# GRatTWCU/Social-STGCNN

Hardware: AMD Instinct MI355X
Metric: scene-windows/sec fwd+bwd (obs=8,pred=12) (higher is better)
Workload: dtype f32; 1 GPU; synthetic V=32 scene-windows, obs 8 / pred 12, batch 2048 per GPU, f32 (BASELINE north-star: V<=32, batch=2048; SURVEY 8d generator); global_batch=2048, step=aggregation + forward + bivariate NLL + backward + SGD update, parallelism=dp1

## Files before the change

include/stgcnn_hip.h:

```cpp
#ifndef STGCNN_HIP_H
#define STGCNN_HIP_H

#include <stddef.h>
#include <stdint.h>

#ifdef __cplusplus
extern "C" {
#endif

#define STG_OK 0
#define STG_EINVAL (-1)
#define STG_EUNSUPPORTED (-2)
#define STG_ELDS (-3)

#define STG_ABI_VERSION 8
#define STG_MAX_BLOCKS 4

int stg_abi_version(void);
const char *stg_last_error(void);

int stg_adj_build(const float *rel, int64_t rel_sn, int64_t rel_sv, int64_t rel_sc, int64_t rel_st,
                  const int32_t *num_peds, int N, int V, int T, int normalize,
                  float *nodes, float *adj, void *stream);

int stg_spatial_agg_fwd(const float *x, int64_t x_sn, int64_t x_sc, int64_t x_st, int64_t x_sv,
                        const float *adj, int64_t a_sn, const int32_t *num_peds,
                        int N, int C, int T, int V, float *y, void *stream);
int stg_spatial_agg_bwd(const float *dy, const float *adj, int64_t a_sn, const int32_t *num_peds,
                        int N, int C, int T, int V, float *dx, void *stream);

int stg_conv_t_fwd(const float *x, int64_t x_sn, int64_t x_sc, int64_t x_st, int64_t x_sv,
                   const float *w, const float *b, const int32_t *num_peds,
                   int N, int Cin, int Cout, int T, int V, int kt, int pad, float *y, void *stream);
int stg_conv_t_bwd(const float *x, int64_t x_sn, int64_t x_sc, int64_t x_st, int64_t x_sv,
                   const float *w, const float *dy, const int32_t *num_peds,
                   int N, int Cin, int Cout, int T, int V, int kt, int pad,
                   float *dx, float *dw, float *db, void *stream);

typedef struct {
    int32_t n_stgcnn;
    int32_t n_txpcnn;
    int32_t c_in;
    int32_t c_out;
    int32_t t_obs;
    int32_t t_pred;
    int32_t kt;
    int32_t residual0;
    int32_t use_mdn;
    int32_t bn_mode;
    float bn_eps;
    float bn_momentum;
    int32_t flags;
    int32_t wg_waves;
} stg_model_desc;

#define STG_OPT_WG_PATH 1
#define STG_OPT_SPLIT_BF16 2
#define STG_OPT_BF16_STORE 8
#define STG_OPT_F32_MFMA 16
#define STG_OPT_WAVE_PATH 4

int64_t stg_model_param_count(const stg_model_desc *d);
int64_t stg_model_buffer_count(const stg_model_desc *d);
int64_t stg_model_ws_floats(const stg_model_desc *d, int V);
int64_t stg_model_ws_tail_floats(const stg_model_desc *d, int N, int V);
int64_t stg_model_stat_floats(const stg_model_desc *d);
int64_t stg_model_fwd_scratch_floats(const stg_model_desc *d, int N, int V);
int64_t stg_model_bwd_scratch_floats(const stg_model_desc *d, int N, int V);

int stg_model_fwd(const stg_model_desc *d, const float *params, const float *buffers,
                  const float *x, int64_t x_sn, int64_t x_sc, int64_t x_st, int64_t x_sv,
                  const float *adj, int64_t a_sn, const int32_t *num_peds, int N, int V,
                  float *y, float *ws, float *stats, float *scratch, void **events, int n_events, void *stream);
int stg_model_bwd(const stg_model_desc *d, const float *params, const float *buffers,
                  const float *x, int64_t x_sn, int64_t x_sc, int64_t x_st, int64_t x_sv,
                  const float *adj, int64_t a_sn, const int32_t *num_peds, int N, int V,
                  const float *dy, const float *ws, float *scratch, float *grad_params, float *dx,
                  void **events, int n_events, void *stream);

int stg_model_bwd_nll(const stg_model_desc *d, const float *params, const float *buffers, const float *x, int64_t x_sn,
                      int64_t x_sc, int64_t x_st, int64_t x_sv, const float *adj, int64_t a_sn, const int32_t *num_peds,
                      int N, int V, const float *y, const float *target, const float *weights, float *losses,
                      const float *ws, float *scratch, float *grad_params, void **events, int n_events, void *stream);

typedef struct stg_step_tail {
    float *params;
    const float *lr_dev;
    float lr;
    const float *stats;
    float *buffers;
    int64_t *const *nbt;
    int n_bn;
    float *total;
} stg_step_tail;
int stg_model_bwd_step(const stg_model_desc *d, const float *params, const float *buffers, const float *x, int64_t x_sn,
                       int64_t x_sc, int64_t x_st, int64_t x_sv, const float *adj, int64_t a_sn, const int32_t *num_peds,
                       int N, int V, const float *y, const float *target, const float *weights, float *losses,
                       const float *ws, float *scratch, float *grad_params, const stg_step_tail *tail, void **events,
                       int n_events, void *stream);
int stg_bn_fold(const stg_model_desc *d, const float *stats, const int32_t *num_peds, int N,
                float *buffers, int64_t *const *nbt, int n_bn, void *stream);

int stg_nll_fwd(const float *pred, int64_t p_sn, int64_t p_sf, int64_t p_sp, int64_t p_sv,
                const float *target, const int32_t *num_peds, const float *grad_scale, int N, int P, int V,
                float *loss, float *grad, void *stream);
int stg_nll_bwd(const float *grad, const float *gloss, int N, int P, int V, float *out, void *stream);

int stg_sgd_step(float *params, const float *grads, int64_t count, float lr, void *stream);

int stg_scene_order(const int32_t *num_peds, int N, int V, int32_t *order, int32_t *key_start, void *stream);

int stg_optim_step(float *params, float *grads, int64_t count, const float *lr_dev, float lr, float max_norm,
                   float *grad_norm, void *stream);

int stg_gather_windows(const float *seq_rel_all, const int32_t *win_start, const int32_t *index, int n_windows, int N,
                       int V, int T_obs, int T_pred, float *obs_rel, float *target, int32_t *num_peds, void *stream);

int stg_dp_pack(const float *grads, const float *bn_before, const float *bn_after, const int32_t *num_peds, int N,
                float momentum, int rank, int world, int n_params, int n_buffers, float *pack, void *stream);
int stg_dp_fold(const float *pack, const float *bn_before, float momentum, int rank, int world, int n_params,
                int n_buffers, float *buffers, int64_t *const *nbt, int n_bn, void *stream);
int stg_weighted_sum(const float *values, const float *weights, int N, float *out, void *stream);

int stg_train_tail(const stg_model_desc *d, const float *stats, const int32_t *num_peds, int N, float *buffers,
                   int64_t *const *nbt, int n_bn, const float *losses, const float *weights, float *total,
                   float *params, float *grads, int64_t count, const float *lr_dev, float lr, float max_norm,
                   float *grad_norm, void *stream);

int stg_bestofk_eval(const float *pred, int64_t p_sn, int64_t p_sf, int64_t p_sp, int64_t p_sv,
                     const float *target_rel, const float *obs_last, const int32_t *num_peds, const float *noise,
                     uint64_t seed, int N, int P, int V, int K, float *ade, float *fde, void *stream);

int stg_sample_trajectories(const float *pred, int64_t p_sn, int64_t p_sf, int64_t p_sp, int64_t p_sv,
                            const float *obs_last, const int32_t *num_peds, const float *noise, uint64_t seed,
                            const uint64_t *seed_dev, int N, int P, int V, int K, float *samples, float *mean,
                            void *stream);

#define STG_TRACK_MAX_DETECTIONS 2048
#define STG_TRACK_MAX_SLOTS 2048
#define STG_TRACK_DUPLICATE 1
#define STG_TRACK_OVERFLOW 2
#define STG_TRACK_TRUNCATED 4
#define STG_TRACK_TOO_MANY 8
int stg_frame_scene_counts(const int32_t *frame_start, const int64_t *ids, int F, int T_obs, int32_t *count,
                           void *stream);
int stg_frame_scenes(const int32_t *frame_start, const int64_t *ids, const double *xy, const int32_t *frames, int N,
                     int V, int T_obs, double scale, double *obs_abs, int64_t *out_ids, int32_t *num_peds,
                     void *stream);
int stg_track_push(const int64_t *det_id, const double *det_xy, const int32_t *det_count, int M_max, int64_t *slot_id,
                   uint32_t *mask, double *ring, int32_t *head_flags, int S, int T_obs, double scale, int V,
                   double *obs_abs, int64_t *out_ids, int32_t *num_peds, void *stream);

#define STG_TRACK_MAX_STREAMS 4096
#define STG_TRACK_MAX_TOTAL_DETECTIONS (STG_TRACK_MAX_STREAMS * STG_TRACK_MAX_DETECTIONS)
int stg_track_push_streams(const int64_t *det_id, int64_t id_stride, const double *det_xy, int64_t xy_stride,
                           int M_total, const int32_t *det_start, const int32_t *pushed, int NS, int M_max,
                           int64_t *slot_id, uint32_t *mask, double *ring, int32_t *head_flags, int S, int T_obs,
                           double scale, int V, double *obs_abs, int64_t *out_ids, int32_t *num_peds,
                           int32_t *out_flags, int block_threads, void *stream);

int stg_fill_tracks(double *obs_abs, const int32_t *seen, const int32_t *num_peds, int N, int T_obs, int V,
                    double scale, void *stream);
int stg_frame_scene_counts_rule(const int32_t *frame_start, const int64_t *ids, int F, int T_obs, int min_seen,
                                int max_gap, int32_t *count, void *stream);
int stg_frame_scenes_rule(const int32_t *frame_start, const int64_t *ids, const double *xy, const int32_t *frames,
                          int N, int V, int T_obs, double scale, int min_seen, int max_gap, double *obs_abs,
                          int64_t *out_ids, int32_t *num_peds, int32_t *seen, void *stream);
int stg_track_push_rule(const int64_t *det_id, const double *det_xy, const int32_t *det_count, int M_max,
                        int64_t *slot_id, uint32_t *mask, double *ring, int32_t *head_flags, int S, int T_obs,
                        double scale, int V, int min_seen, int max_gap, double *obs_abs, int64_t *out_ids,
                        int32_t *num_peds, int32_t *seen, void *stream);
int stg_track_push_streams_rule(const int64_t *det_id, int64_t id_stride, const double *det_xy, int64_t xy_stride,
                                int M_total, const int32_t *det_start, const int32_t *pushed, int NS, int M_max,
                                int64_t *slot_id, uint32_t *mask, double *ring, int32_t *head_flags, int S, int T_obs,
                                double scale, int V, int min_seen, int max_gap, double *obs_abs, int64_t *out_ids,
                                int32_t *num_peds, int32_t *out_flags, int32_t *seen, int block_threads,
                                void *stream);

#define STG_TRACK_MAX_HISTORY 256
#define STG_TRACK_TIME_ORDER 16
int stg_track_push_timed(const int64_t *det_id, const double *det_xy, const int32_t *det_count,
                         const int64_t *det_time, int M_max, int64_t *slot_id, int64_t *t_ring, double *xy_ring,
                         int32_t *slot_head, int64_t *clock, int32_t *head_flags, int S, int R, int T_obs, double scale,
                         int V, int64_t step, int64_t max_dt, int min_seen, int max_gap, double *obs_abs,
                         int64_t *out_ids, int32_t *num_peds, int32_t *seen, void *stream);
int stg_track_push_streams_timed(const int64_t *det_id, int64_t id_stride, const double *det_xy, int64_t xy_stride,
                                 int M_total, const int32_t *det_start, const int32_t *pushed, const int64_t *det_time,
                                 int NS, int M_max, int64_t *slot_id, int64_t *t_ring, double *xy_ring,
                                 int32_t *slot_head, int64_t *clock, int32_t *head_flags, int S, int R, int T_obs,
                                 double scale, int V, int64_t step, int64_t max_dt, int min_seen, int max_gap,
                                 double *obs_abs, int64_t *out_ids, int32_t *num_peds, int32_t *out_flags,
                                 int32_t *seen, int block_threads, void *stream);

#define STG_RISK_MAX_V 256
#define STG_RISK_MAX_K 64
#define STG_RISK_MAX_Z 16
#define STG_RISK_MAX_P 32
int stg_sample_risk(const float *pred, int64_t p_sn, int64_t p_sf, int64_t p_sp, int64_t p_sv, const float *obs_last,
                    const int32_t *num_peds, const float *noise, uint64_t seed, const uint64_t *seed_dev, int N, int P,
                    int V, int K, float radius, const float *zones, int64_t z_sn, int Z, int32_t *conflict,
                    int32_t *conflict_any, int32_t *partner, int32_t *pair, int32_t *zone_any, int32_t *zone_count,
                    int32_t *ped_zone, void *stream);

#define STG_SCORE_MAX_V 256
#define STG_SCORE_MAX_K 64
#define STG_SCORE_MAX_P 32
#define STG_SCORE_MAX_Q 4
typedef struct stg_score_state {
    int64_t *rec_ids;
    int32_t *rec_peds;
    float *rec_mean, *rec_cov, *rec_samples, *acc, *acc_mean;
    int32_t *steps, *head;
    double *totals, *traj_totals;
} stg_score_state;
typedef struct stg_score_out {
    int64_t *rec_ids;
    int32_t *matched;
    float *err, *d2, *nll, *best;
    int32_t *traj_steps;
    float *traj_ade, *traj_fde, *traj_ade_mean, *traj_fde_mean;
} stg_score_out;
int stg_score_push(const int64_t *det_id, const double *det_xy, const int32_t *det_count, int M_max, double scale,
                   const float *mean, const float *v_pred, int64_t p_sn, int64_t p_sf, int64_t p_sp, int64_t p_sv,
                   const float *samples, const int64_t *ids, const int32_t *num_peds, int P, int V, int K,
                   const stg_score_state *state, const float *thr, int Q, const stg_score_out *out, void *stream);
int stg_score_push_streams(const int64_t *det_id, int64_t id_stride, const double *det_xy, int64_t xy_stride,
                           int M_total, const int32_t *det_start, const int32_t *pushed, int NS, int M_max,
                           double scale, const float *mean, const float *v_pred, int64_t p_sn, int64_t p_sf,
                           int64_t p_sp, int64_t p_sv, const float *samples, const int64_t *ids,
                           const int32_t *num_peds, int P, int V, int K, const stg_score_state *state,
                           const float *thr, int Q, const stg_score_out *out, void *stream);

#define STG_ASSOC_MAX_SLOTS STG_TRACK_MAX_SLOTS
#define STG_ASSOC_MAX_DETECTIONS STG_TRACK_MAX_DETECTIONS
#define STG_ASSOC_FULL 1
int stg_associate(int64_t *det_id, const double *det_xy, const int32_t *det_count, int M_max, int64_t *trk_id,
                  double *trk_pos, double *trk_vel, int32_t *trk_miss, int32_t *trk_hits, int64_t *next_id,
                  int32_t *assoc_flags, int C, double scale, double gate2, double gate_new2, int max_miss,
                  void *stream);
int stg_associate_streams(int64_t *det_id, int64_t id_stride, const double *det_xy, int64_t xy_stride, int M_total,
                          const int32_t *det_start, const int32_t *pushed, int NS, int M_max, int64_t *trk_id,
                          double *trk_pos, double *trk_vel, int32_t *trk_miss, int32_t *trk_hits, int64_t *next_id,
                          int32_t *assoc_flags, int C, double scale, double gate2, double gate_new2, int max_miss,
                          void *stream);

int stg_selftest_mfma(const float *a, const float *b, int K, float *c, void *stream);

#ifdef __cplusplus
}
#endif
#endif
```

social_stgcnn_amd/_lib.py:

```python
import ctypes
import os
import subprocess

import torch

_HERE = os.path.dirname(os.path.abspath(__file__))
CSRC = os.path.join(_HERE, "csrc")
DIAG = os.environ.get("STG_USE_DIAG_LIB", "0") not in ("", "0")
LIB_PATH = os.path.join(CSRC, "libstgcnn_hip_diag.so" if DIAG else "libstgcnn_hip.so")
ABI_VERSION = 8
OPT_WG_PATH, OPT_SPLIT_BF16, OPT_WAVE_PATH, OPT_BF16_STORE, OPT_F32_MFMA = 1, 2, 4, 8, 16
EUNSUPPORTED = -2

c_f = ctypes.c_void_p
c_i = ctypes.c_int
c_l = ctypes.c_int64


class ModelDesc(ctypes.Structure):
    _fields_ = [("n_stgcnn", ctypes.c_int32), ("n_txpcnn", ctypes.c_int32), ("c_in", ctypes.c_int32),
                ("c_out", ctypes.c_int32), ("t_obs", ctypes.c_int32), ("t_pred", ctypes.c_int32),
                ("kt", ctypes.c_int32), ("residual0", ctypes.c_int32), ("use_mdn", ctypes.c_int32),
                ("bn_mode", ctypes.c_int32), ("bn_eps", ctypes.c_float), ("bn_momentum", ctypes.c_float),
                ("flags", ctypes.c_int32), ("wg_waves", ctypes.c_int32)]


class ScoreState(ctypes.Structure):
    _fields_ = [(n, ctypes.c_void_p) for n in ("rec_ids", "rec_peds", "rec_mean", "rec_cov", "rec_samples", "acc",
                                               "acc_mean", "steps", "head", "totals", "traj_totals")]


class ScoreOut(ctypes.Structure):
    _fields_ = [(n, ctypes.c_void_p) for n in ("rec_ids", "matched", "err", "d2", "nll", "best", "traj_steps",
                                               "traj_ade", "traj_fde", "traj_ade_mean", "traj_fde_mean")]


_SIGNATURES = {
    "stg_abi_version": (c_i, []),
    "stg_last_error": (ctypes.c_char_p, []),
    "stg_adj_build": (c_i, [c_f, c_l, c_l, c_l, c_l, c_f, c_i, c_i, c_i, c_i, c_f, c_f, c_f]),
    "stg_spatial_agg_fwd": (c_i, [c_f, c_l, c_l, c_l, c_l, c_f, c_l, c_f, c_i, c_i, c_i, c_i, c_f, c_f]),
    "stg_spatial_agg_bwd": (c_i, [c_f, c_f, c_l, c_f, c_i, c_i, c_i, c_i, c_f, c_f]),
    "stg_conv_t_fwd": (c_i, [c_f, c_l, c_l, c_l, c_l, c_f, c_f, c_f, c_i, c_i, c_i, c_i, c_i, c_i, c_i, c_f, c_f]),
    "stg_conv_t_bwd": (c_i, [c_f, c_l, c_l, c_l, c_l, c_f, c_f, c_f, c_i, c_i, c_i, c_i, c_i, c_i, c_i,
                             c_f, c_f, c_f, c_f]),
    "stg_model_param_count": (c_l, [ctypes.POINTER(ModelDesc)]),
    "stg_model_buffer_count": (c_l, [ctypes.POINTER(ModelDesc)]),
    "stg_model_ws_floats": (c_l, [ctypes.POINTER(ModelDesc), c_i]),
    "stg_model_ws_tail_floats": (c_l, [ctypes.POINTER(ModelDesc), c_i, c_i]),
    "stg_model_stat_floats": (c_l, [ctypes.POINTER(ModelDesc)]),
    "stg_model_fwd_scratch_floats": (c_l, [ctypes.POINTER(ModelDesc), c_i, c_i]),
    "stg_model_bwd_scratch_floats": (c_l, [ctypes.POINTER(ModelDesc), c_i, c_i]),
    "stg_model_fwd": (c_i, [ctypes.POINTER(ModelDesc), c_f, c_f, c_f, c_l, c_l, c_l, c_l, c_f, c_l, c_f, c_i, c_i,
                            c_f, c_f, c_f, c_f, ctypes.POINTER(ctypes.c_void_p), c_i, c_f]),
    "stg_model_bwd": (c_i, [ctypes.POINTER(ModelDesc), c_f, c_f, c_f, c_l, c_l, c_l, c_l, c_f, c_l, c_f, c_i, c_i,
                            c_f, c_f, c_f, c_f, c_f, ctypes.POINTER(ctypes.c_void_p), c_i, c_f]),
    "stg_model_bwd_nll": (c_i, [ctypes.POINTER(ModelDesc), c_f, c_f, c_f, c_l, c_l, c_l, c_l, c_f, c_l, c_f, c_i, c_i,
                                c_f, c_f, c_f, c_f, c_f, c_f, c_f, ctypes.POINTER(ctypes.c_void_p), c_i, c_f]),
    "stg_model_bwd_step": (c_i, [ctypes.POINTER(ModelDesc), c_f, c_f, c_f, c_l, c_l, c_l, c_l, c_f, c_l, c_f, c_i, c_i,
                                 c_f, c_f, c_f, c_f, c_f, c_f, c_f, ctypes.c_void_p, ctypes.POINTER(ctypes.c_void_p), c_i,
                                 c_f]),
    "stg_bn_fold": (c_i, [ctypes.POINTER(ModelDesc), c_f, c_f, c_i, c_f, ctypes.POINTER(ctypes.c_void_p), c_i, c_f]),
    "stg_nll_fwd": (c_i, [c_f, c_l, c_l, c_l, c_l, c_f, c_f, c_f, c_i, c_i, c_i, c_f, c_f, c_f]),
    "stg_nll_bwd": (c_i, [c_f, c_f, c_i, c_i, c_i, c_f, c_f]),
    "stg_sgd_step": (c_i, [c_f, c_f, c_l, ctypes.c_float, c_f]),
    "stg_scene_order": (c_i, [c_f, c_i, c_i, c_f, c_f, c_f]),
    "stg_optim_step": (c_i, [c_f, c_f, c_l, c_f, ctypes.c_float, ctypes.c_float, c_f, c_f]),
    "stg_bestofk_eval": (c_i, [c_f, c_l, c_l, c_l, c_l, c_f, c_f, c_f, c_f, ctypes.c_uint64, c_i, c_i, c_i, c_i,
                               c_f, c_f, c_f]),
    "stg_sample_trajectories": (c_i, [c_f, c_l, c_l, c_l, c_l, c_f, c_f, c_f, ctypes.c_uint64, c_f, c_i, c_i, c_i, c_i,
                                      c_f, c_f, c_f]),
    "stg_sample_risk": (c_i, [c_f, c_l, c_l, c_l, c_l, c_f, c_f, c_f, ctypes.c_uint64, c_f, c_i, c_i, c_i, c_i,
                              ctypes.c_float, c_f, c_l, c_i, c_f, c_f, c_f, c_f, c_f, c_f, c_f, c_f]),
    "stg_gather_windows": (c_i, [c_f, c_f, c_f, c_i, c_i, c_i, c_i, c_i, c_f, c_f, c_f, c_f]),
    "stg_dp_pack": (c_i, [c_f, c_f, c_f, c_f, c_i, ctypes.c_float, c_i, c_i, c_i, c_i, c_f, c_f]),
    "stg_dp_fold": (c_i, [c_f, c_f, ctypes.c_float, c_i, c_i, c_i, c_i, c_f, ctypes.POINTER(ctypes.c_void_p), c_i, c_f]),
    "stg_weighted_sum": (c_i, [c_f, c_f, c_i, c_f, c_f]),
    "stg_train_tail": (c_i, [ctypes.POINTER(ModelDesc), c_f, c_f, c_i, c_f, ctypes.POINTER(ctypes.c_void_p), c_i, c_f, c_f,
                             c_f, c_f, c_f, c_l, c_f, ctypes.c_float, ctypes.c_float, c_f, c_f]),
    "stg_frame_scene_counts": (c_i, [c_f, c_f, c_i, c_i, c_f, c_f]),
    "stg_frame_scenes": (c_i, [c_f, c_f, c_f, c_f, c_i, c_i, c_i, ctypes.c_double, c_f, c_f, c_f, c_f]),
    "stg_track_push": (c_i, [c_f, c_f, c_f, c_i, c_f, c_f, c_f, c_f, c_i, c_i, ctypes.c_double, c_i, c_f, c_f, c_f,
                             c_f]),
    "stg_track_push_streams": (c_i, [c_f, c_l, c_f, c_l, c_i, c_f, c_f, c_i, c_i, c_f, c_f, c_f, c_f, c_i, c_i,
                                     ctypes.c_double, c_i, c_f, c_f, c_f, c_f, c_i, c_f]),
    "stg_fill_tracks": (c_i, [c_f, c_f, c_f, c_i, c_i, c_i, ctypes.c_double, c_f]),
    "stg_frame_scene_counts_rule": (c_i, [c_f, c_f, c_i, c_i, c_i, c_i, c_f, c_f]),
    "stg_frame_scenes_rule": (c_i, [c_f, c_f, c_f, c_f, c_i, c_i, c_i, ctypes.c_double, c_i, c_i, c_f, c_f, c_f, c_f,
                                    c_f]),
    "stg_track_push_rule": (c_i, [c_f, c_f, c_f, c_i, c_f, c_f, c_f, c_f, c_i, c_i, ctypes.c_double, c_i, c_i, c_i,
                                  c_f, c_f, c_f, c_f, c_f]),
    "stg_track_push_streams_rule": (c_i, [c_f, c_l, c_f, c_l, c_i, c_f, c_f, c_i, c_i, c_f, c_f, c_f, c_f, c_i, c_i,
                                          ctypes.c_double, c_i, c_i, c_i, c_f, c_f, c_f, c_f, c_f, c_i, c_f]),
    "stg_track_push_timed": (c_i, [c_f, c_f, c_f, c_f, c_i, c_f, c_f, c_f, c_f, c_f, c_f, c_i, c_i, c_i,
                                   ctypes.c_double, c_i, c_l, c_l, c_i, c_i, c_f, c_f, c_f, c_f, c_f]),
    "stg_track_push_streams_timed": (c_i, [c_f, c_l, c_f, c_l, c_i, c_f, c_f, c_f, c_i, c_i, c_f, c_f, c_f, c_f, c_f,
                                           c_f, c_i, c_i, c_i, ctypes.c_double, c_i, c_l, c_l, c_i, c_i, c_f, c_f, c_f,
                                           c_f, c_f, c_i, c_f]),
    "stg_score_push": (c_i, [c_f, c_f, c_f, c_i, ctypes.c_double, c_f, c_f, c_l, c_l, c_l, c_l, c_f, c_f, c_f, c_i, c_i,
                             c_i, ctypes.POINTER(ScoreState), c_f, c_i, ctypes.POINTER(ScoreOut), c_f]),
    "stg_score_push_streams": (c_i, [c_f, c_l, c_f, c_l, c_i, c_f, c_f, c_i, c_i, ctypes.c_double, c_f, c_f, c_l, c_l,
                                     c_l, c_l, c_f, c_f, c_f, c_i, c_i, c_i, ctypes.POINTER(ScoreState), c_f, c_i,
                                     ctypes.POINTER(ScoreOut), c_f]),
    "stg_associate": (c_i, [c_f, c_f, c_f, c_i, c_f, c_f, c_f, c_f, c_f, c_f, c_f, c_i, ctypes.c_double,
                            ctypes.c_double, ctypes.c_double, c_i, c_f]),
    "stg_associate_streams": (c_i, [c_f, c_l, c_f, c_l, c_i, c_f, c_f, c_i, c_i, c_f, c_f, c_f, c_f, c_f, c_f, c_f,
                                    c_i, ctypes.c_double, ctypes.c_double, ctypes.c_double, c_i, c_f]),
    "stg_selftest_mfma": (c_i, [c_f, c_f, c_i, c_f, c_f]),
}
EXPORTS = tuple(_SIGNATURES)

_lib = None


def build(verbose=False):
    cmd = ["make", "-C", CSRC, "-j8"] + (["DIAG=1"] if DIAG else [])
    res = subprocess.run(cmd, stdout=subprocess.PIPE, stderr=subprocess.STDOUT, text=True)
    if verbose or res.returncode != 0:
        print(res.stdout)
    if res.returncode != 0:
        raise RuntimeError("building libstgcnn_hip.so failed (exit %d)" % res.returncode)
    return LIB_PATH


def lib():
    global _lib
    if _lib is None:
        if not os.path.exists(LIB_PATH):
            raise RuntimeError(
                "social_stgcnn_amd: %s is missing -- build it with `make -C %s` (hipcc, "
                "--offload-arch=gfx950) or `python -c 'import __graft_entry__ as g; g.build()'`. "
                "There is no CPU or eager-PyTorch fallback for this path." % (LIB_PATH, CSRC))
        h = ctypes.CDLL(LIB_PATH)
        for name, (res, args) in _SIGNATURES.items():
            fn = getattr(h, name)
            fn.restype = res
            fn.argtypes = args
        if h.stg_abi_version() != ABI_VERSION:
            raise RuntimeError("libstgcnn_hip.so ABI %d != binding ABI %d" % (h.stg_abi_version(), ABI_VERSION))
        _lib = h
    return _lib


class StepTail(ctypes.Structure):
    _fields_ = [("params", ctypes.c_void_p), ("lr_dev", ctypes.c_void_p), ("lr", ctypes.c_float),
                ("stats", ctypes.c_void_p), ("buffers", ctypes.c_void_p), ("nbt", ctypes.POINTER(ctypes.c_void_p)),
                ("n_bn", ctypes.c_int), ("total", ctypes.c_void_p)]


class HipEvents:
    _hip = None

    @classmethod
    def hip(cls):
        if cls._hip is None:
            h = ctypes.CDLL("libamdhip64.so")
            h.hipEventCreate.argtypes = [ctypes.POINTER(ctypes.c_void_p)]
            h.hipEventElapsedTime.argtypes = [ctypes.POINTER(ctypes.c_float), ctypes.c_void_p, ctypes.c_void_p]
            h.hipEventSynchronize.argtypes = [ctypes.c_void_p]
            h.hipEventDestroy.argtypes = [ctypes.c_void_p]
            cls._hip = h
        return cls._hip

    def __init__(self, n):
        self.n = n
        self.arr = (ctypes.c_void_p * n)()
        for i in range(n):
            ev = ctypes.c_void_p()
            if self.hip().hipEventCreate(ctypes.byref(ev)) != 0:
                raise RuntimeError("hipEventCreate failed")
            self.arr[i] = ev

    def intervals_ms(self):
        out = []
        self.hip().hipEventSynchronize(self.arr[self.n - 1])
        for k in range(1, self.n):
            ms = ctypes.c_float()
            if self.hip().hipEventElapsedTime(ctypes.byref(ms), self.arr[k - 1], self.arr[k]) != 0:
                raise RuntimeError("hipEventElapsedTime failed")
            out.append(ms.value)
        return out

    def __del__(self):
        try:
            for i in range(self.n):
                self.hip().hipEventDestroy(self.arr[i])
        except Exception:
            pass


def check(rc, what):
    if rc != 0:
        msg = lib().stg_last_error().decode("utf-8", "replace")
        raise RuntimeError("%s failed (status %d): %s" % (what, rc, msg))


def stream_ptr():
    return ctypes.c_void_p(torch.cuda.current_stream().cuda_stream)


def ptr(t):
    if t is None:
        return None
    return ctypes.c_void_p(t.data_ptr())


def require_gpu(*tensors):
    for t in tensors:
        if t is not None and not t.is_cuda:
            raise RuntimeError("social_stgcnn_amd runs on MI355X only: got a %s tensor (no CPU fallback)"
                               % t.device.type)


def seed_u64(seed):
# ... 24 lines not shown
```

social_stgcnn_amd/csrc/model_bwd.hip:

```cpp
#include "model_common.hpp"
#include "stgcn_block.hpp"
#include "txp_scene_common.hpp"
#include "txp_f32_operands.hpp"
#include "step_plan.hpp"
#include "txp_wgrad.hpp"
#include "tail_parts.hpp"
#include "nll_elem.hpp"

namespace stg {

struct BwdArgs {
    ModelLayout lay;
    const float *params, *buffers, *x;
    int64_t x_sn, x_sc, x_st, x_sv;
    const float *adj;
    int64_t a_sn;
    const int32_t *num_peds;
    int N, V;
    const float *dy, *ws;
    const float *nll_target, *nll_weights;
    float *nll_losses;
    int64_t ws_stride;
    float *slab1;
    float *dzg;
// ... 200 lines not shown
                if (!STG_SKIP(a, 2)) {
                    if (l == 0)
                        txp_dgrad<Cfg::T, WAVES>(Pm + w_off, dzb, dcur, vi, false);
                    else
                        txp_dgrad<Cfg::P, WAVES>(Pm + w_off, dzb, dcur, vi, !is_out);
                }
                __syncthreads();
            }
        } else {
            for (int e = tid; e < C * T * vi; e += NT) {
                const int r = e / vi, w = e - r * vi;
                dcur[e] = dyn[(int64_t)r * V + w];
            }
            __syncthreads();
        }
        float *H1 = dzb, *DH2 = dzb + C * (T + 2) * Vl, *DB1 = DH2 + C * (T + 2) * Vl;
        for (int j = L.n_blocks - 1; j >= 0 && !STG_SKIP(a, 4); --j) {
            const float *xin = j > 0 ? wsn + L.ws_hdr_floats + (int64_t)L.blk[j - 1].ws_s * V : nullptr;
            float *dxs = j > 0 ? dcur : nullptr;
            float *dxg = j == 0 ? dxn : nullptr;
            if (L.blk[j].cin == Cfg::CIN0)
                stgcn_block_bwd<Cfg::CIN0, WAVES, true>(a, params, L.blk[j], n, vi, dcur, H1, DH2, DB1, red, tot, gsm, wsn,
                                                        xin, dxs, dxg, nullptr);
            else
                stgcn_block_bwd<Cfg::C, WAVES, true>(a, params, L.blk[j], n, vi, dcur, H1, DH2, DB1, red, tot, gsm, wsn, xin,
                                                     dxs, dxg, nullptr);
        }
    }
    __syncthreads();
    float *slab = a.slab1 + (int64_t)blockIdx.x * n_small;
    for (int e = tid; e < n_small; e += NT) slab[e] = gsm[e];
}

struct ReduceSeg {
    int p0, len, rows, row_stride;
    int64_t base;
};
struct ReduceArgs {
    ReduceSeg seg[kMaxTxp + 3];
    int n_seg;
    const float *slabs;
    float *grad;
    int n_params;
};

struct TailArgs {
    float *params;
    const float *lr_dev;
    float lr;
    const float *stats, *losses, *weights;
    const int32_t *num_peds;
    float *buffers, *total;
    NbtPtrs nbt;
    int n_reduce, n_buffers, N, stat_floats;
    float momentum;
};

__global__ __launch_bounds__(256) void reduce_slabs_kernel(const ReduceArgs a, const TailArgs t_) {
    __shared__ float part[32][8];
    if ((int)blockIdx.x >= t_.n_reduce) {
        float *acc_s = &part[0][0];
        __shared__ float dec_s[256];
        __shared__ int cnt_s[256];
        const int b = (int)blockIdx.x - t_.n_reduce;
        if (b < t_.n_buffers)
            bn_fold_body<256>(b, t_.stats, t_.num_peds, t_.N, t_.stat_floats, t_.momentum, t_.buffers, t_.nbt, acc_s, dec_s,
                              cnt_s);
        else if (t_.total)
            weighted_sum_body(t_.losses, t_.weights, t_.N, t_.total, acc_s);
        return;
    }
    const int col = threadIdx.x & 7, grp = threadIdx.x >> 3;
    const int p = blockIdx.x * 8 + col;
    float s = 0.f;
    if (p < a.n_params) {
        for (int q = 0; q < a.n_seg; ++q) {
            const ReduceSeg g = a.seg[q];
            if (p >= g.p0 && p < g.p0 + g.len) {
                const float *src = a.slabs + g.base + (p - g.p0);
                int k = grp;
                for (; k + 992 < g.rows; k += 1024) {
                    float v[32];
#pragma unroll
                    for (int u = 0; u < 32; ++u) v[u] = src[(int64_t)(k + 32 * u) * g.row_stride];
#pragma unroll
                    for (int u = 0; u < 32; ++u) s += v[u];
                }
                for (; k + 480 < g.rows; k += 512) {
                    float v[16];
#pragma unroll
                    for (int u = 0; u < 16; ++u) v[u] = src[(int64_t)(k + 32 * u) * g.row_stride];
#pragma unroll
                    for (int u = 0; u < 16; ++u) s += v[u];
                }
                for (; k + 96 < g.rows; k += 128) {
                    float v[4];
#pragma unroll
                    for (int u = 0; u < 4; ++u) v[u] = src[(int64_t)(k + 32 * u) * g.row_stride];
#pragma unroll
                    for (int u = 0; u < 4; ++u) s += v[u];
                }
                for (; k < g.rows; k += 32) s += src[(int64_t)k * g.row_stride];
            }
        }
    }
    part[grp][col] = s;
    __syncthreads();
    if (grp == 0 && p < a.n_params) {
        float t = 0.f;
#pragma unroll
        for (int g = 0; g < 32; ++g) t += part[g][col];
        a.grad[p] = t;
        if (t_.params) t_.params[p] -= (t_.lr_dev ? t_.lr_dev[0] : t_.lr) * t;
    }
}

static int env_waves(const char *name, int dflt) {
    const int w = diag_env(name, dflt);
    return (w == 1 || w == 2 || w == 4 || w == 8) ? w : dflt;
}

static size_t bwd_lds_bytes(const ModelLayout &L, int V, int waves) {
    const int plane = Cfg::P * txp_sc(V);
    const int st = (2 * Cfg::C * (Cfg::T + 2) + Cfg::C * Cfg::T) * V;
    const int reg = plane > st ? plane : st;
    const int dcur = Cfg::P * Cfg::C * V;
    const int n_small = L.n_blk_params + L.n_txp;
    const size_t fl = ((n_small + 3) & ~3) + (size_t)reg + (size_t)dcur + (size_t)waves * kRedMax + kRedMax;
    return fl * sizeof(float);
}

static int bwd_waves(const StepPath &path, int V) {
    return path.wg_waves ? path.wg_waves : (V <= 40 ? 1 : (V <= 80 ? 4 : 8));
}

static int bwd_grid_w(const ModelLayout &L, int N, int V, int waves) {
    const size_t lds = bwd_lds_bytes(L, V, waves);
    if (lds > (size_t)kLdsBytes) return -1;
    int per_cu = (int)(kLdsBytes / lds);
    const int by_waves = 8 / waves > 0 ? 8 / waves : 1;
    if (per_cu > by_waves) per_cu = by_waves;
    if (per_cu < 1) per_cu = 1;
    int grid = kNumCU * per_cu;
    if (const int g = diag_env("STG_BWD_GRID", 0)) grid = g > 0 ? g : grid;
    return grid < N ? grid : N;
}
static int bwd_grid(const ModelLayout &L, const StepPath &path, int N, int V) { return bwd_grid_w(L, N, V, bwd_waves(path, V)); }
constexpr int kBwdTierV = 32;
static int bwd_grid_small(const ModelLayout &L, int N, int V) {
    return V > kBwdTierV ? bwd_grid_w(L, N, kBwdTierV, 1) : 0;
}

struct BwdCarve {
    int64_t rows, slab2, dzg, order, total;
};
static bool bwd_carve(const ModelLayout &L, const StepPath &path, int N, int V, BwdCarve *c, WgradGeom *wg) {
    const int g1 = bwd_grid(L, path, N, V);
    if (g1 < 0) return false;
    int gs = bwd_grid_small(L, N, V);
    if (gs < 0) gs = 0;
    int64_t n_rows = g1 + gs;
    if (path.scene() && N > n_rows) n_rows = N;
    c->rows = 0;
    int64_t fl = (n_rows * (L.n_blk_params + L.n_txp) + 3) & ~(int64_t)3;
    c->slab2 = fl;
    c->dzg = fl;
    if (L.n_txp > 0) {
        if (!wgrad_geom(L, N, V, wg)) return false;
        fl = (fl + wgrad_slab_base(L.L + 1, wg->rows) + 3) & ~(int64_t)3;
        c->dzg = fl;
        fl = (fl + (int64_t)N * (L.L + 1) * dz_slot(V) + 3) & ~(int64_t)3;
    }
    c->order = fl;
    c->total = fl + order_floats(N, V);
    return true;
}

}

extern "C" {

int64_t stg_model_bwd_scratch_floats(const stg_model_desc *d, int N, int V) {
    stg::ModelLayout l;
    const int rc = stg::make_layout(d, &l);
    if (rc != STG_OK) return rc;
    if (N <= 0 || V <= 0) return stg::fail(STG_EINVAL, "stg_model_bwd_scratch_floats: N=%d V=%d", N, V);
    stg::BwdCarve c;
    stg::WgradGeom wg{};
    if (!stg::bwd_carve(l, stg::choose_path(l, N, V), N, V, &c, &wg)) return stg::fail(STG_ELDS, "stg_model_bwd: V=%d does not fit the LDS of one CU", V);
    return c.total;
}

static int model_bwd_impl(const stg_model_desc *d, const float *params, const float *buffers, const float *x, int64_t x_sn,
                          int64_t x_sc, int64_t x_st, int64_t x_sv, const float *adj, int64_t a_sn,
                          const int32_t *num_peds, int N, int V, const float *dy, const float *nll_target,
                          const float *nll_weights, float *nll_losses, const stg_step_tail *tail, const float *ws,
                          float *scratch, float *grad_params, float *dx, void **events, int n_events, void *stream) {
    using namespace stg;
    BwdArgs a{};
    const int rc = make_layout(d, &a.lay);
    if (rc != STG_OK) return rc;
    const ModelLayout &L = a.lay;
    STG_REQUIRE(N >= 0 && V > 0, STG_EINVAL, "stg_model_bwd: bad sizes N=%d V=%d", N, V);
    STG_REQUIRE(grad_params, STG_EINVAL, "stg_model_bwd: null grad_params");
    STG_REQUIRE(N == 0 || (params && buffers && x && adj && dy && ws && scratch), STG_EINVAL,
                "stg_model_bwd: null pointer");
    STG_REQUIRE((reinterpret_cast<uintptr_t>(ws) & 15) == 0 && (reinterpret_cast<uintptr_t>(scratch) & 15) == 0,
                STG_EINVAL, "stg_model_bwd: ws / scratch must be 16-byte aligned");
    hipStream_t st = as_stream(stream);
    EventList evl{events, events ? n_events : 0, 0, st};
    evl.mark();
    if (N == 0) {
        hipError_t e = hipMemsetAsync(grad_params, 0, sizeof(float) * L.n_params, st);
        if (e != hipSuccess) return hip_fail(e, "stg_model_bwd: memset");
        return STG_OK;
    }
    BwdCarve cv;
    WgradGeom wg{};
    const StepPath path = choose_path(L, N, V);
    STG_REQUIRE(bwd_carve(L, path, N, V, &cv, &wg), STG_ELDS, "stg_model_bwd: V=%d does not fit the LDS of one CU", V);
    const int n_small = L.n_blk_params + L.n_txp;
    float *rows = scratch + cv.rows, *slab2 = scratch + cv.slab2;
    float *dzg = L.n_txp > 0 ? scratch + cv.dzg : nullptr;
    STG_REQUIRE(path.scene() || !(L.flags & STG_OPT_BF16_STORE), STG_EUNSUPPORTED,
                "stg_model_bwd: bf16 storage (STG_OPT_BF16_STORE) is built for the wave-per-scene kernels only");
    STG_REQUIRE(!((L.flags & STG_OPT_BF16_STORE) && (L.flags & STG_OPT_SPLIT_BF16)), STG_EUNSUPPORTED,
                "stg_model_bwd: STG_OPT_BF16_STORE and STG_OPT_SPLIT_BF16 cannot be combined");
    if (nll_target && ((L.flags & STG_OPT_SPLIT_BF16) || L.n_txp == 0))
        return STG_EUNSUPPORTED;
    STG_REQUIRE(!(path.scene() && dx), STG_EUNSUPPORTED,
                "stg_model_bwd: dx is only computed by the workgroup-per-scene kernels: set STG_OPT_WG_PATH in the "
                "descriptor of the forward and the backward call");
    a.params = params; a.buffers = buffers; a.x = x;
    a.x_sn = x_sn; a.x_sc = x_sc; a.x_st = x_st; a.x_sv = x_sv;
    a.adj = adj; a.a_sn = a_sn; a.num_peds = num_peds; a.N = N; a.V = V;
    a.nll_target = nll_target; a.nll_weights = nll_weights; a.nll_losses = nll_losses;
    a.dy = dy; a.ws = ws; a.ws_stride = ws_floats_per_scene(L, V); a.slab1 = rows; a.dzg = dzg; a.dx = dx;
    int32_t *order = reinterpret_cast<int32_t *>(scratch + cv.order);
    bool sorted;
    const WsTail wt = ws_tail(L, path, N, V);
    const float *ws_end = ws + wt.base;
    if (tail_has_order(path, num_peds, N, V)) {
        order = reinterpret_cast<int32_t *>(const_cast<float *>(ws_end) + wt.order);
        sorted = true;
    } else {
        sorted = launch_scene_order(num_peds, N, V, order, order + N, st, order + N + V + 2);
    }
    int32_t *order_peds = order + N + V + 2;
    const int serp = diag_env("STG_WALK", 1);
    a.tier = SceneTier{sorted ? order : nullptr, sorted ? order + N : nullptr, -1, V, serp};
    a.debug_skip = diag_env("STG_DEBUG_SKIP", 0);
    int slab_rows;
    if (path.scene()) {
        TxpBwdArgs t{};
        t.lay = L; t.params = params; t.num_peds = num_peds; t.N = N; t.V = V; t.dy = dy; t.ws = ws;
        t.nll_target = nll_target; t.nll_weights = nll_weights; t.nll_losses = nll_losses;
        t.x = x; t.x_sn = x_sn; t.x_sc = x_sc; t.x_st = x_st; t.x_sv = x_sv; t.adj = adj; t.a_sn = a_sn;
        t.ws_stride = a.ws_stride; t.dzg = dzg; t.rows = rows;
        t.tier = a.tier;
        t.Vl = V;
        t.debug_skip = a.debug_skip;
        t.split_bf16 = (L.flags & STG_OPT_SPLIT_BF16) ? 1 : 0;
        t.stagger = diag_env("STG_STAGGER_B", 0);
        if (wt.wp >= 0) t.wp = reinterpret_cast<const unsigned *>(ws_end + wt.wp);
        const int rcw = launch_scene_bwd(path, t, st);
        if (rcw != STG_OK) return rcw;
        slab_rows = N;
    } else {
        const int waves = bwd_waves(path, V);
        const size_t lds = bwd_lds_bytes(L, V, waves);
        STG_REQUIRE(lds <= (size_t)kLdsBytes, STG_ELDS, "stg_model_bwd: V=%d needs %zu bytes of LDS (> %d)", V, lds,
                    kLdsBytes);
        const int grid = bwd_grid(L, path, N, V);
        void (*k1)(BwdArgs, const float *);
        switch (waves) {
            case 1: k1 = model_bwd_kernel<1>; break;
            case 2: k1 = model_bwd_kernel<2>; break;
            case 4: k1 = model_bwd_kernel<4>; break;
            default: k1 = model_bwd_kernel<8>; break;
        }
        slab_rows = grid;
        const int grid_small = a.tier.order ? bwd_grid_small(L, N, V) : 0;
        if (grid_small > 0) a.tier.v_lo = kBwdTierV;
        int rck = launch(Launch{"stg_model_bwd: K1", dim3(grid), dim3(waves * 64), lds, st}, k1, a, params);
        if (rck != STG_OK) return rck;
        if (grid_small > 0) {
            a.Vl = kBwdTierV;
            a.tier.v_lo = -1; a.tier.v_hi = kBwdTierV;
            a.slab1 = rows + (int64_t)grid * n_small;
            rck = launch(Launch{"stg_model_bwd: K1 (small scenes)", dim3(grid_small), dim3(64), bwd_lds_bytes(L, kBwdTierV, 1), st},
                         model_bwd_kernel<1>, a, params);
            if (rck != STG_OK) return rck;
            slab_rows = grid + grid_small;
            a.slab1 = rows;
            a.Vl = 0;
            a.tier.v_hi = V;
        }
    }
    evl.mark();

    ReduceArgs r{};
    r.slabs = scratch;
    r.grad = grad_params;
    r.n_params = L.n_params;
    r.seg[r.n_seg++] = ReduceSeg{0, L.n_blk_params, slab_rows, n_small, cv.rows};
    if (L.n_txp > 0) {
        r.seg[r.n_seg++] = ReduceSeg{L.prelus, L.n_txp, slab_rows, n_small, cv.rows + (int64_t)L.n_blk_params};
        WgradArgs w{};
        w.lay = L; w.num_peds = num_peds; w.order = a.tier.order; w.order_peds = sorted ? order_peds : nullptr;
        w.key_start = a.tier.key_start;
        w.serpentine = a.tier.serpentine; w.N = N; w.V = V;
        w.ws = ws; w.dzg = dzg; w.ws_stride = a.ws_stride; w.slab2 = slab2; w.rows = wg.rows; w.debug_skip = a.debug_skip;
        for (int l = 0; l <= L.L + 1; ++l) w.wg_begin[l] = wg.wg_begin[l];
        if (!STG_SKIP(a, 1)) {
            const int rck = launch_txp_wgrad(w, wg, st);
            if (rck != STG_OK) return rck;
        }
        evl.mark();
        for (int l = 0; l <= L.L; ++l) {
            const int p0 = l == L.L ? L.out_w : L.txp_w[l];
            r.seg[r.n_seg++] = ReduceSeg{p0, wgrad_row_len(l), STG_SKIP(a, 1) ? 0 : wg.wg_begin[l + 1] - wg.wg_begin[l],
                                         wgrad_row_len(l), cv.slab2 + wgrad_slab_base(l, wg.rows)};
        }
    }
    TailArgs ta{};
    ta.n_reduce = (L.n_params + 7) / 8;
    int extra = 0;
    if (tail) {
        ta.params = tail->params; ta.lr_dev = tail->lr_dev; ta.lr = tail->lr;
        ta.stats = tail->stats; ta.buffers = tail->buffers; ta.total = tail->total;
        ta.losses = nll_losses; ta.weights = nll_weights; ta.num_peds = num_peds;
        ta.N = N; ta.stat_floats = L.stat_floats; ta.momentum = d->bn_momentum;
        ta.n_buffers = (tail->stats && N > 0) ? L.n_buffers : 0;
        ta.nbt.n = tail->nbt ? tail->n_bn : 0;
        for (int k = 0; k < ta.nbt.n; ++k) ta.nbt.p[k] = tail->nbt[k];
        extra = ta.n_buffers + 1;
    }
    hipLaunchKernelGGL(reduce_slabs_kernel, dim3(ta.n_reduce + extra), dim3(256), 0, st, r, ta);
    STG_LAUNCH_CHECK("stg_model_bwd: reduce_slabs");
    evl.mark();
    evl.finish();
    return STG_OK;
}

int stg_model_bwd(const stg_model_desc *d, const float *params, const float *buffers, const float *x, int64_t x_sn,
                  int64_t x_sc, int64_t x_st, int64_t x_sv, const float *adj, int64_t a_sn, const int32_t *num_peds,
                  int N, int V, const float *dy, const float *ws, float *scratch, float *grad_params, float *dx,
                  void **events, int n_events, void *stream) {
    return model_bwd_impl(d, params, buffers, x, x_sn, x_sc, x_st, x_sv, adj, a_sn, num_peds, N, V, dy, nullptr, nullptr,
                          nullptr, nullptr, ws, scratch, grad_params, dx, events, n_events, stream);
}

int stg_model_bwd_nll(const stg_model_desc *d, const float *params, const float *buffers, const float *x, int64_t x_sn,
                      int64_t x_sc, int64_t x_st, int64_t x_sv, const float *adj, int64_t a_sn, const int32_t *num_peds,
                      int N, int V, const float *y, const float *target, const float *weights, float *losses,
                      const float *ws, float *scratch, float *grad_params, void **events, int n_events, void *stream) {
    if (!target || !losses || (N > 0 && !y)) return stg::fail(STG_EINVAL, "stg_model_bwd_nll: null pointer");
    return model_bwd_impl(d, params, buffers, x, x_sn, x_sc, x_st, x_sv, adj, a_sn, num_peds, N, V, y, target, weights,
                          losses, nullptr, ws, scratch, grad_params, nullptr, events, n_events, stream);
}

int stg_model_bwd_step(const stg_model_desc *d, const float *params, const float *buffers, const float *x, int64_t x_sn,
                       int64_t x_sc, int64_t x_st, int64_t x_sv, const float *adj, int64_t a_sn, const int32_t *num_peds,
                       int N, int V, const float *y, const float *target, const float *weights, float *losses,
                       const float *ws, float *scratch, float *grad_params, const stg_step_tail *tail, void **events,
                       int n_events, void *stream) {
    if (!target || !losses || (N > 0 && !y)) return stg::fail(STG_EINVAL, "stg_model_bwd_step: null pointer");
    if (!tail || !tail->params || (tail->stats && !tail->buffers) || tail->n_bn < 0 || tail->n_bn > 3 * STG_MAX_BLOCKS)
        return stg::fail(STG_EINVAL, "stg_model_bwd_step: bad tail");
    if (N == 0) return STG_EUNSUPPORTED;
    return model_bwd_impl(d, params, buffers, x, x_sn, x_sc, x_st, x_sv, adj, a_sn, num_peds, N, V, y, target, weights,
                          losses, tail, ws, scratch, grad_params, nullptr, events, n_events, stream);
}

}
```

social_stgcnn_amd/csrc/model_fwd.hip:

```cpp
#include "model_common.hpp"
#include "stgcn_block.hpp"
#include "txp_scene_common.hpp"
#include "txp_f32_operands.hpp"
#include "step_plan.hpp"

namespace stg {

struct FwdArgs {
    ModelLayout lay;
    const float *params, *buffers, *x;
    int64_t x_sn, x_sc, x_st, x_sv;
    const float *adj;
    int64_t a_sn;
    const int32_t *num_peds;
    int N, V;
    float *y, *ws;
    int64_t ws_stride;
    float *stats;
    const int32_t *order;
    const float *agg;
    int64_t agg_stride, agg_ax, agg_cs;
    int debug_skip;
};

// ... 4 lines not shown
                              const float *in, float *out, int vi, int V, float *zsave, float *yout) {
    constexpr int C = Cfg::C, P = Cfg::P, KS = CINL * 9 / 4;
    const int lane = threadIdx.x & 63, wave = threadIdx.x >> 6;
    const int nq = lane & 15, kq = lane >> 4;
    const int SW = txp_sw(vi), SC = txp_sc(vi);
    const int npos = C * vi, ntiles = (npos + 15) >> 4;
    float wreg[KS];
    load_w_fwd<CINL>(W, wreg);
    f32x4 binit;
#pragma unroll
    for (int r = 0; r < 4; ++r) binit[r] = (4 * kq + r) < P ? bias[4 * kq + r] : 0.f;

    for (int tile0 = wave * 2; tile0 < ntiles; tile0 += WAVES * 2) {
        int pos[2], hh[2], ww[2], base[2];
        bool ok[2];
#pragma unroll
        for (int u = 0; u < 2; ++u) {
            pos[u] = (tile0 + u) * 16 + nq;
            ok[u] = pos[u] < npos;
            const int pc = ok[u] ? pos[u] : 0;
            hh[u] = pc / vi;
            ww[u] = pc - hh[u] * vi;
            base[u] = kq * SC + hh[u] * SW + ww[u];
        }
        f32x4 acc0 = binit, acc1 = binit;
#pragma unroll
        for (int tap = 0; tap < 9; ++tap) {
            const int toff = (tap / 3) * SW + (tap % 3);
#pragma unroll
            for (int j = 0; j < CINL / 4; ++j) {
                const float b0 = in[base[0] + 4 * j * SC + toff];
                const float b1 = in[base[1] + 4 * j * SC + toff];
                acc0 = __builtin_amdgcn_mfma_f32_16x16x4f32(wreg[tap * (CINL / 4) + j], b0, acc0, 0, 0, 0);
                acc1 = __builtin_amdgcn_mfma_f32_16x16x4f32(wreg[tap * (CINL / 4) + j], b1, acc1, 0, 0, 0);
            }
        }
#pragma unroll
        for (int u = 0; u < 2; ++u) {
            if (!ok[u] || kq == 3) continue;
            const f32x4 acc = u == 0 ? acc0 : acc1;
#pragma unroll
            for (int r = 0; r < 4; ++r) {
                const int co = 4 * kq + r;
                const float z = acc[r];
                const int flat = (co * C + hh[u]) * vi + ww[u];
                if (kind == 2) {
                    yout[(int64_t)(co * C + hh[u]) * V + ww[u]] = z;
                } else {
                    const int li = co * SC + (hh[u] + 1) * SW + (ww[u] + 1);
                    float av = z > 0.f ? z : alpha * z;
                    if (kind == 1) av += in[li];
                    out[li] = av;
                    if (zsave) zsave[flat] = z;
                }
            }
        }
    }
}

template <int WAVES>
__global__ __launch_bounds__(WAVES * 64) void model_fwd_kernel(const FwdArgs a, const float *__restrict__ params,
                                                               const float *__restrict__ buffers) {
    constexpr int C = Cfg::C, T = Cfg::T, P = Cfg::P, NT = WAVES * 64;
    extern __shared__ __attribute__((aligned(16))) float sm[];
    const int V = a.V, tid = threadIdx.x;
    const int xin_floats = C * T * V;
    const int plane_floats = fwd_plane_floats(V);
    const int reg_floats = plane_floats > 3 * C * T * V ? plane_floats : 3 * C * T * V;
    float *bufA = sm;
    float *reg = bufA + plane_floats;
    float *red = reg + reg_floats;
    const ModelLayout &L = a.lay;
    const int c_in = L.blk[0].cin;
    const int out_rows = L.n_txp > 0 ? C * P : C * T;

    for (int it = blockIdx.x; it < a.N; it += gridDim.x) {
        const int n = a.order ? a.order[it] : it;
        int vi = a.num_peds ? a.num_peds[n] : V;
        vi = vi < 0 ? 0 : (vi > V ? V : vi);
        float *yn = a.y + (int64_t)n * out_rows * V;
        if (vi < V)
            for (int e = tid; e < out_rows * (V - vi); e += NT) {
                const int r = e / (V - vi), w = vi + (e - r * (V - vi));
                yn[(int64_t)r * V + w] = 0.f;
            }
        if (vi == 0) continue;
        float *wsn = a.ws ? a.ws + n * a.ws_stride : nullptr;
        float *statn = a.stats ? a.stats + (int64_t)n * L.stat_floats : nullptr;
        const int SW = txp_sw(vi), SC = txp_sc(vi);
        __syncthreads();
        float *X = reg, *G = reg + xin_floats, *H = G + C * T * V;
        {
            const float *xn = a.x + n * a.x_sn;
            for (int e = tid; e < c_in * T * vi; e += NT) {
                const int v = e % vi, ct = e / vi, t = ct % T, c = ct / T;
                X[e] = xn[c * a.x_sc + t * a.x_st + v * a.x_sv];
            }
            if (L.n_txp > 0) {
                float4 *z4 = reinterpret_cast<float4 *>(bufA);
                for (int e = tid; e < ((P * SC) >> 2); e += NT) z4[e] = make_float4(0.f, 0.f, 0.f, 0.f);
            }
        }
        __syncthreads();
        for (int j = 0; j < L.n_blocks && !STG_SKIP(a, 32); ++j) {
            const bool last = j == L.n_blocks - 1;
            float *yb = (last && L.n_txp == 0) ? yn : nullptr;
            const float *pax = j == 0 ? a.agg + n * a.agg_stride + a.agg_ax : nullptr;
            const float *pcs = j == 0 ? a.agg + n * a.agg_stride + a.agg_cs : nullptr;
            if (L.blk[j].cin == Cfg::CIN0)
                stgcn_block_fwd<Cfg::CIN0, WAVES>(a, params, buffers, L.blk[j], n, vi, X, G, H, red, wsn, statn, pax, pcs,
                                                  last && L.n_txp > 0, bufA, SC, bufA, 0, yb, !last);
            else
                stgcn_block_fwd<Cfg::C, WAVES>(a, params, buffers, L.blk[j], n, vi, X, G, H, red, wsn, statn, pax, pcs,
                                               last && L.n_txp > 0, bufA, SC, bufA, 0, yb, !last);
            float *tmp = X; X = H; H = tmp;
        }
        if (L.n_txp == 0 || STG_SKIP(a, 16)) continue;
        float *bufB = reg;
        for (int e = tid; e < P * SC; e += NT) bufB[e] = 0.f;
        __syncthreads();
        const float *__restrict__ Pm = params;
        float *in = bufA, *out = bufB;
        auto save_plane = [&](const float *pl, int idx) {
            if (!wsn) return;
            float *dst = wsn + ws_plane_off(L, V, idx);
            for (int h = 0; h < C; ++h)
                for (int e = tid; e < SW * P; e += NT) {
                    const int col = e / P, ch = e - col * P;
                    dst[(h * SW) * P + e] = pl[ch * SC + (h + 1) * SW + col];
                }
        };
        save_plane(in, 0);
        for (int l = 0; l < L.L; ++l) {
            float *zs = wsn ? wsn + L.ws_hdr_floats + (int64_t)L.ws_z[l] * V : nullptr;
            const float alpha = Pm[L.prelus + l];
            if (l == 0)
                txp_layer_fwd<Cfg::T, WAVES>(Pm + L.txp_w[0], Pm + L.txp_b[0], alpha, 0, in, out, vi, V, zs, nullptr);
            else
                txp_layer_fwd<Cfg::P, WAVES>(Pm + L.txp_w[l], Pm + L.txp_b[l], alpha, 1, in, out, vi, V, zs, nullptr);
            __syncthreads();
            float *tmp = in; in = out; out = tmp;
            save_plane(in, l + 1);
        }
        txp_layer_fwd<Cfg::P, WAVES>(Pm + L.out_w, Pm + L.out_b, 0.f, 2, in, out, vi, V, nullptr, yn);
    }
}

static size_t fwd_lds_bytes(int V, int waves) {
    const int plane = fwd_plane_floats(V);
    const int reg = plane > 3 * Cfg::C * Cfg::T * V ? plane : 3 * Cfg::C * Cfg::T * V;
    return (size_t)(plane + reg + waves * 16 + 16) * sizeof(float);
}

}

extern "C" int stg_model_fwd(const stg_model_desc *d, const float *params, const float *buffers, const float *x,
                             int64_t x_sn, int64_t x_sc, int64_t x_st, int64_t x_sv, const float *adj,
                             int64_t a_sn, const int32_t *num_peds, int N, int V, float *y, float *ws,
                             float *stats, float *scratch, void **events, int n_events, void *stream) {
    using namespace stg;
    FwdArgs a{};
    const int rc = make_layout(d, &a.lay);
    if (rc != STG_OK) return rc;
    STG_REQUIRE(N >= 0 && V > 0, STG_EINVAL, "stg_model_fwd: bad sizes N=%d V=%d", N, V);
    if (N == 0) return STG_OK;
    STG_REQUIRE(params && buffers && x && adj && y, STG_EINVAL, "stg_model_fwd: null pointer");
    STG_REQUIRE(scratch && (reinterpret_cast<uintptr_t>(scratch) & 15) == 0, STG_EINVAL,
                "stg_model_fwd: scratch (stg_model_fwd_scratch_floats floats, 16-byte aligned) is missing");
    STG_REQUIRE(!ws || (reinterpret_cast<uintptr_t>(ws) & 15) == 0, STG_EINVAL, "stg_model_fwd: ws must be 16-byte aligned");
    const ModelLayout &L = a.lay;
    a.params = params; a.buffers = buffers; a.x = x;
    a.x_sn = x_sn; a.x_sc = x_sc; a.x_st = x_st; a.x_sv = x_sv;
    a.adj = adj; a.a_sn = a_sn; a.num_peds = num_peds; a.N = N; a.V = V;
    a.y = y; a.ws = ws; a.ws_stride = ws_floats_per_scene(L, V); a.stats = stats;
    const StepPath path = choose_path(L, N, V);
    const FwdCarve fc = fwd_carve(L, path, N, V);
    const WsTail wt = ws_tail(L, path, N, V);
    float *ws_end = ws ? ws + wt.base : nullptr;
    STG_REQUIRE(path.scene() || !(L.flags & STG_OPT_BF16_STORE), STG_EUNSUPPORTED,
                "stg_model_fwd: bf16 storage (STG_OPT_BF16_STORE) is built for the wave-per-scene kernels only "
                "(one st_gcn block, input_feat 2, V <= 68, no STG_OPT_WG_PATH)");
    hipStream_t st = as_stream(stream);
    EventList evl{events, events ? n_events : 0, 0, st};
    evl.mark();
    const BlockLayout &b0 = L.blk[0];
    if (ws) {
        a.agg = ws; a.agg_stride = a.ws_stride;
        a.agg_ax = L.ws_hdr_floats + (int64_t)b0.ws_ax * V;
        a.agg_cs = L.ws_hdr_floats + (int64_t)b0.ws_cs * V;
    } else {
        a.agg = scratch + fc.agg; a.agg_stride = (int64_t)(b0.cin + 1) * Cfg::T * V;
        a.agg_ax = 0;
        a.agg_cs = (int64_t)b0.cin * Cfg::T * V;
    }
    a.debug_skip = diag_env("STG_DEBUG_SKIP", 0);
    int32_t *order = reinterpret_cast<int32_t *>(ws_end && path.scene() ? ws_end + wt.order : scratch + fc.order);
    bool sorted_in_agg = false;
    {
        AggPrep prep{};
        prep.params = params;
        prep.n_layers = L.L + 1;
        for (int l = 0; l <= L.L; ++l) prep.w_off[l] = l < L.L ? L.txp_w[l] : L.out_w;
        if (ws_end && wt.wp >= 0) prep.wp = reinterpret_cast<unsigned *>(ws_end + wt.wp);
        if (fc.wp_fwd >= 0) prep.wp_fwd = reinterpret_cast<unsigned *>(scratch + fc.wp_fwd);
        sorted_in_agg = path.scene() && agg_sorts(num_peds, N, V);
        if (sorted_in_agg) { prep.order = order; prep.key_start = order + N; prep.order_peds = order + N + V + 2; }
        const int rca = launch_stgcn_agg(b0.cin, x, x_sn, x_sc, x_st, x_sv, adj, a_sn, num_peds, N, V,
                                         const_cast<float *>(a.agg), a.agg_stride, a.agg_ax, a.agg_cs, st,
                                         (prep.wp || prep.wp_fwd || prep.order) ? &prep : nullptr);
        if (rca != STG_OK) return rca;
    }
    evl.mark();
    if (path.scene()) {
        bool sorted = sorted_in_agg;
        if (!sorted) {
            sorted = launch_scene_order(num_peds, N, V, order, order + N, st, order + N + V + 2);
            if (!sorted && scene_order_applies(num_peds, N, V)) return hip_fail(hipErrorLaunchFailure, "stg_model_fwd: scene_order launch");
        }
        TxpFwdArgs t{};
        t.lay = L; t.params = params; t.buffers = buffers; t.num_peds = num_peds; t.N = N; t.V = V;
        t.x = x; t.x_sn = x_sn; t.x_sc = x_sc; t.x_st = x_st; t.x_sv = x_sv;
        t.adj = adj; t.a_sn = a_sn;
        t.agg = a.agg; t.agg_stride = a.agg_stride; t.agg_ax = a.agg_ax; t.agg_cs = a.agg_cs;
        t.y = y; t.ws = ws; t.ws_stride = a.ws_stride; t.stats = stats;
        if (fc.wp_fwd >= 0) t.wpf = reinterpret_cast<const unsigned *>(scratch + fc.wp_fwd);
        if (fc.stamps >= 0) t.stamps = reinterpret_cast<unsigned long long *>(scratch + fc.stamps);
        const int serp = diag_env("STG_WALK", 1);
        t.tier = SceneTier{sorted ? order : nullptr, sorted ? order + N : nullptr, -1, V, serp};
        t.Vl = V;
        t.debug_skip = a.debug_skip;
        t.stagger = diag_env("STG_STAGGER_F", 0);
        const int rcw = launch_scene_fwd(path, t, st);
        evl.mark();
        evl.finish();
        return rcw;
    }
    int waves = V <= 12 ? 1 : (V <= 40 ? 2 : (V <= 80 ? 4 : 8));
    if (path.wg_waves) waves = path.wg_waves;
    const size_t lds = fwd_lds_bytes(V, waves);
    STG_REQUIRE(lds <= (size_t)kLdsBytes, STG_ELDS, "stg_model_fwd: V=%d needs %zu bytes of LDS (> %d)", V, lds,
                kLdsBytes);
    const Launch lc{"stg_model_fwd", dim3((unsigned)N), dim3(waves * 64), lds, st};
    int rck;
    switch (waves) {
        case 1: rck = launch(lc, model_fwd_kernel<1>, a, params, buffers); break;
        case 2: rck = launch(lc, model_fwd_kernel<2>, a, params, buffers); break;
        case 4: rck = launch(lc, model_fwd_kernel<4>, a, params, buffers); break;
        default: rck = launch(lc, model_fwd_kernel<8>, a, params, buffers); break;
    }
    if (rck != STG_OK) return rck;
    evl.mark();
    evl.finish();
    return STG_OK;
}
```

social_stgcnn_amd/csrc/model_layout.hip:

```cpp
#include <cstring>
#include <type_traits>
#include "model_common.hpp"
#include "scene_order.hpp"
#include "step_plan.hpp"
#include "txp_wave.hpp"

namespace stg {

int make_layout(const stg_model_desc *d, ModelLayout *lay) {
    STG_REQUIRE(d && lay, STG_EINVAL, "model descriptor is null");
    STG_REQUIRE(d->n_stgcnn >= 1 && d->n_stgcnn <= STG_MAX_BLOCKS, STG_EUNSUPPORTED,
                "n_stgcnn=%d outside 1..%d", d->n_stgcnn, STG_MAX_BLOCKS);
    STG_REQUIRE(d->n_txpcnn >= 0 && d->n_txpcnn <= kMaxTxp, STG_EUNSUPPORTED, "n_txpcnn=%d outside 0..%d",
                d->n_txpcnn, kMaxTxp);
    STG_REQUIRE(d->c_out == Cfg::C && d->t_obs == Cfg::T && d->kt == Cfg::KT, STG_EUNSUPPORTED,
                "fused kernels are built for output_feat=%d seq_len=%d kernel_size=%d (got %d,%d,%d)", Cfg::C,
                Cfg::T, Cfg::KT, d->c_out, d->t_obs, d->kt);
    STG_REQUIRE(d->c_in == Cfg::CIN0 || d->c_in == Cfg::C, STG_EUNSUPPORTED,
                "fused kernels are built for input_feat %d or %d (got %d)", Cfg::CIN0, Cfg::C, d->c_in);
    STG_REQUIRE(d->n_txpcnn == 0 || d->t_pred == Cfg::P, STG_EUNSUPPORTED,
                "fused kernels are built for pred_seq_len=%d (got %d)", Cfg::P, d->t_pred);
    STG_REQUIRE(d->bn_mode == 0 || d->bn_mode == 1, STG_EINVAL, "bn_mode=%d (0 eval, 1 per-scene train)", d->bn_mode);
    STG_REQUIRE(d->residual0 >= 0 && d->residual0 <= 2, STG_EINVAL, "residual0=%d", d->residual0);
    STG_REQUIRE(d->residual0 != 1 || d->c_in == d->c_out, STG_EINVAL, "identity residual needs c_in == c_out");
    STG_REQUIRE((d->flags & ~(STG_OPT_WG_PATH | STG_OPT_SPLIT_BF16 | STG_OPT_WAVE_PATH | STG_OPT_BF16_STORE | STG_OPT_F32_MFMA)) == 0, STG_EINVAL,
                "unknown flags 0x%x", d->flags);
    STG_REQUIRE(d->wg_waves == 0 || d->wg_waves == 1 || d->wg_waves == 2 || d->wg_waves == 4 || d->wg_waves == 8,
                STG_EINVAL, "wg_waves=%d (0 auto, 1, 2, 4, 8)", d->wg_waves);
    ModelLayout &l = *lay;
    l = layout_of(ModelShape{d->n_stgcnn, d->n_txpcnn, d->c_in, d->residual0, d->use_mdn});
    l.bn_mode = d->bn_mode;
    l.eps = d->bn_eps;
    l.momentum = d->bn_momentum;
    l.flags = d->flags;
    l.wg_waves = d->wg_waves;
    return STG_OK;
}

bool is_canonical(const ModelLayout &L) {
    ModelLayout c = L;
    c.eps = kCanonLayout.eps;
    c.momentum = kCanonLayout.momentum;
    c.bn_mode = kCanonLayout.bn_mode;
    c.flags = kCanonLayout.flags;
    c.wg_waves = kCanonLayout.wg_waves;
    static_assert(std::is_trivially_copyable<ModelLayout>::value && sizeof(ModelLayout) % 4 == 0, "compared bytewise");
    return std::memcmp(&c, &kCanonLayout, sizeof c) == 0;
}

constexpr int kSmallBatch = 288;

StepPath choose_path(const ModelLayout &L, int N, int V) {
    StepPath p{StepPath::Workgroup, L.wg_waves, txp_fwd_x6_fits(L, V), txp_bwd_x6_fits(L, V)};
    if (L.n_txp < 1 || L.n_blocks != 1 || L.blk[0].cin != Cfg::CIN0 || (L.flags & STG_OPT_WG_PATH)) return p;
    if (p.fwd_x6 && p.bwd_x6) {
        p.kind = StepPath::SceneX6;
    } else if (txp_wave_f32_fits(V)) {
        if (N >= kSmallBatch || L.wg_waves != 0 || V > 40 || (L.flags & (STG_OPT_WAVE_PATH | STG_OPT_BF16_STORE)))
            p.kind = StepPath::WaveF32;
        else
            p.wg_waves = N <= 192 ? 8 : 4;
    }
    return p;
}

FwdCarve fwd_carve(const ModelLayout &L, const StepPath &path, int N, int V) {
    const bool stamps = diag_env("STG_STAMPS", 0) != 0;
    FwdCarve c;
    c.agg = 0;
    c.order = (((int64_t)N * (L.blk[0].cin + 1) * Cfg::T * V + 3) & ~(int64_t)3) + 4;
    c.stamps = stamps ? c.order + order_floats(N, V) : -1;
    const int64_t wp = (c.order + order_floats(N, V) + (stamps ? (int64_t)N * 32 : 0) + 3) & ~(int64_t)3;
    c.wp_fwd = path.scene() && path.fwd_x6 ? wp : -1;
    c.total = wp + (path.fwd_x6 ? txp_bwd_x6_wp_floats(L) : 0);
    return c;
}

WsTail ws_tail(const ModelLayout &L, const StepPath &path, int N, int V) {
    WsTail t;
    t.base = (int64_t)N * ws_floats_per_scene(L, V);
    t.wp = path.scene() && path.bwd_x6 ? 0 : -1;
    t.order = path.bwd_x6 ? txp_bwd_x6_wp_floats(L) : 0;
    t.total = t.order + order_floats(N, V);
    return t;
}

int launch_scene_fwd(const StepPath &path, const TxpFwdArgs &a, hipStream_t st) {
    return path.fwd_x6 ? launch_txp_fwd_x6(a, st) : launch_txp_fwd_wave(a, st);
}
int launch_scene_bwd(const StepPath &path, const TxpBwdArgs &a, hipStream_t st) {
    return path.bwd_x6 ? launch_txp_bwd_x6(a, st) : launch_txp_bwd_wave(a, st);
}

__global__ __launch_bounds__(1024) void scene_order_kernel(const int32_t *__restrict__ num_peds, int N, int V,
                                                           int32_t *__restrict__ order,
                                                           int32_t *__restrict__ key_start,
                                                           int32_t *__restrict__ order_peds) {
    extern __shared__ int hist[];
    __shared__ int wave_tot[16];
    scene_order_body<16>(num_peds, N, V, order, key_start, order_peds, hist, wave_tot);
}

bool launch_scene_order(const int32_t *num_peds, int N, int V, int32_t *order, int32_t *key_start, hipStream_t st,
                        int32_t *order_peds) {
    if (!order || !scene_order_applies(num_peds, N, V)) return false;
    const size_t lds = (size_t)(V + 1) * 16 * sizeof(int);
    if (lds > 48 * 1024 &&
        hipFuncSetAttribute(reinterpret_cast<const void *>(&scene_order_kernel),
                            hipFuncAttributeMaxDynamicSharedMemorySize, (int)lds) != hipSuccess)
        return false;
    hipLaunchKernelGGL(scene_order_kernel, dim3(1), dim3(1024), lds, st, num_peds, N, V, order, key_start, order_peds);
    return hipGetLastError() == hipSuccess;
}

}

extern "C" {

int64_t stg_model_param_count(const stg_model_desc *d) {
    stg::ModelLayout l;
    const int rc = stg::make_layout(d, &l);
    return rc == STG_OK ? l.n_params : rc;
}
int64_t stg_model_buffer_count(const stg_model_desc *d) {
    stg::ModelLayout l;
    const int rc = stg::make_layout(d, &l);
    return rc == STG_OK ? l.n_buffers : rc;
}
int64_t stg_model_ws_floats(const stg_model_desc *d, int V) {
    stg::ModelLayout l;
    const int rc = stg::make_layout(d, &l);
    if (rc != STG_OK) return rc;
    if (V <= 0) return stg::fail(STG_EINVAL, "stg_model_ws_floats: V=%d", V);
    return stg::ws_floats_per_scene(l, V);
}
int64_t stg_model_ws_tail_floats(const stg_model_desc *d, int N, int V) {
    stg::ModelLayout l;
    const int rc = stg::make_layout(d, &l);
    if (rc != STG_OK) return rc;
    if (N < 0 || V <= 0) return stg::fail(STG_EINVAL, "stg_model_ws_tail_floats: N=%d V=%d", N, V);
    return stg::ws_tail(l, stg::choose_path(l, N, V), N, V).total;
}
int64_t stg_model_fwd_scratch_floats(const stg_model_desc *d, int N, int V) {
    stg::ModelLayout l;
    const int rc = stg::make_layout(d, &l);
    if (rc != STG_OK) return rc;
    if (N < 0 || V <= 0) return stg::fail(STG_EINVAL, "stg_model_fwd_scratch_floats: N=%d V=%d", N, V);
    return stg::fwd_carve(l, stg::choose_path(l, N, V), N, V).total;
}
int stg_scene_order(const int32_t *num_peds, int N, int V, int32_t *order, int32_t *key_start, void *stream) {
    STG_REQUIRE(N >= 0 && V > 0, STG_EINVAL, "stg_scene_order: bad sizes N=%d V=%d", N, V);
    if (N == 0) return STG_OK;
    STG_REQUIRE(num_peds && order, STG_EINVAL, "stg_scene_order: null pointer");
    STG_REQUIRE(N >= 2, STG_EUNSUPPORTED, "stg_scene_order: a single scene needs no order");
    STG_REQUIRE(N <= stg::kOrderMaxN && V <= stg::kOrderMaxV, STG_EUNSUPPORTED,
                "stg_scene_order: N=%d V=%d outside the single-workgroup sort (N <= %d, V <= %d)", N, V,
                stg::kOrderMaxN, stg::kOrderMaxV);
    STG_REQUIRE(stg::launch_scene_order(num_peds, N, V, order, key_start, stg::as_stream(stream)), STG_EINVAL,
                "stg_scene_order: launch failed");
    return STG_OK;
}

int64_t stg_model_stat_floats(const stg_model_desc *d) {
    stg::ModelLayout l;
    const int rc = stg::make_layout(d, &l);
    return rc == STG_OK ? l.stat_floats : rc;
}

}
```

social_stgcnn_amd/csrc/step_plan.hpp:

```cpp
#pragma once
#include "model_common.hpp"

namespace stg {

struct TxpFwdArgs;
struct TxpBwdArgs;

struct StepPath {
    enum Kind { SceneX6, WaveF32, Workgroup } kind;
    int wg_waves;
    bool fwd_x6, bwd_x6;
    bool scene() const { return kind != Workgroup; }
};
StepPath choose_path(const ModelLayout &L, int N, int V);

struct FwdCarve {
    int64_t agg, order, stamps, wp_fwd, total;
};
FwdCarve fwd_carve(const ModelLayout &L, const StepPath &path, int N, int V);

struct WsTail {
    int64_t base, wp, order, total;
};
WsTail ws_tail(const ModelLayout &L, const StepPath &path, int N, int V);
inline bool tail_has_order(const StepPath &path, const int32_t *num_peds, int N, int V) {
    return path.scene() && scene_order_applies(num_peds, N, V);
}

int launch_scene_fwd(const StepPath &path, const TxpFwdArgs &a, hipStream_t st);
int launch_scene_bwd(const StepPath &path, const TxpBwdArgs &a, hipStream_t st);

}
```

social_stgcnn_amd/csrc/txp_scene_common.hpp:

```cpp
#pragma once
#include "model_common.hpp"
#include "stgcn_block.hpp"

namespace stg {

struct MixGeom {
    int on;
    int v_small, v_mid;
    int block_floats;
};

constexpr int kTeamMaxV = 128;
struct TeamGeom {
    int on;
    int v1, v2;
    int region_floats;
};

struct TxpFwdArgs {
    ModelLayout lay;
    const float *params, *buffers;
    const int32_t *num_peds;
    SceneTier tier;
    int Vl;
    MixGeom mix;
    TeamGeom team;
    int N, V;
    const float *x;
    int64_t x_sn, x_sc, x_st, x_sv;
    const float *adj;
    int64_t a_sn;
    const float *agg;
    int64_t agg_stride, agg_ax, agg_cs;
    float *y;
    const unsigned *wpf;
    float *ws;
    int64_t ws_stride;
    float *stats;
    unsigned long long *stamps;
    int debug_skip;
    int stagger;
};

struct TxpBwdArgs {
    ModelLayout lay;
    const float *params;
    const int32_t *num_peds;
    SceneTier tier;
    int Vl;
    MixGeom mix;
    TeamGeom team;
    int N, V;
    const float *x;
    int64_t x_sn, x_sc, x_st, x_sv;
    const float *adj;
    int64_t a_sn;
    const float *dy;
    const float *nll_target;
    const float *nll_weights;
    float *nll_losses;
    const float *ws;
    int64_t ws_stride;
    float *dzg;
    const unsigned *wp;
    float *rows;
    int debug_skip;
    int split_bf16;
    int stagger;
};

bool txp_fwd_x6_fits(const ModelLayout &L, int V);
bool txp_bwd_x6_fits(const ModelLayout &L, int V);
int64_t txp_bwd_x6_wp_floats(const ModelLayout &L);
int launch_txp_fwd_x6(const TxpFwdArgs &a, hipStream_t st);
int launch_txp_bwd_x6(const TxpBwdArgs &a, hipStream_t st);

__host__ __device__ inline int ptab_floats(int v) { return ((Cfg::T * v + 1) / 2 + 3) & ~3; }
__host__ __device__ inline int bwd_ptab_floats(int v) { return ptab_floats(v) + kRedMax; }
__host__ __device__ inline int wave_param_floats(const ModelLayout &L) {
    return ((L.n_blk_params + 3) & ~3) + ((L.n_buffers + 3) & ~3);
}

__device__ __forceinline__ void build_ptab(ptab_t *ptab, int vi) {
    const int lane = threadIdx.x & 63;
    for (int p = lane; p < Cfg::T * vi; p += 64) {
        const int h = p / vi;
        ptab[p] = (ptab_t)((h << 8) | (p - h * vi));
    }
}
__device__ __forceinline__ void build_ptab(ptab_t *ptab, int w0, int wc) {
    const int lane = threadIdx.x & 63;
    if (wc <= 0 && lane == 0) ptab[0] = 0;
    for (int p = lane; p < Cfg::T * wc; p += 64) {
        const int h = p / wc;
        ptab[p] = (ptab_t)((h << 8) | (w0 + p - h * wc));
    }
}


__device__ __forceinline__ void vm_drain() { __builtin_amdgcn_s_waitcnt(0x0F70); }

__device__ __forceinline__ void stage_block_params(const ModelLayout &L, const float *__restrict__ params,
                                                   const float *__restrict__ buffers, float *blk_p, float *blk_b, int nt) {
    for (int e = threadIdx.x; e < L.n_blk_params; e += nt) blk_p[e] = params[e];
    if (buffers)
        for (int e = threadIdx.x; e < L.n_buffers; e += nt) blk_b[e] = buffers[e];
    __syncthreads();
}

inline int wave_wpb(size_t per_wave) {
    int wpb = diag_env("STG_TXP_WPB", 4);
    if (wpb != 1 && wpb != 2 && wpb != 8) wpb = 4;
    while (wpb > 1 && per_wave * wpb > (size_t)kLdsBytes) wpb >>= 1;
    return wpb;
}

inline int wave_grid(size_t lds, int wpb, int N) {
    int per_cu = (int)(kLdsBytes / lds);
    if (per_cu * wpb > 8) per_cu = 8 / wpb;
    if (per_cu < 1) per_cu = 1;
    const int need = (N + wpb - 1) / wpb;
    const int g = kNumCU * per_cu;
    if (g >= need) return need;
    const int rounds = (need + g - 1) / g;
    return (need + rounds - 1) / rounds;
}

}
```

social_stgcnn_amd/csrc/txp_x6.hip:

```cpp
#include "txp_scene_common.hpp"
#include "nll_elem.hpp"
#include "txp_conv_bf16.hpp"

namespace stg {

namespace {

constexpr int C = Cfg::C, P = Cfg::P, T = Cfg::T;

enum class Shape { Generic, Canon, Canon32 };
constexpr int kCanonV = 32;
constexpr int64_t kCanonWs32 = ws_floats_per_scene(kCanonLayout, kCanonV);
constexpr int64_t kCanonAggStride32[2] = {(int64_t)(Cfg::CIN0 + 1) * Cfg::T * kCanonV, kCanonWs32};
constexpr int64_t kCanonAggAx32[2] = {0, kCanonLayout.ws_hdr_floats + (int64_t)kCanonLayout.blk[0].ws_ax * kCanonV};
constexpr int64_t kCanonAggCs32[2] = {(int64_t)Cfg::CIN0 * Cfg::T * kCanonV,
                                      kCanonLayout.ws_hdr_floats + (int64_t)kCanonLayout.blk[0].ws_cs * kCanonV};

template <Shape S, typename Args>
__device__ __forceinline__ void fold_shape(Args &a) {
    if constexpr (S != Shape::Generic) {
        ModelLayout k = kCanonLayout;
        k.eps = a.lay.eps;
        k.momentum = a.lay.momentum;
        k.bn_mode = a.lay.bn_mode;
        k.flags = a.lay.flags;
        k.wg_waves = a.lay.wg_waves;
        a.lay = k;
    }
    if constexpr (S == Shape::Canon32) {
        a.V = a.Vl = kCanonV;
        a.num_peds = nullptr;
        a.tier.order = nullptr;
        a.tier.key_start = nullptr;
        a.ws_stride = kCanonWs32;
    }
}
__device__ __forceinline__ unsigned canon32_code(int t, int nq) {
    return (unsigned)(cv::tile_row(kCanonV, t) << 8 | (cv::tile_col0(kCanonV, t) + nq));
}
template <Shape S>
__device__ __forceinline__ int lay_txp_b(const ModelLayout &L, int l) {
    if constexpr (S == Shape::Generic) return L.txp_b[l];
    else return kCanonLayout.txp_b[l];
}
template <Shape S>
__device__ __forceinline__ int lay_ws_z(const ModelLayout &L, int l) {
    if constexpr (S == Shape::Generic) return L.ws_z[l];
    else return kCanonLayout.ws_z[l];
}

constexpr int kF6Tiles = 10, kF6Slots = 7;

__host__ __device__ inline int fwd6_region_floats(int v) { return (cv::image_bytes(v, kF6Slots) / 4 + 3) & ~3; }

template <bool BF, typename CK, Shape SH = Shape::Generic>
__device__ __forceinline__ void txp_fwd_scene_x6(const TxpFwdArgs &a, const float *__restrict__ params,
                                                 const float *blk_params, const float *blk_buffers, int n, int vi,
                                                 float *region, ptab_t *ptab, const CK &ck) {
    const ModelLayout &L = a.lay;
    const int V = a.V, lane = threadIdx.x & 63, nq = lane & 15, kq = lane >> 4;
    float *yn = a.y + (int64_t)n * (C * P) * V;
    if (vi < V)
        for (int e = lane + 64 * ck.ci(); e < C * P * (V - vi); e += 64 * ck.nch()) {
            const int r = e / (V - vi), w = vi + (e - r * (V - vi));
            yn[(int64_t)r * V + w] = 0.f;
        }
    if (vi == 0) return;
    const int npos = C * ck.wc(), ntiles = (npos + 15) >> 4;
    const float *Pm = params;
    float *wsn = a.ws ? a.ws + n * a.ws_stride : nullptr;
    float *statn = a.stats ? a.stats + (int64_t)n * L.stat_floats : nullptr;
    unsigned char *img = reinterpret_cast<unsigned char *>(region);
    const cv::LaneGeom lg = cv::lane_geom(vi, kF6Slots);
    constexpr bool bf16 = BF;
    const int SWs = save_sw(vi, bf16), VWs = save_vw(vi, bf16);

    {
        float sv[C * T / 2];
        const float *agn = a.agg + n * a.agg_stride;
        stgcn_block_fwd_cols<true, SH != Shape::Canon32>(a, blk_params, blk_buffers, L.blk[0], n, vi, wsn, statn,
                                                         agn + a.agg_ax, agn + a.agg_cs, nullptr, 0, region,
                                                         cv::image_bytes(vi, kF6Slots) >> 4, ptab, sv, ck);
        float *d2 = wsn ? wsn + ws_plane_off(L, V, 0) : nullptr;
        const int pl = lane & 31, pw = ck.w0() + pl, q = lane >> 5;
        if (pl < ck.wc()) {
#pragma unroll
            for (int row = 0; row < C; ++row) {
                const f32x4 v4 = {sv[row], sv[C + row], sv[2 * C + row], sv[3 * C + row]};
                cv::put4(img, (unsigned)(cv::pos_off(vi, 1 + row, pw) + 8 * q), lg.PL, v4);
                if (d2) {
                    store_vec4(d2, (row * SWs + pw + 1) * 3 + q, v4, bf16);
                    if (q == 0) store_vec4(d2, (row * SWs + pw + 1) * 3 + 2, f32x4{0.f, 0.f, 0.f, 0.f}, bf16);
                }
            }
        }
        if (wsn && lane < 2 * C * 3 && ck.lead()) {
            const int b = lane / 3, q = lane - b * 3, pos = (b >> 1) * SWs + ((b & 1) ? vi + 1 : 0);
            for (int l = 0; l <= L.L; ++l)
                store_vec4(wsn + ws_plane_off(L, V, l), pos * 3 + q, f32x4{0.f, 0.f, 0.f, 0.f}, bf16);
        }
    }
    ck.sync();

    if (STG_SKIP(a, 16)) return;
    const unsigned lds_base = (unsigned)(uintptr_t)img;
    [[maybe_unused]] cv::LaneBases lb;
    if constexpr (SH == Shape::Canon32) {
        static_assert(!CK::kTeam && 16 * kF6Tiles == C * kCanonV, "Canon32: one wave, ten full tiles");
        lb = cv::lane_bases(lds_base, lg, vi);
    }
    f32x4 av[kF6Tiles];
#pragma unroll
    for (int t = 0; t < kF6Tiles; ++t) av[t] = f32x4{0.f, 0.f, 0.f, 0.f};
    for (int l = 0; l <= L.L; ++l) {
        const bool is_out = l == L.L;
        cv::u32x4 w[cv::kWpVecs];
        cv::load_wp(a.wpf + (int64_t)l * cv::kWpDwords, w);
        const float *bias = Pm + (is_out ? L.out_b : lay_txp_b<SH>(L, l));
        f32x4 binit;
#pragma unroll
        for (int r = 0; r < 4; ++r) binit[r] = kq < 3 ? bias[4 * kq + r] : 0.f;
        const float alpha = is_out ? 0.f : Pm[L.prelus + l];
        float *zs = (wsn && !is_out) ? wsn + L.ws_hdr_floats + (int64_t)lay_ws_z<SH>(L, l) * V : nullptr;
        float *ps = (wsn && !is_out) ? wsn + ws_plane_off(L, V, l + 1) : nullptr;
        asm volatile("" ::"v"(w[0]), "v"(w[cv::kWpVecs - 1]), "v"(binit), "v"(alpha) : "memory");
        vm_drain();
        __builtin_amdgcn_s_setprio(1);
        auto finish = [&](int t, int h, int wc, bool ok, const f32x4 &z) __attribute__((always_inline)) {
            if (ok && kq < 3) {
                if (is_out) {
#pragma unroll
                    for (int r = 0; r < 4; ++r) yn[(int64_t)((4 * kq + r) * C + h) * V + wc] = z[r];
                } else {
                    f32x4 v4;
#pragma unroll
                    for (int r = 0; r < 4; ++r) v4[r] = (z[r] > 0.f ? z[r] : alpha * z[r]) + av[t][r];
                    av[t] = v4;
                    if (zs) {
                        store_vec4(zs, (h * VWs + wc) * 3 + kq, z, bf16);
                        store_vec4(ps, (h * SWs + wc + 1) * 3 + kq, v4, bf16);
                    }
                }
            }
        };
        if constexpr (SH == Shape::Canon32) {
            cv::for_tiles<kF6Tiles>([&](auto tc) __attribute__((always_inline)) {
                constexpr int t = decltype(tc)::value;
                cv::BHalf b;
                f32x4 z = binit;
                cv::load_b_half_imm<0, kCanonV, t>(lb, b);
                cv::mma_half<0>(w, b, z);
                cv::load_b_half_imm<1, kCanonV, t>(lb, b);
                cv::mma_half<1>(w, b, z);
                finish(t, cv::tile_row(kCanonV, t), cv::tile_col0(kCanonV, t) + nq, true, z);
            });
        } else {
            unsigned code = cv::tile_code(0, ptab, npos);
#pragma unroll
            for (int t = 0; t < kF6Tiles; ++t) {
                if (t < ntiles) {
                    const cv::Tile tl = cv::tile_from<1>(t, code, npos, lg, vi);
                    if (t + 1 < kF6Tiles) code = cv::tile_code(t + 1, ptab, npos);
                    cv::BHalf b;
                    f32x4 z = binit;
                    cv::load_b_half<0>(lds_base, tl, b);
                    cv::mma_half<0>(w, b, z);
                    cv::load_b_half<1>(lds_base, tl, b);
                    cv::mma_half<1>(w, b, z);
                    finish(t, tl.h, tl.w, tl.ok, z);
                }
            }
        }
        __builtin_amdgcn_s_setprio(0);
        if (is_out) break;
        ck.sync();
        unsigned codes[kF6Tiles];
#pragma unroll
        for (int t = 0; t < kF6Tiles; ++t) codes[t] = SH == Shape::Canon32 ? canon32_code(t, nq) : cv::tile_code(t, ptab, npos);
#pragma unroll
        for (int t = 0; t < kF6Tiles; ++t) {
            const int p = 16 * t + nq;
            if (p < npos && kq < 3) {
                const unsigned hw = codes[t];
                cv::put4(img, (unsigned)(cv::pos_off(vi, 1 + (int)(hw >> 8), (int)(hw & 0xffu)) + 8 * kq), lg.PL, av[t]);
            }
        }
        ck.sync();
    }
}

template <int WPB, bool BF, Shape S>
__global__ __launch_bounds__(WPB * 64, WPB == 8 ? 1 : 2) __attribute__((amdgpu_waves_per_eu(2, 2))) void txp_fwd_x6_kernel(
    const TxpFwdArgs a0, const float *__restrict__ params, const float *__restrict__ buffers) {
    extern __shared__ __attribute__((aligned(16))) float sm[];
    TxpFwdArgs a = a0;
    fold_shape<S>(a);
    if constexpr (S == Shape::Canon32) {
        const int w = a.ws != nullptr;
        a.agg_stride = kCanonAggStride32[w];
        a.agg_ax = kCanonAggAx32[w];
        a.agg_cs = kCanonAggCs32[w];
    }
    const int Vl = a.Vl, wave = threadIdx.x >> 6;
    const int per_wave = fwd6_region_floats(Vl) + ptab_floats(Vl);
    float *region = sm + wave * per_wave;
    ptab_t *ptab = reinterpret_cast<ptab_t *>(region + fwd6_region_floats(Vl));
    float *blk_p = sm + WPB * per_wave, *blk_b = blk_p + ((a.lay.n_blk_params + 3) & ~3);
    stage_block_params(a.lay, params, buffers, blk_p, blk_b, WPB * 64);
    const int gw = __builtin_amdgcn_readfirstlane(blockIdx.x * WPB + wave), nw = gridDim.x * WPB;
    int begin, end;
    tier_range(a.tier, a.N, a.V, begin, end);
    const int M = end - begin;
    for (int r = 0; r * nw < M; ++r) {
        const int it = walk_item(r, gw, nw, M, a.tier.order != nullptr && a.tier.serpentine);
        if (it < 0) continue;
        const int n = __builtin_amdgcn_readfirstlane(a.tier.order ? scene_index(a.tier.order[begin + it], a.N) : it);
        int vi = a.num_peds ? a.num_peds[n] : a.V;
        vi = __builtin_amdgcn_readfirstlane(vi < 0 ? 0 : (vi > a.V ? a.V : vi));
        txp_fwd_scene_x6<BF, SoloScene, S>(a, params, blk_p, blk_b, n, vi, region, ptab, SoloScene{vi});
        __builtin_amdgcn_wave_barrier();
    }
}

constexpr int kX6Tiles = 10;
constexpr int kX6Slots = 7;
__host__ __device__ inline int bwd6_region_floats(int v) {
    const int img = cv::image_bytes(v, kX6Slots) / 4, tail = (2 * C * (T + 2) + C * T) * v;
    return ((img > tail ? img : tail) + 3) & ~3;
}

template <bool BF, typename CK, Shape SH = Shape::Generic>
__device__ __forceinline__ void txp_bwd_scene_x6(const TxpBwdArgs &a, const float *blk_params, int n, int vi, float *region,
                                                 ptab_t *ptab, const CK &ck) {
    const ModelLayout &L = a.lay;
    const int V = a.V, lane = threadIdx.x & 63, nq = lane & 15, kq = lane >> 4;
    float *slope_row = a.rows + (int64_t)n * (L.n_blk_params + L.n_txp) + L.n_blk_params;
    if (vi == 0) {
        for (int e = lane; e < L.n_blk_params + L.n_txp; e += 64) slope_row[e - L.n_blk_params] = 0.f;
        if (a.nll_target && lane == 0) a.nll_losses[n] = 0.f;
        return;
    }
    const int npos = C * ck.wc(), ntiles = (npos + 15) >> 4;
    const float *Pm = a.params;
    const float *wsn = a.ws + n * a.ws_stride;
    const float *dyn = a.dy + (int64_t)n * (C * P) * V;
    float *prow = ck.row(slope_row - L.n_blk_params);
    if constexpr (CK::kTeam) {
        for (int e = lane; e < kTeamRow; e += 64) prow[e] = 0.f;
    }
    unsigned char *img = reinterpret_cast<unsigned char *>(region);
    const cv::LaneGeom lg = cv::lane_geom(vi, kX6Slots);
    constexpr bool bf16 = BF;
    const int VWs = save_vw(vi, bf16);
    auto tile_slots = [&](int t, int &rec, int &quad) {
        if constexpr (SH == Shape::Canon32) {
            const int h = cv::tile_row(kCanonV, t), w = cv::tile_col0(kCanonV, t) + nq;
            quad = (h * VWs + w) * 3 + kq;
            rec = cv::pos_off(vi, 1 + h, w) + 8 * kq;
        } else {
            const int p = 16 * t + nq;
            const unsigned hw = ptab[p < npos ? p : 0];
            const int h = (int)(hw >> 8), w = (int)(hw & 0xffu);
            quad = (h * VWs + w) * 3 + kq;
            rec = (p < npos && kq < 3) ? cv::pos_off(vi, 1 + h, w) + 8 * kq : -1;
        }
    };
    auto has_quad = [&](int rec) { return SH == Shape::Canon32 ? kq < 3 : rec >= 0; };
    {
        uint4 *z4 = reinterpret_cast<uint4 *>(img);
        for (int e = lane + 64 * ck.ci(); e < cv::image_bytes(vi, kX6Slots) >> 4; e += 64 * ck.nch()) z4[e] = make_uint4(0u, 0u, 0u, 0u);
    }
    [[maybe_unused]] cv::LaneBases lb;
    if constexpr (SH == Shape::Canon32) {
        static_assert(!CK::kTeam && 16 * kX6Tiles == C * kCanonV, "Canon32: one wave, ten full tiles");
        lb = cv::lane_bases((unsigned)(uintptr_t)img, lg, vi);
    } else {
        build_ptab(ptab, ck.w0(), ck.wc());
    }
    ck.sync();
    f32x4 dcur[kX6Tiles];
#pragma unroll
    for (int t = 0; t < kX6Tiles; ++t) dcur[t] = f32x4{0.f, 0.f, 0.f, 0.f};

    for (int l = L.L; l >= 0; --l) {
        float *dzo = a.dzg + ((int64_t)n * (L.L + 1) + l) * dz_slot(V);
        if (STG_SKIP(a, 512) || (l == L.L && STG_SKIP(a, 2048)) || (l != L.L && STG_SKIP(a, 4096))) {
        } else if (l == L.L) {
            const int wcw = ck.wc();
            const int vp = wcw <= 1 ? 1 : (wcw <= 2 ? 2 : (wcw <= 4 ? 4 : (wcw <= 8 ? 8 : (wcw <= 16 ? 16 : 32))));
            const int sh = __builtin_ctz(vp), rpi = 64 >> sh;
            const int sub = lane >> sh, wl = lane & (vp - 1), w = ck.w0() + wl;
            const bool okw = wl < wcw;
            float *S = reinterpret_cast<float *>(img + lg.PL);
            auto put1 = [&](int rc, float g) { S[rc * vi + w] = g; };
            if (a.nll_target) {
                const float *tn = a.nll_target + (int64_t)n * P * V * 2;
                const float inv_cnt = 1.0f / (float)(P * vi);
                const float gs = inv_cnt * (a.nll_weights ? a.nll_weights[n] : 1.f);
                float lacc = 0.f;
#pragma unroll 1
                for (int p0 = 0; p0 < P; p0 += rpi) {
                    const int p = p0 + sub;
                    if (okw && p < P) {
                        const float *q = dyn + (int64_t)p * V + w;
                        const float2 tg = *reinterpret_cast<const float2 *>(tn + ((int64_t)p * V + w) * 2);
                        float g[5];
#ifdef STG_DIAG
                        if (STG_SKIP(a, 1 << 21))
                            lacc += nll_elem_t<true>(q[0], q[(int64_t)P * V], q[(int64_t)2 * P * V], q[(int64_t)3 * P * V],
                                                     q[(int64_t)4 * P * V], tg.x, tg.y, true, g);
                        else
#endif
                        lacc += nll_elem(q[0], q[(int64_t)P * V], q[(int64_t)2 * P * V], q[(int64_t)3 * P * V],
                                         q[(int64_t)4 * P * V], tg.x, tg.y, true, g);
#pragma unroll
                        for (int f = 0; f < C; ++f) put1(f * P + p, g[f] * gs);
                    }
                }
                float ls[1] = {lacc};
                ck.template reduce<1>(ls);
                if (ck.writer()) {
                    if constexpr (CK::kTeam) prow[kTeamRowLoss] = ls[0];
                    else a.nll_losses[n] = ls[0] * inv_cnt;
                }
            } else {
                constexpr int U = 4;
#pragma unroll 1
                for (int r0 = 0; r0 < C * P; r0 += rpi * U) {
                    float dv[U];
#pragma unroll
                    for (int u = 0; u < U; ++u) {
                        const int row = r0 + u * rpi + sub;
                        dv[u] = (okw && row < C * P) ? dyn[(int64_t)row * V + w] : 0.f;
                    }
#pragma unroll
                    for (int u = 0; u < U; ++u) {
                        const int row = r0 + u * rpi + sub;
                        if (okw && row < C * P) put1(row, dv[u]);
                    }
                }
            }
            __builtin_amdgcn_wave_barrier();
            vm_drain();
            f32x4 (&qd)[kX6Tiles] = dcur;
#pragma unroll
            for (int t = 0; t < kX6Tiles; ++t) {
                const int p = 16 * t + nq;
                const unsigned hw = SH == Shape::Canon32 ? canon32_code(t, nq) : ptab[p < npos ? p : 0];
                const float *sq = S + ((4 * (kq < 3 ? kq : 0)) * C + (int)(hw >> 8)) * vi + (int)(hw & 0xffu);
                qd[t] = f32x4{sq[0], sq[C * vi], sq[2 * C * vi], sq[3 * C * vi]};
            }
            ck.sync();
            {
                uint4 *z4 = reinterpret_cast<uint4 *>(img + lg.PL);
                for (int e = lane + 64 * ck.ci(); e < (2 * lg.PL + 128) >> 4; e += 64 * ck.nch()) z4[e] = make_uint4(0u, 0u, 0u, 0u);
            }
            ck.sync();
            int rec[kX6Tiles], qv[kX6Tiles];
#pragma unroll
            for (int t = 0; t < kX6Tiles; ++t) tile_slots(t, rec[t], qv[t]);
#pragma unroll
            for (int t = 0; t < kX6Tiles; ++t) {
                if (has_quad(rec[t])) {
                    cv::put4(img, (unsigned)rec[t], lg.PL, qd[t]);
                    store_vec4(dzo, qv[t], qd[t], bf16);
                }
            }
        } else {
            const float *zl = wsn + L.ws_hdr_floats + (int64_t)lay_ws_z<SH>(L, l) * V;
            const float alpha = Pm[L.prelus + l];
            float slope_acc = 0.f;
            f32x4 zv[kX6Tiles];
            int rec[kX6Tiles], qv[kX6Tiles];
#pragma unroll
            for (int t = 0; t < kX6Tiles; ++t) tile_slots(t, rec[t], qv[t]);
#pragma unroll
            for (int t = 0; t < kX6Tiles; ++t)
                zv[t] = has_quad(rec[t]) ? load_vec4_raw(zl, qv[t], bf16) : f32x4{1.f, 1.f, 1.f, 1.f};
            asm volatile("" ::"v"(zv[0]), "v"(zv[1]), "v"(zv[2]), "v"(zv[3]), "v"(zv[4]), "v"(zv[5]), "v"(zv[6]), "v"(zv[7]),
                         "v"(zv[8]), "v"(zv[9]), "v"(alpha)
                         : "memory");
            vm_drain();
#pragma unroll
            for (int t = 0; t < kX6Tiles; ++t) {
                if (has_quad(rec[t])) {
                    f32x4 dzv;
                    const f32x4 zq = finish_vec4(zv[t], bf16);
#pragma unroll
                    for (int r = 0; r < 4; ++r) {
                        const float z = zq[r], d = dcur[t][r];
                        float dz = d;
                        if (!(z > 0.f)) {
                            dz = alpha * d;
                            slope_acc = fmaf(d, z, slope_acc);
                        }
                        dzv[r] = dz;
                    }
                    cv::put4(img, (unsigned)rec[t], lg.PL, dzv);
                    store_vec4(dzo, qv[t], dzv, bf16);
                }
            }
            float ss[1] = {slope_acc};
            ck.template reduce<1>(ss);
            if (ck.writer()) prow[L.n_blk_params + l] = ss[0];
        }
        ck.sync();
        if (!STG_SKIP(a, 1024)) {
            cv::u32x4 w[cv::kWpVecs];
            cv::load_wp(a.wp + (int64_t)l * cv::kWpDwords, w);
            asm volatile("" ::"v"(w[0]), "v"(w[cv::kWpVecs - 1]) : "memory");
            vm_drain();
            const unsigned lds_base = (unsigned)(uintptr_t)img;
            const bool keep = l != L.L && l != 0;
            const f32x4 zero = {0.f, 0.f, 0.f, 0.f};
            if constexpr (SH == Shape::Canon32) {
                cv::for_tiles<kX6Tiles>([&](auto tc) __attribute__((always_inline)) {
                    constexpr int t = decltype(tc)::value;
                    cv::BHalf b;
                    f32x4 acc = keep ? dcur[t] : zero;
                    cv::load_b_half_imm<0, kCanonV, t>(lb, b);
                    cv::mma_half<0>(w, b, acc);
                    cv::load_b_half_imm<1, kCanonV, t>(lb, b);
                    cv::mma_half<1>(w, b, acc);
                    dcur[t] = acc;
                });
            } else {
                unsigned code = cv::tile_code(0, ptab, npos);
#pragma unroll
                for (int t = 0; t < kX6Tiles; ++t) {
                    if (t < ntiles) {
                        const cv::Tile tl = cv::tile_from<1>(t, code, npos, lg, vi);
                        if (t + 1 < kX6Tiles) code = cv::tile_code(t + 1, ptab, npos);
                        cv::BHalf b;
                        f32x4 acc = keep ? dcur[t] : zero;
                        cv::load_b_half<0>(lds_base, tl, b);
                        cv::mma_half<0>(w, b, acc);
                        cv::load_b_half<1>(lds_base, tl, b);
                        cv::mma_half<1>(w, b, acc);
                        dcur[t] = acc;
                    }
                }
            }
        }
        ck.sync();
    }
    float *D = region;
#pragma unroll
    for (int t = 0; t < kX6Tiles; ++t) {
        const int p = 16 * t + nq;
        if (p < npos && kq < T / 4) {
            const unsigned hw = SH == Shape::Canon32 ? canon32_code(t, nq) : ptab[p];
            const int h = (int)(hw >> 8), ww = (int)(hw & 0xffu);
#pragma unroll
            for (int r = 0; r < 4; ++r) D[((4 * kq + r) * C + h) * vi + ww] = dcur[t][r];
        }
    }
    __builtin_amdgcn_wave_barrier();
    if constexpr (!CK::kTeam) {
        for (int e = L.L + lane; e < L.n_txp; e += 64) slope_row[e] = 0.f;
    }
    if (!STG_SKIP(a, 4))
        stgcn_block_bwd_cols<true>(a, blk_params, L.blk[0], n, vi, D, slope_row - L.n_blk_params, a.ws + n * a.ws_stride, ck);
    if constexpr (CK::kTeam) {
        ck.sync();
        if (ck.lead()) {
            float *row = slope_row - L.n_blk_params;
            const int nrow = L.n_blk_params + L.n_txp;
            for (int e0 = 0; e0 < kTeamRow; e0 += 64) {
                const int e = e0 + lane < kTeamRow ? e0 + lane : kTeamRow - 2;
                float t = ck.row_of(0)[e];
                for (int c = 1; c < ck.nch(); ++c) t += ck.row_of(c)[e];
                if (e < nrow) row[e] = t;
                if (e == kTeamRowLoss && a.nll_target) a.nll_losses[n] = t * (1.0f / (float)(P * vi));
            }
        }
    }
}

template <int WPB, bool BF, Shape S>
__global__ __launch_bounds__(WPB * 64, WPB == 8 ? 1 : 2) __attribute__((amdgpu_waves_per_eu(2, 2))) void txp_bwd_x6_kernel(
    const TxpBwdArgs a0) {
    extern __shared__ __attribute__((aligned(16))) float sm[];
    TxpBwdArgs a = a0;
    fold_shape<S>(a);
    const int Vl = a.Vl, wave = threadIdx.x >> 6;
    const int per_wave = bwd6_region_floats(Vl) + bwd_ptab_floats(Vl);
    float *region = sm + wave * per_wave;
    ptab_t *ptab = reinterpret_cast<ptab_t *>(region + bwd6_region_floats(Vl));
    float *blk_p = sm + WPB * per_wave;
    stage_block_params(a.lay, a.params, nullptr, blk_p, nullptr, WPB * 64);
    const int gw = __builtin_amdgcn_readfirstlane(blockIdx.x * WPB + wave), nw = gridDim.x * WPB;
    int begin, end;
    tier_range(a.tier, a.N, a.V, begin, end);
    const int M = end - begin;
    for (int r = 0; r * nw < M; ++r) {
        const int it = walk_item(r, gw, nw, M, a.tier.order != nullptr && a.tier.serpentine);
        if (it < 0) continue;
        const int n = __builtin_amdgcn_readfirstlane(a.tier.order ? scene_index(a.tier.order[begin + it], a.N) : it);
        int vi = a.num_peds ? a.num_peds[n] : a.V;
        vi = __builtin_amdgcn_readfirstlane(vi < 0 ? 0 : (vi > a.V ? a.V : vi));
        txp_bwd_scene_x6<BF, SoloScene, S>(a, blk_p, n, vi, region, ptab, SoloScene{vi});
        __builtin_amdgcn_wave_barrier();
    }
}

struct TeamCount {
    int n4, n2, n1;
    int u4, u2, units;
    bool sorted;
};
__device__ __forceinline__ TeamCount team_count(const SceneTier &t, const TeamGeom &g, const int32_t *num_peds, int N, int V) {
    TeamCount c;
    c.sorted = t.order && t.key_start;
    if (c.sorted) {
        const int a4 = g.v2 < V ? t.key_start[V - g.v2] : 0, a2 = g.v1 < V ? t.key_start[V - g.v1] : 0;
        c.n4 = a4;
        c.n2 = a2 - a4;
        c.u2 = (c.n2 + 1) >> 1;
    } else {
        const bool pairs = !num_peds && V > g.v1 && V <= g.v2;
        c.n4 = (V > g.v1 && !pairs) ? N : 0;
        c.n2 = pairs ? N : 0;
        c.u2 = (c.n2 + 1) >> 1;
    }
    c.n1 = N - c.n4 - c.n2;
    c.u4 = c.n4;
    c.units = c.u4 + c.u2 + ((c.n1 + 3) >> 2);
    return c;
}
struct TeamUnit {
    int n, vi;
    int nch, ci, slot;
    int w0, wc;
};
__device__ __forceinline__ TeamUnit team_unit(const SceneTier &t, const TeamCount &c, const int32_t *__restrict__ num_peds,
                                              int N, int V, int u) {
    const int wave = __builtin_amdgcn_readfirstlane(threadIdx.x >> 6);
    TeamUnit q;
    int idx;
    if (u < c.u4) {
        q.nch = 4; q.slot = 0; q.ci = wave; idx = u;
    } else if (u < c.u4 + c.u2) {
        const int i0 = c.n4 + 2 * (u - c.u4);
        if (i0 + 1 < c.n4 + c.n2) { q.nch = 2; q.slot = wave >> 1; q.ci = wave & 1; idx = i0 + q.slot; }
        else { q.nch = 4; q.slot = 0; q.ci = wave; idx = i0; }
    } else {
        q.nch = 1; q.slot = wave; q.ci = 0; idx = c.n4 + c.n2 + 4 * (u - c.u4 - c.u2) + wave;
    }
    q.n = idx < N ? (c.sorted ? scene_index(t.order[idx], N) : idx) : -1;
    q.n = __builtin_amdgcn_readfirstlane(q.n);
    int vi = q.n >= 0 ? (num_peds ? num_peds[q.n] : V) : 0;
    vi = __builtin_amdgcn_readfirstlane(vi < 0 ? 0 : (vi > V ? V : vi));
    q.vi = vi;
    const int wc = (vi + q.nch - 1) / q.nch;
    q.w0 = q.ci * wc;
    q.wc = vi - q.w0 < wc ? (vi - q.w0 > 0 ? vi - q.w0 : 0) : wc;
    return q;
}
__device__ __forceinline__ int team_workers(int units, int grid) {
    const int rounds = (units + grid - 1) / grid;
    return rounds > 0 ? (units + rounds - 1) / rounds : 1;
}
__host__ __device__ inline int team_ptab_floats() { return ptab_floats(32); }

template <bool BF>
__global__ __launch_bounds__(256, 2) __attribute__((amdgpu_waves_per_eu(2, 2))) void txp_fwd_team_kernel(
    const TxpFwdArgs a, const float *__restrict__ params, const float *__restrict__ buffers) {
    extern __shared__ __attribute__((aligned(16))) float sm[];
    const int wave = __builtin_amdgcn_readfirstlane(threadIdx.x >> 6);
    const int R = a.team.region_floats;
    ptab_t *ptab = reinterpret_cast<ptab_t *>(sm + R + wave * team_ptab_floats());
    float *xr = sm + R + 4 * team_ptab_floats();
    float *blk_p = xr + 2 * kXrFwd, *blk_b = blk_p + ((a.lay.n_blk_params + 3) & ~3);
    stage_block_params(a.lay, params, buffers, blk_p, blk_b, 256);
    const TeamCount tc = team_count(a.tier, a.team, a.num_peds, a.N, a.V);
    const int G = team_workers(tc.units, gridDim.x);
    int prev = 1;
    for (int r = 0; r * G < tc.units; ++r) {
        const int u = walk_item(r, blockIdx.x, G, tc.units, a.tier.serpentine != 0);
        if (u < 0 || (int)blockIdx.x >= G) continue;
        const TeamUnit q = team_unit(a.tier, tc, a.num_peds, a.N, a.V, u);
        if (q.nch > 1 || prev > 1) team_barrier();
        prev = q.nch;
        if (q.n >= 0) {
            const TeamScene ck{q.vi, q.w0, q.wc, q.nch, q.ci, xr + (q.slot & 1) * kXrFwd, nullptr, q.nch > 1 && !STG_SKIP(a, 1 << 20)};
            float *region = sm + q.slot * ((R >> 2) * q.nch);
            txp_fwd_scene_x6<BF>(a, params, blk_p, blk_b, q.n, q.vi, region, ptab, ck);
        }
        __builtin_amdgcn_wave_barrier();
    }
}

template <bool BF>
__global__ __launch_bounds__(256, 2) __attribute__((amdgpu_waves_per_eu(2, 2))) void txp_bwd_team_kernel(const TxpBwdArgs a) {
    extern __shared__ __attribute__((aligned(16))) float sm[];
    const int wave = __builtin_amdgcn_readfirstlane(threadIdx.x >> 6);
    const int R = a.team.region_floats;
    ptab_t *ptab = reinterpret_cast<ptab_t *>(sm + R + wave * team_ptab_floats());
    float *xr = sm + R + 4 * team_ptab_floats();
    float *blk_p = xr + kXrBwdWg;
    stage_block_params(a.lay, a.params, nullptr, blk_p, nullptr, 256);
    const TeamCount tc = team_count(a.tier, a.team, a.num_peds, a.N, a.V);
    const int G = team_workers(tc.units, gridDim.x);
    int prev = 1;
    for (int r = 0; r * G < tc.units; ++r) {
        const int u = walk_item(r, blockIdx.x, G, tc.units, a.tier.serpentine != 0);
        if (u < 0 || (int)blockIdx.x >= G) continue;
        const TeamUnit q = team_unit(a.tier, tc, a.num_peds, a.N, a.V, u);
        if (q.nch > 1 || prev > 1) team_barrier();
        prev = q.nch;
        if (q.n >= 0) {
            const TeamScene ck{q.vi, q.w0, q.wc, q.nch, q.ci, xr + (q.slot & 1) * kXrRows,
                               xr + 2 * kXrRows + q.slot * q.nch * kTeamRow, q.nch > 1 && !STG_SKIP(a, 1 << 20)};
            float *region = sm + q.slot * ((R >> 2) * q.nch);
            txp_bwd_scene_x6<BF>(a, blk_p, q.n, q.vi, region, ptab, ck);
        }
        __builtin_amdgcn_wave_barrier();
    }
}

}

bool txp_fwd_x6_fits(const ModelLayout &L, int V) {
    return L.n_txp > 0 && V <= kTeamMaxV && !(L.flags & STG_OPT_F32_MFMA) && L.n_blocks == 1 &&
           L.blk[0].cin == Cfg::CIN0 && !diag_env("STG_FWD_F32", 0);
}

constexpr int kTeamFineBatch = 1536, kTeamFinestBatch = 384;
static int team_waves(int v, int v1, int v2) { return v <= v1 ? 1 : (v <= v2 ? 2 : 4); }
static bool team_geom(int N, int V, bool uniform, TeamGeom *g) {
    g->on = 0;
    if (V > kTeamMaxV) return false;
    int v1 = 32, v2 = 64;
    if (N < kTeamFinestBatch) { v1 = 8; v2 = 16; }
    else if (N < kTeamFineBatch) { v1 = 16; v2 = 32; }
    if (uniform)
        while (v1 < 32 && (int64_t)N * team_waves(V, v1, v2) > 2048) { v1 *= 2; v2 *= 2; }
    if (const int e = diag_env("STG_TEAM_V1", 0)) v1 = e;
    if (const int e = diag_env("STG_TEAM_V2", 0)) v2 = e;
    if (v1 > 32) v1 = 32;
    if (v2 > 64) v2 = 64;
    if (v2 < v1) v2 = v1;
    auto region = [&](int v) { return fwd6_region_floats(v); };
    int r = 4 * region(v1 < V ? v1 : V);
    if (2 * region(v2 < V ? v2 : V) > r) r = 2 * region(v2 < V ? v2 : V);
    if (region(V) > r) r = region(V);
    g->on = 1; g->v1 = v1; g->v2 = v2; g->region_floats = (r + 15) & ~15;
    return true;
}
static bool team_wanted(int N, int V, bool uniform, TeamGeom *g) {
    if (!team_geom(N, V, uniform, g)) return false;
    return V > 16 * kF6Tiles / C || g->v1 < V || diag_env("STG_TEAM", 0) != 0;
}
static int team_grid(size_t lds_bytes, int N) {
    int per_cu = (int)(kLdsBytes / lds_bytes);
    if (per_cu > 2) per_cu = 2;
    if (per_cu < 1) per_cu = 1;
    const int g = kNumCU * per_cu;
    return g < N ? g : N;
}

template <typename Args>
static Shape canon_shape(const Args &a, bool *ok) {
    *ok = true;
    if (!is_canonical(a.lay)) return Shape::Generic;
    if (a.num_peds || a.V != kCanonV) return Shape::Canon;
    *ok = a.Vl == kCanonV && !a.tier.order && !a.tier.key_start && a.ws_stride == kCanonWs32;
    return Shape::Canon32;
}
static bool canon32_agg_matches(const TxpFwdArgs &a) {
    const int w = a.ws != nullptr;
    return a.agg_stride == kCanonAggStride32[w] && a.agg_ax == kCanonAggAx32[w] && a.agg_cs == kCanonAggCs32[w];
}

template <int W>
static auto fwd_x6_kernel(bool bf, Shape sh) {
    if (bf) return sh == Shape::Canon32 ? txp_fwd_x6_kernel<W, true, Shape::Canon32> : txp_fwd_x6_kernel<W, true, Shape::Generic>;
    if (sh == Shape::Canon32) return txp_fwd_x6_kernel<W, false, Shape::Canon32>;
    return sh == Shape::Canon ? txp_fwd_x6_kernel<W, false, Shape::Canon> : txp_fwd_x6_kernel<W, false, Shape::Generic>;
}
template <int W>
static auto bwd_x6_kernel(bool bf, Shape sh) {
    if (bf) {
        if (sh == Shape::Canon32) return txp_bwd_x6_kernel<W, true, Shape::Canon32>;
        return sh == Shape::Canon ? txp_bwd_x6_kernel<W, true, Shape::Canon> : txp_bwd_x6_kernel<W, true, Shape::Generic>;
    }
    if (sh == Shape::Canon32) return txp_bwd_x6_kernel<W, false, Shape::Canon32>;
    return sh == Shape::Canon ? txp_bwd_x6_kernel<W, false, Shape::Canon> : txp_bwd_x6_kernel<W, false, Shape::Generic>;
}

int launch_txp_fwd_x6(const TxpFwdArgs &a0, hipStream_t st) {
    TxpFwdArgs a = a0;
    STG_REQUIRE(a.wpf, STG_EINVAL, "txp_fwd_x6: the prepared operands are missing");
    const bool bf = (a.lay.flags & STG_OPT_BF16_STORE) != 0;
    if (team_wanted(a.N, a.V, a.num_peds == nullptr, &a.team)) {
        const size_t lds = ((size_t)a.team.region_floats + 4 * team_ptab_floats() + 2 * kXrFwd + wave_param_floats(a.lay)) * sizeof(float);
        STG_REQUIRE(lds <= (size_t)kLdsBytes, STG_ELDS, "txp_fwd_team: V=%d needs %zu bytes of LDS", a.V, lds);
        return launch(Launch{"txp_fwd_team", dim3(team_grid(lds, a.N)), dim3(256), lds, st},
                      bf ? txp_fwd_team_kernel<true> : txp_fwd_team_kernel<false>, a, a.params, a.buffers);
    }
    STG_REQUIRE(a.V <= 16 * kF6Tiles / C, STG_EUNSUPPORTED, "txp_fwd_x6: V=%d outside the exact-bf16 kernels", a.V);
    const size_t per_wave = (size_t)(fwd6_region_floats(a.Vl) + ptab_floats(a.Vl)) * sizeof(float);
    const int wpb = wave_wpb(per_wave) == 8 ? 8 : 4;
    const size_t lds = per_wave * wpb + wave_param_floats(a.lay) * sizeof(float);
    bool ok;
    const Shape sh = canon_shape(a, &ok);
    STG_REQUIRE(ok && (sh != Shape::Canon32 || canon32_agg_matches(a)), STG_EINVAL,
                "txp_fwd_x6: the canonical V=%d batch does not match its compiled layout", a.V);
    return launch(Launch{"txp_fwd_x6", dim3(wave_grid(lds, wpb, a.N)), dim3(wpb * 64), lds, st},
                  wpb == 8 ? fwd_x6_kernel<8>(bf, sh) : fwd_x6_kernel<4>(bf, sh), a, a.params, a.buffers);
}

bool txp_bwd_x6_fits(const ModelLayout &L, int V) {
    return L.n_txp > 0 && V <= kTeamMaxV && L.n_blocks == 1 && L.blk[0].cin == Cfg::CIN0 &&
           !(L.flags & (STG_OPT_SPLIT_BF16 | STG_OPT_F32_MFMA)) && !diag_env("STG_BWD_F32", 0);
}
int64_t txp_bwd_x6_wp_floats(const ModelLayout &L) { return (int64_t)(L.L + 1) * cv::kWpDwords; }
int launch_txp_bwd_x6(const TxpBwdArgs &a0, hipStream_t st) {
    TxpBwdArgs a = a0;
    STG_REQUIRE(a.wp, STG_EINVAL, "txp_bwd_x6: the prepared operands are missing");
    const bool bf = (a.lay.flags & STG_OPT_BF16_STORE) != 0;
    if (team_wanted(a.N, a.V, a.num_peds == nullptr, &a.team)) {
        const size_t lds = ((size_t)a.team.region_floats + 4 * team_ptab_floats() + kXrBwdWg + wave_param_floats(a.lay)) * sizeof(float);
        STG_REQUIRE(lds <= (size_t)kLdsBytes, STG_ELDS, "txp_bwd_team: V=%d needs %zu bytes of LDS", a.V, lds);
        return launch(Launch{"txp_bwd_team", dim3(team_grid(lds, a.N)), dim3(256), lds, st},
                      bf ? txp_bwd_team_kernel<true> : txp_bwd_team_kernel<false>, a);
    }
    STG_REQUIRE(a.V <= 16 * kX6Tiles / C, STG_EUNSUPPORTED, "txp_bwd_x6: V=%d outside the exact-bf16 kernels", a.V);
    const size_t per_wave = (size_t)(bwd6_region_floats(a.Vl) + bwd_ptab_floats(a.Vl)) * sizeof(float);
    const int wpb = wave_wpb(per_wave) == 8 ? 8 : 4;
    const size_t lds = per_wave * wpb + wave_param_floats(a.lay) * sizeof(float);
    bool ok;
    const Shape sh = canon_shape(a, &ok);
    STG_REQUIRE(ok, STG_EINVAL, "txp_bwd_x6: the canonical V=%d batch does not match its compiled layout", a.V);
    return launch(Launch{"txp_bwd_x6", dim3(wave_grid(lds, wpb, a.N)), dim3(wpb * 64), lds, st},
                  wpb == 8 ? bwd_x6_kernel<8>(bf, sh) : bwd_x6_kernel<4>(bf, sh), a);
}

}
```

social_stgcnn_amd/model.py:

```python
import torch
import torch.nn as nn

from . import ops


class ConvTemporalGraphical(nn.Module):

    def __init__(self, in_channels, out_channels, kernel_size, t_kernel_size=1, t_stride=1, t_padding=0,
                 t_dilation=1, bias=True):
        super(ConvTemporalGraphical, self).__init__()
        self.kernel_size = kernel_size
        self.conv = nn.Conv2d(in_channels, out_channels, kernel_size=(t_kernel_size, 1),
                              padding=(t_padding, 0), stride=(t_stride, 1), dilation=(t_dilation, 1), bias=bias)

    def forward(self, x, A, num_peds=None):
        assert A.size(-3) == self.kernel_size
        if self.conv.stride != (1, 1) or self.conv.dilation != (1, 1):
            raise NotImplementedError("ConvTemporalGraphical HIP path supports t_stride=1, t_dilation=1")
        x = ops.conv_t(x, self.conv.weight, self.conv.bias, self.conv.padding[0], num_peds)
        x = ops.spatial_agg(x, A, num_peds)
        return x.contiguous(), A


class _Identity:
    def __call__(self, x):
        return x


class _Zero:
    def __call__(self, x):
        return 0


def _block_tensors(blk):
    params = [blk.gcn.conv.weight, blk.gcn.conv.bias, blk.tcn[0].weight, blk.tcn[0].bias, blk.tcn[1].weight,
              blk.tcn[2].weight, blk.tcn[2].bias, blk.tcn[3].weight, blk.tcn[3].bias]
    bufs = [blk.tcn[0].running_mean, blk.tcn[0].running_var, blk.tcn[3].running_mean, blk.tcn[3].running_var]
    nbt = [blk.tcn[0].num_batches_tracked, blk.tcn[3].num_batches_tracked]
    if isinstance(blk.residual, nn.Sequential):
        params += [blk.residual[0].weight, blk.residual[0].bias, blk.residual[1].weight, blk.residual[1].bias]
        bufs += [blk.residual[1].running_mean, blk.residual[1].running_var]
        nbt += [blk.residual[1].num_batches_tracked]
    params += [blk.prelu.weight]
    return params, bufs, nbt


def _check_block(blk, training):
    if blk.gcn.conv.bias is None:
        raise NotImplementedError("st_gcn HIP path needs the gcn conv bias")
    if blk.stride != 1:
        raise NotImplementedError("st_gcn HIP path supports stride=1")
    if training and blk.tcn[4].p > 0:
        raise NotImplementedError("st_gcn HIP path supports dropout=0 in training")
    bn = blk.tcn[0]
    if bn.momentum is None or not bn.track_running_stats or not bn.affine:
        raise NotImplementedError("st_gcn HIP path needs default BatchNorm2d settings")


class st_gcn(nn.Module):

    def __init__(self, in_channels, out_channels, kernel_size, use_mdn=False, stride=1, dropout=0, residual=True):
        super(st_gcn, self).__init__()
        assert len(kernel_size) == 2
        assert kernel_size[0] % 2 == 1
        padding = ((kernel_size[0] - 1) // 2, 0)
        self.use_mdn = use_mdn
        self.stride = stride
        self.in_channels = in_channels
        self.out_channels = out_channels
        self.kt = kernel_size[0]
        self.gcn = ConvTemporalGraphical(in_channels, out_channels, kernel_size[1])
        self.tcn = nn.Sequential(
            nn.BatchNorm2d(out_channels),
            nn.PReLU(),
            nn.Conv2d(out_channels, out_channels, (kernel_size[0], 1), (stride, 1), padding),
            nn.BatchNorm2d(out_channels),
            nn.Dropout(dropout, inplace=True),
        )
        if not residual:
            self.residual = _Zero()
            self.residual_kind = 0
        elif (in_channels == out_channels) and (stride == 1):
            self.residual = _Identity()
            self.residual_kind = 1
        else:
            self.residual = nn.Sequential(
                nn.Conv2d(in_channels, out_channels, kernel_size=1, stride=(stride, 1)),
                nn.BatchNorm2d(out_channels),
            )
            self.residual_kind = 2
        self.prelu = nn.PReLU()
        self._pp = ops.FlatPack()
        self._pb = ops.FlatPack()

    def forward(self, x, A, num_peds=None):
        assert A.size(-3) == self.gcn.kernel_size
        _check_block(self, self.training)
        params, bufs, nbt = _block_tensors(self)
        flat_p = self._pp.ensure(params)
        flat_b = self._pb.ensure(bufs)
        desc = ops.make_desc(1, 0, self.in_channels, self.out_channels, x.shape[2], 0, self.kt, self.residual_kind,
                             self.use_mdn, self.training, self.tcn[0].eps, self.tcn[0].momentum,
                             options=getattr(self, "options", None))
        y = ops.fused_model(x, A, num_peds, desc, flat_p, flat_b, nbt, frozenset(), params, self)
        return y, A


class social_stgcnn(nn.Module):

    def __init__(self, n_stgcnn=1, n_txpcnn=1, input_feat=2, output_feat=5, seq_len=8, pred_seq_len=12,
                 kernel_size=3):
        super(social_stgcnn, self).__init__()
        self.n_stgcnn = n_stgcnn
        self.n_txpcnn = n_txpcnn
        self.input_feat = input_feat
        self.output_feat = output_feat
        self.seq_len = seq_len
        self.pred_seq_len = pred_seq_len
        self.kt = kernel_size

        self.st_gcns = nn.ModuleList()
        self.st_gcns.append(st_gcn(input_feat, output_feat, (kernel_size, seq_len)))
        for j in range(1, self.n_stgcnn):
            self.st_gcns.append(st_gcn(output_feat, output_feat, (kernel_size, seq_len)))

        self.tpcnns = nn.ModuleList()
        self.tpcnns.append(nn.Conv2d(seq_len, pred_seq_len, 3, padding=1))
        for j in range(1, self.n_txpcnn):
            self.tpcnns.append(nn.Conv2d(pred_seq_len, pred_seq_len, 3, padding=1))
        self.tpcnn_ouput = nn.Conv2d(pred_seq_len, pred_seq_len, 3, padding=1)

        self.prelus = nn.ModuleList()
        for j in range(self.n_txpcnn):
            self.prelus.append(nn.PReLU())
        self._pp = ops.FlatPack()
        self._pb = ops.FlatPack()

    def _tensors(self):
        params, bufs, nbt = [], [], []
        for blk in self.st_gcns:
            p, b, c = _block_tensors(blk)
            params += p
            bufs += b
            nbt += c
        n_blk = len(params)
        for conv in self.tpcnns:
            params += [conv.weight, conv.bias]
        params += [self.tpcnn_ouput.weight, self.tpcnn_ouput.bias]
        params += [p.weight for p in self.prelus]
        hidden = max(1, self.n_txpcnn - 1)
        dead = set()
        for j in range(hidden, self.n_txpcnn):
            dead.add(n_blk + 2 * j)
            dead.add(n_blk + 2 * j + 1)
            dead.add(n_blk + 2 * self.n_txpcnn + 2 + j)
        return params, bufs, nbt, frozenset(dead)

    def flat_parameters(self):
        params = self._tensors()[0]
        return self._pp.ensure(params)

    def forward(self, v, a, num_peds=None):
        return self._forward(v, a, num_peds)

    def _forward(self, v, a, num_peds=None, defer_bn_fold=False):
        assert a.size(-3) == self.st_gcns[0].gcn.kernel_size
        if self.n_txpcnn < 1:
            raise NotImplementedError("social_stgcnn needs n_txpcnn >= 1 (model.py:168 always builds tpcnns[0])")
        for blk in self.st_gcns:
            _check_block(blk, self.training)
        params, bufs, nbt, dead = self._tensors()
        flat_p = self._pp.ensure(params)
        flat_b = self._pb.ensure(bufs)
        bn = self.st_gcns[0].tcn[0]
        desc = ops.make_desc(self.n_stgcnn, self.n_txpcnn, self.input_feat, self.output_feat, self.seq_len,
                             self.pred_seq_len, self.kt, self.st_gcns[0].residual_kind, False, self.training,
                             bn.eps, bn.momentum, options=getattr(self, "options", None))
        y = ops.fused_model(v, a, num_peds, desc, flat_p, flat_b, nbt, dead, params, self, defer_bn_fold)
        return y, a
```

social_stgcnn_amd/ops.py:

```python
import collections
import ctypes
import dataclasses
import math

import torch

from . import _lib
from ._lib import ModelDesc, check, lib, peds_arg, ptr, require_gpu, seed_u64, stream_ptr


def _adj_layout(adj, n, t, v):
    if adj.dim() == 3:
        if tuple(adj.shape) != (t, v, v):
            raise ValueError("adjacency %s does not match x (T=%d, V=%d)" % (tuple(adj.shape), t, v))
        return adj.contiguous(), 0
    if adj.dim() == 4:
        if tuple(adj.shape) != (n, t, v, v):
            raise ValueError("adjacency %s does not match x (N=%d, T=%d, V=%d)" % (tuple(adj.shape), n, t, v))
        if adj.stride()[1:] != (v * v, v, 1):
            adj = adj.contiguous()
        return adj, adj.stride(0)
    raise ValueError("adjacency must be (T,V,V) or (N,T,V,V), got %d dims" % adj.dim())


def adj_build(seq_rel, num_peds=None, normalize=True, out=None):
    require_gpu(seq_rel)
    _lib.as_f32(seq_rel, "seq_rel")
    n, v, c, t = seq_rel.shape
    if c != 2:
        raise ValueError("seq_rel must be (N,V,2,T)")
    peds = peds_arg(num_peds, n, seq_rel.device)
    if out is not None:
        nodes, adj = out
        if tuple(nodes.shape) != (n, t, v, 2) or tuple(adj.shape) != (n, t, v, v) or not (
                nodes.is_contiguous() and adj.is_contiguous()):
            raise ValueError("adj_build: out = (nodes (N,T,V,2), adj (N,T,V,V)), contiguous")
    else:
        nodes = torch.empty((n, t, v, 2), device=seq_rel.device, dtype=torch.float32)
        adj = torch.empty((n, t, v, v), device=seq_rel.device, dtype=torch.float32)
    sn, sv, sc, st = seq_rel.stride()
    check(lib().stg_adj_build(ptr(seq_rel), sn, sv, sc, st, ptr(peds), n, v, t, 1 if normalize else 0,
                              ptr(nodes), ptr(adj), stream_ptr()), "stg_adj_build")
    return nodes, adj


class _SpatialAgg(torch.autograd.Function):
    @staticmethod
    def forward(ctx, x, adj, num_peds):
        require_gpu(x, adj)
        _lib.as_f32(x, "x")
        _lib.as_f32(adj, "adj")
        n, c, t, v = x.shape
        adj_c, a_sn = _adj_layout(adj, n, t, v)
        peds = peds_arg(num_peds, n, x.device)
        y = torch.empty((n, c, t, v), device=x.device, dtype=torch.float32)
        sn, sc, st, sv = x.stride()
        check(lib().stg_spatial_agg_fwd(ptr(x), sn, sc, st, sv, ptr(adj_c), a_sn, ptr(peds), n, c, t, v, ptr(y),
                                        stream_ptr()), "stg_spatial_agg_fwd")
        ctx.save_for_backward(adj_c, peds if peds is not None else torch.empty(0))
        ctx.a_sn = a_sn
        ctx.has_peds = peds is not None
        return y

    @staticmethod
    def backward(ctx, dy):
        adj_c, peds = ctx.saved_tensors
        dy = dy.contiguous()
        n, c, t, v = dy.shape
        dx = torch.empty_like(dy)
        check(lib().stg_spatial_agg_bwd(ptr(dy), ptr(adj_c), ctx.a_sn, ptr(peds) if ctx.has_peds else None, n, c, t,
                                        v, ptr(dx), stream_ptr()), "stg_spatial_agg_bwd")
        return dx, None, None


def spatial_agg(x, adj, num_peds=None):
    return _SpatialAgg.apply(x, adj, num_peds)


class _ConvT(torch.autograd.Function):
    @staticmethod
    def forward(ctx, x, weight, bias, pad, num_peds):
        require_gpu(x, weight, bias)
        _lib.as_f32(x, "x")
        n, cin, t, v = x.shape
        cout, cin_w, kt, kw = weight.shape
        if cin_w != cin or kw != 1:
            raise ValueError("weight %s does not match input channels %d" % (tuple(weight.shape), cin))
        to = t + 2 * pad - kt + 1
        peds = peds_arg(num_peds, n, x.device)
        w = weight.contiguous()
        b = bias.contiguous() if bias is not None else None
        y = torch.empty((n, cout, to, v), device=x.device, dtype=torch.float32)
        sn, sc, st, sv = x.stride()
        check(lib().stg_conv_t_fwd(ptr(x), sn, sc, st, sv, ptr(w), ptr(b), ptr(peds), n, cin, cout, t, v, kt, pad,
                                   ptr(y), stream_ptr()), "stg_conv_t_fwd")
        ctx.save_for_backward(x, w, peds if peds is not None else torch.empty(0))
        ctx.has_peds = peds is not None
        ctx.has_bias = bias is not None
        ctx.pad = pad
        return y

    @staticmethod
    def backward(ctx, dy):
        x, w, peds = ctx.saved_tensors
        dy = dy.contiguous()
        n, cin, t, v = x.shape
        cout, _, kt, _ = w.shape
        dx = torch.empty((n, cin, t, v), device=x.device, dtype=torch.float32) if ctx.needs_input_grad[0] else None
        dw = torch.zeros_like(w)
        db = torch.zeros(cout, device=x.device, dtype=torch.float32) if ctx.has_bias else None
        sn, sc, st, sv = x.stride()
        check(lib().stg_conv_t_bwd(ptr(x), sn, sc, st, sv, ptr(w), ptr(dy), ptr(peds) if ctx.has_peds else None, n,
                                   cin, cout, t, v, kt, ctx.pad, ptr(dx), ptr(dw), ptr(db), stream_ptr()),
              "stg_conv_t_bwd")
        return dx, dw, db, None, None


def conv_t(x, weight, bias, pad=0, num_peds=None):
    return _ConvT.apply(x, weight, bias, pad, num_peds)


def flat_walk(items):
    off = 0
    for i, it in enumerate(items):
        cnt = it.numel() if torch.is_tensor(it) else math.prod(it)
        yield i, off, cnt
        off += cnt


class FlatPack:

    def __init__(self):
        self.flat = None

    def ensure(self, tensors):
        total = sum(t.numel() for t in tensors)
        dev = tensors[0].device
        flat = self.flat
        if (flat is not None and flat.device == dev and flat.numel() == total
                and all(tensors[i].data_ptr() == flat.data_ptr() + 4 * off and tensors[i].is_contiguous()
                        for i, off, _ in flat_walk(tensors))):
            return flat
        flat = torch.empty(total, device=dev, dtype=torch.float32)
        with torch.no_grad():
            for i, off, n in flat_walk(tensors):
                t = tensors[i]
                flat[off:off + n].copy_(t.detach().reshape(-1))
                t.data = flat[off:off + n].view(t.shape)
        self.flat = flat
        return flat


class KernelOptions(dict):
    DEFAULTS = {"wg_path": False, "split_bf16": False, "wg_waves": 0, "wave_path": False, "bf16_store": False,
                "f32_mfma": False}

    def __init__(self, **kw):
        bad = set(kw) - set(self.DEFAULTS)
        if bad:
            raise KeyError("unknown kernel options %s" % sorted(bad))
        super().__init__(self.DEFAULTS)
        self.update(kw)


OPTIONS = KernelOptions()


def make_desc(n_stgcnn, n_txpcnn, c_in, c_out, t_obs, t_pred, kt, residual0, use_mdn, training,
              eps=1e-5, momentum=0.1, options=None):
    o = OPTIONS if options is None else options
    flags = ((_lib.OPT_WG_PATH if o["wg_path"] else 0) | (_lib.OPT_SPLIT_BF16 if o["split_bf16"] else 0)
             | (_lib.OPT_WAVE_PATH if o["wave_path"] else 0)
             | (_lib.OPT_BF16_STORE if o["bf16_store"] else 0)
             | (_lib.OPT_F32_MFMA if o["f32_mfma"] else 0))
    return ModelDesc(n_stgcnn, n_txpcnn, c_in, c_out, t_obs, t_pred, kt, residual0, 1 if use_mdn else 0,
                     1 if training else 0, eps, momentum, flags, int(o["wg_waves"]))


class KernelTimer:
    MAX_KERNELS = 8

    def __init__(self):
        self.calls = {"model_fwd": [], "model_bwd": []}

    def events(self, name):
        ev = _lib.HipEvents(self.MAX_KERNELS + 1)
        self.calls[name].append(ev)
        return ev

    def kernel_ms(self, name):
        rows = []
        for ev in self.calls[name]:
            row = []
            hip = ev.hip()
            hip.hipEventSynchronize(ev.arr[0])
            for k in range(1, ev.n):
                ms = ctypes.c_float()
                if hip.hipEventElapsedTime(ctypes.byref(ms), ev.arr[k - 1], ev.arr[k]) != 0:
                    hip.hipGetLastError()
                    break
                row.append(ms.value)
            rows.append(row)
        if not rows:
            return []
        n = min(len(r) for r in rows)
        return [sum(r[k] for r in rows) / len(rows) for k in range(n)]

    def mean_ms(self, name):
        return sum(self.kernel_ms(name))


def _timer_of(holder):
    return getattr(holder, "timer", None) if holder is not None else None


def _size(n, what):
    if n < 0:
        check(int(n), what)
    return int(n)


def _ptr_array(tensors):
    return (ctypes.c_void_p * len(tensors))(*[t.data_ptr() for t in tensors]) if len(tensors) else None


@dataclasses.dataclass(eq=False)
class FwdRecord:
    desc: ModelDesc
    a_sn: int
    dead: frozenset
    shapes: list
    flat_params: torch.Tensor
    flat_buffers: torch.Tensor
    x: torch.Tensor
    adj_c: torch.Tensor
    peds: torch.Tensor
    ws: torch.Tensor
    stats: torch.Tensor = None
    nbt: list = None
    n: int = 0


class _FusedModel(torch.autograd.Function):

    @staticmethod
    def forward(ctx, x, adj, num_peds, desc, flat_params, flat_buffers, nbt, dead, holder, grad_on, defer_bn_fold,
                *params):
        require_gpu(x, adj, flat_params, flat_buffers)
        _lib.as_f32(x, "x")
        _lib.as_f32(adj, "adj")
        L = lib()
        n, cin, t, v = x.shape
        if cin != desc.c_in or t != desc.t_obs:
            raise ValueError("input (N,%d,%d,V) does not match the model (input_feat=%d, seq_len=%d)"
                             % (cin, t, desc.c_in, desc.t_obs))
        adj_c, a_sn = _adj_layout(adj, n, t, v)
        peds = peds_arg(num_peds, n, x.device)
        training = desc.bn_mode == 1
        need_grad = grad_on and any(ctx.needs_input_grad)
        if need_grad and ctx.needs_input_grad[0] and not (desc.flags & _lib.OPT_WG_PATH):
            fields = {f: getattr(desc, f) for f, _ in ModelDesc._fields_}
            fields["flags"] |= _lib.OPT_WG_PATH
            desc = ModelDesc(**fields)
        out_t = desc.t_pred if desc.n_txpcnn > 0 else desc.t_obs
        y = torch.empty((n, desc.c_out, out_t, v), device=x.device, dtype=torch.float32)
        ws = None
        if need_grad:
            wsf = _size(L.stg_model_ws_floats(ctypes.byref(desc), v), "stg_model_ws_floats")
            tail = _size(L.stg_model_ws_tail_floats(ctypes.byref(desc), n, v), "stg_model_ws_tail_floats")
            ws = torch.empty(n * wsf + tail, device=x.device, dtype=torch.float32)
        stats = None
        if training:
            sf = L.stg_model_stat_floats(ctypes.byref(desc))
            stats = torch.empty((n, max(int(sf), 1)), device=x.device, dtype=torch.float32)
        scr = None
        nscr = _size(L.stg_model_fwd_scratch_floats(ctypes.byref(desc), n, v), "stg_model_fwd_scratch_floats")
        if nscr > 0:
            scr = torch.empty(nscr, device=x.device, dtype=torch.float32)
        if holder is not None:
            holder.last_ws_floats = ws.numel() if need_grad else 0
            holder._last_fwd_scratch = scr
        sn, sc, st, sv = x.stride()
        timer = _timer_of(holder)
        ev = timer.events("model_fwd") if timer is not None else None
        check(L.stg_model_fwd(ctypes.byref(desc), ptr(flat_params), ptr(flat_buffers), ptr(x), sn, sc, st, sv,
                              ptr(adj_c), a_sn, ptr(peds), n, v, ptr(y), ptr(ws), ptr(stats), ptr(scr),
                              ev.arr if ev else None, ev.n if ev else 0, stream_ptr()),
              "stg_model_fwd")
        rec = FwdRecord(desc, a_sn, dead, [tuple(p.shape) for p in params], flat_params, flat_buffers, x, adj_c, peds,
                        ws)
        if training and defer_bn_fold:
            rec.stats, rec.nbt, rec.n = stats, nbt, n
        elif training:
            check(L.stg_bn_fold(ctypes.byref(desc), ptr(stats), ptr(peds), n, ptr(flat_buffers), _ptr_array(nbt),
                                len(nbt), stream_ptr()), "stg_bn_fold")
        if holder is not None:
            holder._fwd_state = rec if need_grad else None
        ctx.rec = rec
        ctx.holder = holder
        return y

    @staticmethod
    def backward(ctx, dy):
        if ctx.rec.ws is None:
            raise RuntimeError("backward through a forward that saved no activations")
        grads, dx = _launch_backward(ctx.rec, ctx.holder, dy=dy.contiguous(), need_dx=ctx.needs_input_grad[0])
        return (dx, None, None, None, None, None, None, None, None, None, None, *grads)


def _launch_backward(rec, holder, dy=None, need_dx=False, y=None, target=None, weights=None, step=None):
    L = lib()
    desc, x = rec.desc, rec.x
    n, cin, t, v = x.shape
    np_ = int(L.stg_model_param_count(ctypes.byref(desc)))
    n_scratch = _size(L.stg_model_bwd_scratch_floats(ctypes.byref(desc), n, v), "stg_model_bwd_scratch_floats")
    slabs = torch.empty(n_scratch, device=x.device, dtype=torch.float32)
    grad = torch.empty(np_, device=x.device, dtype=torch.float32)
    sn, sc, st, sv = x.stride()
    timer = _timer_of(holder)
    ev = timer.events("model_bwd") if timer is not None else None
    head = (ctypes.byref(desc), ptr(rec.flat_params), ptr(rec.flat_buffers), ptr(x), sn, sc, st, sv, ptr(rec.adj_c),
            rec.a_sn, ptr(rec.peds), n, v)
    end = (ev.arr if ev else None, ev.n if ev else 0, stream_ptr())
    if dy is not None:
        out = torch.empty((n, cin, t, v), device=x.device, dtype=torch.float32) if need_dx else None
        name, rc = "stg_model_bwd", L.stg_model_bwd(*head, ptr(dy), ptr(rec.ws), ptr(slabs), ptr(grad), ptr(out), *end)
    else:
        out = losses = torch.empty(n, device=x.device, dtype=torch.float32)
        mid = (ptr(y), ptr(target), ptr(weights), ptr(losses), ptr(rec.ws), ptr(slabs), ptr(grad))
        if step is None:
            name, rc = "stg_model_bwd_nll", L.stg_model_bwd_nll(*head, *mid, *end)
        else:
            lr, lr_dev = step
            total = torch.empty(1, device=x.device, dtype=torch.float32)
            tail = _lib.StepTail()
            tail.params, tail.lr_dev, tail.lr = ptr(rec.flat_params), ptr(lr_dev), float(lr)
            tail.total = ptr(total)
            if rec.stats is not None:
                arr = _ptr_array(rec.nbt)
                tail.stats, tail.buffers, tail.nbt, tail.n_bn = ptr(rec.stats), ptr(rec.flat_buffers), arr, len(rec.nbt)
            name, rc = "stg_model_bwd_step", L.stg_model_bwd_step(*head, *mid, ctypes.addressof(tail), *end)
            out = (losses, total[0])
        if rc == _lib.EUNSUPPORTED:
            if ev is not None:
                timer.calls["model_bwd"].pop()
            return None
    check(rc, name)
    grads = [None if i in rec.dead else grad[off:off + cnt].view(rec.shapes[i])
             for i, off, cnt in flat_walk(rec.shapes)]
    if holder is not None:
        holder._flat_grad = grad
        holder._fwd_state = None
    return grads, out


def backward_from_target(holder, y, target, weights=None, step=None):
    rec = getattr(holder, "_fwd_state", None)
    if rec is None:
        raise RuntimeError("backward_from_target: no fused forward with saved activations to start from")
    n, _, _, v = rec.x.shape
    if tuple(y.shape) != (n, 5, rec.desc.t_pred, v) or not y.is_contiguous():
        return None
    target = target.to(torch.float32).contiguous()
    if tuple(target.shape) != (n, rec.desc.t_pred, v, 2):
        raise ValueError("backward_from_target: target (N,P,V,2) expected, got %s" % (tuple(target.shape),))
    w = weights.to(torch.float32).contiguous() if weights is not None else None
    res = _launch_backward(rec, holder, y=y, target=target, weights=w, step=step)
    if res is None:
        return None
    for p, g in zip(holder._tensors()[0], res[0]):
        p.grad = g
    return res[1]


def fused_model(x, adj, num_peds, desc, flat_params, flat_buffers, nbt, dead, params, holder=None,
                defer_bn_fold=False):
    return _FusedModel.apply(x, adj, num_peds, desc, flat_params, flat_buffers, nbt, dead, holder,
                             torch.is_grad_enabled(), defer_bn_fold, *params)


class _BivariateNLL(torch.autograd.Function):

    @staticmethod
    def forward(ctx, pred, target, num_peds):
        require_gpu(pred, target)
        _lib.as_f32(pred, "V_pred")
        n, p, v, f = pred.shape
        if f != 5 or tuple(target.shape) != (n, p, v, 2):
            raise ValueError("bivariate_loss: V_pred (..,P,V,5) / V_trgt (..,P,V,2) expected, got %s / %s"
                             % (tuple(pred.shape), tuple(target.shape)))
        target = target.to(torch.float32).contiguous()
        peds = peds_arg(num_peds, n, pred.device)
        loss = torch.empty(n, device=pred.device, dtype=torch.float32)
        need = ctx.needs_input_grad[0]
        grad = torch.empty((n, 5, p, v), device=pred.device, dtype=torch.float32) if need else None
        sn, sp, sv, sf = pred.stride()
        check(lib().stg_nll_fwd(ptr(pred), sn, sf, sp, sv, ptr(target), ptr(peds), None, n, p, v, ptr(loss), ptr(grad),
                                stream_ptr()), "stg_nll_fwd")
        ctx.grad = grad
        return loss

    @staticmethod
    def backward(ctx, gloss):
        grad = ctx.grad
        n, _, p, v = grad.shape
        gloss = gloss.to(torch.float32).contiguous()
        out = torch.empty_like(grad)
        check(lib().stg_nll_bwd(ptr(grad), ptr(gloss), n, p, v, ptr(out), stream_ptr()), "stg_nll_bwd")
        return out.permute(0, 2, 3, 1), None, None


def bivariate_nll(pred, target, num_peds=None):
    return _BivariateNLL.apply(pred, target, num_peds)


def bivariate_nll_with_grad(y, target, num_peds=None, weights=None):
    require_gpu(y, target)
    n, f, p, v = y.shape
    if f != 5 or tuple(target.shape) != (n, p, v, 2):
        raise ValueError("bivariate_nll_with_grad: y (N,5,P,V) / target (N,P,V,2) expected")
    target = target.to(torch.float32).contiguous()
    peds = peds_arg(num_peds, n, y.device)
    loss = torch.empty(n, device=y.device, dtype=torch.float32)
    grad = torch.empty((n, 5, p, v), device=y.device, dtype=torch.float32)
    w = weights.to(torch.float32).contiguous() if weights is not None else None
    sn, sf, sp, sv = y.stride()
    check(lib().stg_nll_fwd(ptr(y), sn, sf, sp, sv, ptr(target), ptr(peds), ptr(w), n, p, v, ptr(loss), ptr(grad),
                            stream_ptr()), "stg_nll_fwd")
    return loss, grad


def sgd_step(flat_params, flat_grads, lr):
    require_gpu(flat_params, flat_grads)
    check(lib().stg_sgd_step(ptr(flat_params), ptr(flat_grads), flat_params.numel(), float(lr), stream_ptr()),
          "stg_sgd_step")


def optim_step(flat_params, flat_grads, lr, max_norm=None, lr_dev=None, grad_norm=None):
    require_gpu(flat_params, flat_grads)
    check(lib().stg_optim_step(ptr(flat_params), ptr(flat_grads), flat_params.numel(), ptr(lr_dev), float(lr),
                               float(max_norm) if max_norm is not None else 0.0, ptr(grad_norm), stream_ptr()),
          "stg_optim_step")


def train_tail(rec, losses, weights, flat_params, flat_grads, lr, max_norm=None, lr_dev=None):
    require_gpu(losses, flat_params, flat_grads)
    w = weights.to(torch.float32).contiguous() if weights is not None else None
    out = torch.empty(1, device=losses.device, dtype=torch.float32)
    check(lib().stg_train_tail(ctypes.byref(rec.desc), ptr(rec.stats), ptr(rec.peds), rec.n, ptr(rec.flat_buffers),
                               _ptr_array(rec.nbt), len(rec.nbt), ptr(losses), ptr(w), ptr(out), ptr(flat_params),
                               ptr(flat_grads), flat_params.numel(), ptr(lr_dev), float(lr),
                               float(max_norm) if max_norm is not None else 0.0, None, stream_ptr()), "stg_train_tail")
    return out[0]


def dp_pack(flat_grad, bn_before, bn_after, num_peds, n_scenes, momentum, rank, world, pack):
    require_gpu(flat_grad, bn_before, bn_after, pack)
    peds = peds_arg(num_peds, n_scenes, flat_grad.device)
    check(lib().stg_dp_pack(ptr(flat_grad), ptr(bn_before), ptr(bn_after), ptr(peds), int(n_scenes), float(momentum),
                            int(rank), int(world), flat_grad.numel(), bn_before.numel(), ptr(pack), stream_ptr()),
          "stg_dp_pack")


def dp_fold(pack, bn_before, momentum, rank, world, n_params, buffers, nbt=()):
    require_gpu(pack, bn_before, buffers)
    check(lib().stg_dp_fold(ptr(pack), ptr(bn_before), float(momentum), int(rank), int(world), int(n_params),
                            bn_before.numel(), ptr(buffers), _ptr_array(nbt), len(nbt), stream_ptr()), "stg_dp_fold")


def weighted_sum(values, weights=None):
    require_gpu(values)
    values = values.contiguous()
    w = weights.to(torch.float32).contiguous() if weights is not None else None
    out = torch.empty(1, device=values.device, dtype=torch.float32)
    check(lib().stg_weighted_sum(ptr(values), ptr(w), values.numel(), ptr(out), stream_ptr()), "stg_weighted_sum")
    return out[0]


def sample_args(what, y, k, obs_last, noise, seed_dev=None):
    if y.dim() != 4 or y.shape[1] != 5:
        raise ValueError("%s: y (N,5,P,V) expected" % what)
    n, _, p, v = y.shape
    y = y.to(torch.float32)
    if obs_last is not None:
        if tuple(obs_last.shape) != (n, v, 2):
            raise ValueError("%s: obs_last (N,V,2) expected" % what)
        obs_last = obs_last.to(device=y.device, dtype=torch.float32).contiguous()
    if noise is not None:
        if tuple(noise.shape) != (k, n, p, v, 2):
            raise ValueError("%s: noise (K,N,P,V,2) expected" % what)
        noise = noise.to(device=y.device, dtype=torch.float32).contiguous()
    if seed_dev is not None and (seed_dev.numel() != 1 or seed_dev.dtype != torch.int64):
        raise ValueError("%s: seed_dev must be a one-element int64 device tensor" % what)
    return y, obs_last, noise, n, p, v


def best_of_k(y, target_rel, obs_last=None, num_peds=None, k=20, noise=None, seed=0):
    require_gpu(y, target_rel)
    k = int(k)
    y, obs_last, noise, n, p, v = sample_args("best_of_k", y, k, obs_last, noise)
    if tuple(target_rel.shape) != (n, p, v, 2):
        raise ValueError("best_of_k: target_rel (N,P,V,2) expected")
    target_rel = target_rel.to(torch.float32).contiguous()
    peds = peds_arg(num_peds, n, y.device)
    ade = torch.empty((n, v), device=y.device, dtype=torch.float32)
    fde = torch.empty((n, v), device=y.device, dtype=torch.float32)
    sn, sf, sp, sv = y.stride()
    check(lib().stg_bestofk_eval(ptr(y), sn, sf, sp, sv, ptr(target_rel), ptr(obs_last), ptr(peds), ptr(noise),
                                 seed_u64(seed), n, p, v, k, ptr(ade), ptr(fde), stream_ptr()),
          "stg_bestofk_eval")
    return ade, fde


def sample_trajectories(y, obs_last=None, num_peds=None, k=20, noise=None, seed=0, seed_dev=None, samples=None,
                        mean=None):
    require_gpu(y, seed_dev, samples, mean)
    k = int(k)
    if k < 0:
        raise ValueError("sample_trajectories: k must be >= 0")
    y, obs_last, noise, n, p, v = sample_args("sample_trajectories", y, k, obs_last, noise, seed_dev)
    for name, out, shape in (("samples", samples, (k, n, p, v, 2)), ("mean", mean, (n, p, v, 2))):
        if out is not None and (tuple(out.shape) != shape or out.dtype != torch.float32 or not out.is_contiguous()):
            raise ValueError("sample_trajectories: %s must be a contiguous float32 %s tensor" % (name, shape))
    peds = peds_arg(num_peds, n, y.device)
    if samples is None:
# ... 228 lines not shown
```

social_stgcnn_amd/trainer.py:

```python
import argparse
import math
import os
import pickle

import numpy as np
import torch
import torch.distributed as dist

from . import graphs, ops
from .metrics import bivariate_loss, rel_to_abs


def allreduce_flat(flat, group=None):
    if dist.is_available() and dist.is_initialized() and dist.get_world_size(group) > 1:
        dist.all_reduce(flat, op=dist.ReduceOp.SUM, group=group)
    return flat


def bn_fold_scale(counts, rank, momentum):
    keep = 1.0 - momentum
    own = keep ** int(counts[rank])
    later = keep ** int(sum(counts[rank + 1:]))
    total = keep ** int(sum(counts))
    return own, later, total


def fold_bn_across_ranks(before, after, n_local, momentum, group=None, counts=None):
    if not (dist.is_available() and dist.is_initialized()) or dist.get_world_size(group) == 1:
        return after
    world, rank = dist.get_world_size(group), dist.get_rank(group)
    if counts is None:
        t = torch.tensor([int(n_local)], dtype=torch.int64, device=after.device)
        parts = [torch.empty_like(t) for _ in range(world)]
        dist.all_gather(parts, t, group=group)
        counts = [int(p.item()) for p in parts]
    own, later, total = bn_fold_scale(counts, rank, momentum)
    contrib = (after - own * before) * later
    dist.all_reduce(contrib, op=dist.ReduceOp.SUM, group=group)
    return before * total + contrib


def pack_rank_slot(flat_grad, bn_before, bn_after, n_nonempty, momentum, rank, world):
    n_p, n_b = flat_grad.numel(), bn_before.numel()
    pack = torch.zeros(n_p + world * (n_b + 1), dtype=torch.float32, device=flat_grad.device)
    pack[:n_p] = flat_grad
    own = (1.0 - momentum) ** int(n_nonempty)
    lo = n_p + rank * (n_b + 1)
    pack[lo:lo + n_b] = bn_after - own * bn_before
    pack[lo + n_b] = float(n_nonempty)
    return pack


def fold_from_pack(pack, bn_before, momentum, world, n_params):
    n_b = bn_before.numel()
    keep = 1.0 - momentum
    slots = pack[n_params:].reshape(world, n_b + 1).double()
    counts = slots[:, n_b]
    later = torch.flip(torch.cumsum(torch.flip(counts, [0]), 0), [0]) - counts
    acc = (slots[:, :n_b] * (keep ** later)[:, None]).sum(0)
    return (bn_before.double() * keep ** counts.sum() + acc).float()


def broadcast_module(model, src=0, group=None):
    if dist.is_available() and dist.is_initialized() and dist.get_world_size(group) > 1:
        for t in list(model.parameters()) + list(model.buffers()):
            dist.broadcast(t.data, src=src, group=group)


def shard_scenes(num_peds, world, rank, balanced=True):
    counts = np.asarray(num_peds).reshape(-1)
    per = len(counts) // world
    if not balanced:
        return np.arange(rank * per, (rank + 1) * per)
    order = np.argsort(-counts, kind="stable")[: per * world]
    rounds = order.reshape(per, world)
    rounds[1::2] = rounds[1::2, ::-1]
    return np.sort(rounds[:, rank])


def group_weights(n_in_group, batch_size, device=None):
    w = torch.full((n_in_group,), 1.0 / batch_size, dtype=torch.float32)
    w[-1] = 0.0
    return w if device is None else w.to(device)


def group_bounds(n_scenes, batch_size):
    turn_point = int(n_scenes / batch_size) * batch_size + n_scenes % batch_size - 1
    return [i for i in range(n_scenes) if (i + 1) % batch_size == 0 or i == turn_point]


class Trainer:

    def __init__(self, model, lr=0.01, clip_grad=None, group=None, lr_sh_rate=None, lr_gamma=0.2):
        self.model = model
        self.base_lr = float(lr)
        self.lr = float(lr)
        self.clip_grad = clip_grad
        self.group = group
        self.lr_sh_rate = lr_sh_rate
        self.lr_gamma = lr_gamma
        self.epoch = 0
        self._lr_dev = None
        self.world = dist.get_world_size(group) if (dist.is_available() and dist.is_initialized()) else 1

    def _lr_tensor(self, device):
        if self._lr_dev is None or self._lr_dev.device != device:
            self._lr_dev = torch.full((1,), self.lr, device=device, dtype=torch.float32)
        return self._lr_dev

    def scheduler_step(self):
        self.epoch += 1
        if self.lr_sh_rate:
            self.lr = self.base_lr * self.lr_gamma ** (self.epoch // int(self.lr_sh_rate))
            if self._lr_dev is not None:
                self._lr_dev.fill_(self.lr)
        return self.lr

    def _update(self, flat_p, flat_g):
        ops.optim_step(flat_p, flat_g, self.lr, self.clip_grad, self._lr_tensor(flat_p.device))

    def _forward(self, x, adj, num_peds, defer_bn_fold=False):
        model = self.model
        for p in model.parameters():
            p.grad = None
        y, _ = model._forward(x, adj, num_peds, defer_bn_fold)
        return y, model._fwd_state

    def _backward(self, y, target, num_peds, weights, step=None):
        res = ops.backward_from_target(self.model, y.detach(), target, weights, step) if y.requires_grad else None
        if res is not None:
            return res if step is not None else (res, None)
        losses, dy = ops.bivariate_nll_with_grad(y.detach(), target, num_peds, weights)
        y.backward(dy)
        return losses, None

    def forward_backward(self, x, adj, target, num_peds=None, weights=None):
        y, _ = self._forward(x, adj, num_peds)
        losses, _ = self._backward(y, target, num_peds, weights)
        return ops.weighted_sum(losses, weights), losses, y.detach()

    def step(self, x, adj, target, num_peds=None, weights=None):
        if self.world > 1:
            out = self._before_allreduce(x, adj, target, num_peds, weights)
            self._allreduce()
            self._after_allreduce()
            return out
        model = self.model
        training = model.training
        y, rec = self._forward(x, adj, num_peds, defer_bn_fold=training)
        flat_p = model.flat_parameters()
        lr_dev = self._lr_tensor(flat_p.device)
        ride = training and self.clip_grad is None
        losses, total = self._backward(y, target, num_peds, weights, (self.lr, lr_dev) if ride else None)
        if total is None and training:
            total = ops.train_tail(rec, losses, weights, flat_p, self._flat_grad(), self.lr, self.clip_grad, lr_dev)
        elif total is None:
            ops.weighted_sum(losses, weights)
            total = ops.weighted_sum(losses, weights)
            self._update(flat_p, self._flat_grad())
        return total, losses, y.detach()

    def _dp_state(self):
        model = self.model
        flat_p = model.flat_parameters()
        flat_b = model._pb.ensure(model._tensors()[1])
        n = flat_p.numel() + self.world * (flat_b.numel() + 1)
        if getattr(self, "_pack", None) is None or self._pack.numel() != n or self._pack.device != flat_p.device:
            self._pack = torch.zeros(n, device=flat_p.device, dtype=torch.float32)
            self._bn_before = torch.empty_like(flat_b)
        return (flat_p, flat_b, self._pack, self._bn_before, model.st_gcns[0].tcn[0].momentum,
                dist.get_rank(self.group))

    def _before_allreduce(self, x, adj, target, num_peds, weights):
        _, flat_b, pack, before, mom, rank = self._dp_state()
        before.copy_(flat_b)
        out = self.forward_backward(x, adj, target, num_peds, weights)
        ops.dp_pack(self._flat_grad(), before, flat_b, num_peds, int(x.shape[0]), mom, rank, self.world, pack)
        return out

    def _allreduce(self):
        dist.all_reduce(self._pack, op=dist.ReduceOp.SUM, group=self.group)

    def _after_allreduce(self):
        flat_p, flat_b, pack, before, mom, rank = self._dp_state()
        n_p = flat_p.numel()
        ops.dp_fold(pack, before, mom, rank, self.world, n_p, flat_b, self.model._tensors()[2])
        self._update(flat_p, pack[:n_p])

    def capture(self, x, adj, target, num_peds=None, weights=None, warmup=3, pre=None):
        if num_peds is not None and not (torch.is_tensor(num_peds) and num_peds.is_cuda):
            raise ValueError("capture() needs num_peds as a device tensor (no host->device copies in a graph)")
        single = self.world == 1
        model = self.model
        flat_p = model.flat_parameters()
        flat_b = model._pb.ensure(model._tensors()[1])
        nbt = model._tensors()[2]
        self._lr_tensor(flat_p.device)
        saved = (flat_p.clone(), flat_b.clone(), [t.clone() for t in nbt])

        def ahead(fn):
            def run():
                if pre is not None:
                    pre()
                return fn(x, adj, target, num_peds, weights)
            return run
        graphs.warm_up(ahead(self.step if single else self.forward_backward), warmup)
        with torch.no_grad():
            flat_p.copy_(saved[0])
            flat_b.copy_(saved[1])
            for t, t0 in zip(nbt, saved[2]):
                t.copy_(t0)
        if single:
            graph, out = graphs.capture(ahead(self.step))
            self._graph = graph

            def replay():
                graph.replay()
                return out
            return replay

        self._dp_state()
        g_a, out = graphs.capture(ahead(self._before_allreduce))
        g_b, _ = graphs.capture(self._after_allreduce, pool=g_a.pool())
        self._graph = (g_a, g_b)

        def replay():
            g_a.replay()
            self._allreduce()
            g_b.replay()
            return out
        return replay

    def _flat_grad(self):
        flat = getattr(self.model, "_flat_grad", None)
        params = list(self.model._tensors()[0])
        if flat is not None and all(params[i].grad is None or params[i].grad.data_ptr() == flat.data_ptr() + 4 * off
                                    for i, off, _ in ops.flat_walk(params)):
            return flat
        return torch.cat([(p.grad if p.grad is not None else torch.zeros_like(p)).reshape(-1) for p in params])

    def train_epoch(self, batcher, n_scenes, batch_size):
        self.model.train()
        loss_sum, lo = 0.0, 0
        for b in group_bounds(n_scenes, batch_size):
            x, adj, target, peds = batcher(lo, b + 1)
            w = group_weights(b + 1 - lo, batch_size, x.device)
            total, _, _ = self.step(x, adj, target, peds, w)
            loss_sum += float(total)
            lo = b + 1
        return loss_sum / n_scenes

    @torch.no_grad()
    def val_epoch(self, batcher, n_scenes, batch_size):
        self.model.eval()
        loss_sum, lo = 0.0, 0
        for b in group_bounds(n_scenes, batch_size):
            x, adj, target, peds = batcher(lo, b + 1)
            y, _ = self.model(x, adj, peds)
            losses = bivariate_loss(y.permute(0, 2, 3, 1), target, peds)
            loss_sum += float((losses * group_weights(b + 1 - lo, batch_size, x.device)).sum())
            lo = b + 1
        return loss_sum / n_scenes


@torch.no_grad()
def evaluate_ade_fde(model, batches, k_steps=20):
    import torch.distributions.multivariate_normal as torchdist
    model.eval()
    ades, fdes = [], []
    for x, adj, peds, obs_last, tgt_rel in batches:
        y, _ = model(x, adj, peds)
        v_pred = y.permute(0, 2, 3, 1).cpu()
        n = v_pred.shape[0]
        counts = [v_pred.shape[2]] * n if peds is None else [int(c) for c in torch.as_tensor(peds).cpu()]
        obs_last = torch.as_tensor(obs_last).cpu().numpy()
        tgt_rel = torch.as_tensor(tgt_rel).cpu().numpy()
        for i in range(n):
            c = counts[i]
            vp = v_pred[i, :, :c]
            sx, sy, corr = torch.exp(vp[:, :, 2]), torch.exp(vp[:, :, 3]), torch.tanh(vp[:, :, 4])
            cov = torch.zeros(vp.shape[0], c, 2, 2)
            cov[:, :, 0, 0] = sx * sx
            cov[:, :, 0, 1] = corr * sx * sy
            cov[:, :, 1, 0] = corr * sx * sy
            cov[:, :, 1, 1] = sy * sy
            mvn = torchdist.MultivariateNormal(vp[:, :, 0:2], cov)
            tgt_abs = rel_to_abs(tgt_rel[i, :, :c], obs_last[i, :c]).astype(np.float64)
            s_abs = np.stack([rel_to_abs(mvn.sample().numpy(), obs_last[i, :c]) for _ in range(k_steps)])
            err = np.sqrt(((s_abs.astype(np.float64) - tgt_abs[None]) ** 2).sum(axis=3))
            ades += err.mean(axis=1).min(axis=0).tolist()
            fdes += err[:, -1].min(axis=0).tolist()
    return float(np.mean(ades)), float(np.mean(fdes)), ades, fdes


@torch.no_grad()
def evaluate_ade_fde_device(model, batches, k_steps=20, seed=0, noise_fn=None):
    model.eval()
    ades, fdes = [], []
    for b, (x, adj, peds, obs_last, tgt_rel) in enumerate(batches):
        y, _ = model(x, adj, peds)
        n, _, p, v = y.shape
# ... 62 lines not shown
```

Baseline: 10.05 million scene-windows/s.

## Fuse forward and backward scene kernels into a single training-step launch

Adds stg_model_step, which defers the forward scene kernel launch and runs one fused forward+backward+update kernel (launch_txp_step_x6) when the x6 scene path applies, plus a trainer fast path that calls it. This removes a kernel boundary and lets the backward work start inside the same launch as the forward, cutting launch overhead and the global-memory round trip between phases. It adds a new fused kernel whose register and LDS pressure may be higher, and a new opt-out flag to keep the phases separate.

```diff
diff --git a/include/stgcnn_hip.h b/include/stgcnn_hip.h
--- a/include/stgcnn_hip.h
+++ b/include/stgcnn_hip.h
@@ -58,6 +58,7 @@
 #define STG_OPT_SPLIT_BF16 2
 #define STG_OPT_BF16_STORE 8
 #define STG_OPT_F32_MFMA 16
+#define STG_OPT_SEPARATE_FB 32
 #define STG_OPT_WAVE_PATH 4
 
 int64_t stg_model_param_count(const stg_model_desc *d);
@@ -67,6 +68,8 @@
 int64_t stg_model_stat_floats(const stg_model_desc *d);
 int64_t stg_model_fwd_scratch_floats(const stg_model_desc *d, int N, int V);
 int64_t stg_model_bwd_scratch_floats(const stg_model_desc *d, int N, int V);
+int64_t stg_model_fwd_stamps_offset(const stg_model_desc *d, int N, int V);
+int64_t stg_model_bwd_stamps_offset(const stg_model_desc *d, int N, int V);
 
 int stg_model_fwd(const stg_model_desc *d, const float *params, const float *buffers,
                   const float *x, int64_t x_sn, int64_t x_sc, int64_t x_st, int64_t x_sv,
@@ -98,6 +101,12 @@
                        int N, int V, const float *y, const float *target, const float *weights, float *losses,
                        const float *ws, float *scratch, float *grad_params, const stg_step_tail *tail, void **events,
                        int n_events, void *stream);
+int stg_model_step(const stg_model_desc *d, const float *params, const float *buffers, const float *x, int64_t x_sn,
+                   int64_t x_sc, int64_t x_st, int64_t x_sv, const float *adj, int64_t a_sn, const int32_t *num_peds,
+                   int N, int V, float *y, float *ws, float *stats, float *fwd_scratch, const float *target,
+                   const float *weights, float *losses, float *bwd_scratch, float *grad_params,
+                   const stg_step_tail *tail, void **fwd_events, int n_fwd_events, void **bwd_events,
+                   int n_bwd_events, void *stream);
 int stg_bn_fold(const stg_model_desc *d, const float *stats, const int32_t *num_peds, int N,
                 float *buffers, int64_t *const *nbt, int n_bn, void *stream);
 
diff --git a/social_stgcnn_amd/_lib.py b/social_stgcnn_amd/_lib.py
--- a/social_stgcnn_amd/_lib.py
+++ b/social_stgcnn_amd/_lib.py
@@ -9,7 +9,7 @@
 DIAG = os.environ.get("STG_USE_DIAG_LIB", "0") not in ("", "0")
 LIB_PATH = os.path.join(CSRC, "libstgcnn_hip_diag.so" if DIAG else "libstgcnn_hip.so")
 ABI_VERSION = 8
-OPT_WG_PATH, OPT_SPLIT_BF16, OPT_WAVE_PATH, OPT_BF16_STORE, OPT_F32_MFMA = 1, 2, 4, 8, 16
+OPT_WG_PATH, OPT_SPLIT_BF16, OPT_WAVE_PATH, OPT_BF16_STORE, OPT_F32_MFMA, OPT_SEPARATE_FB = 1, 2, 4, 8, 16, 32
 EUNSUPPORTED = -2
 
 c_f = ctypes.c_void_p
@@ -51,6 +51,8 @@
     "stg_model_stat_floats": (c_l, [ctypes.POINTER(ModelDesc)]),
     "stg_model_fwd_scratch_floats": (c_l, [ctypes.POINTER(ModelDesc), c_i, c_i]),
     "stg_model_bwd_scratch_floats": (c_l, [ctypes.POINTER(ModelDesc), c_i, c_i]),
+    "stg_model_fwd_stamps_offset": (c_l, [ctypes.POINTER(ModelDesc), c_i, c_i]),
+    "stg_model_bwd_stamps_offset": (c_l, [ctypes.POINTER(ModelDesc), c_i, c_i]),
     "stg_model_fwd": (c_i, [ctypes.POINTER(ModelDesc), c_f, c_f, c_f, c_l, c_l, c_l, c_l, c_f, c_l, c_f, c_i, c_i,
                             c_f, c_f, c_f, c_f, ctypes.POINTER(ctypes.c_void_p), c_i, c_f]),
     "stg_model_bwd": (c_i, [ctypes.POINTER(ModelDesc), c_f, c_f, c_f, c_l, c_l, c_l, c_l, c_f, c_l, c_f, c_i, c_i,
@@ -60,6 +62,9 @@
     "stg_model_bwd_step": (c_i, [ctypes.POINTER(ModelDesc), c_f, c_f, c_f, c_l, c_l, c_l, c_l, c_f, c_l, c_f, c_i, c_i,
                                  c_f, c_f, c_f, c_f, c_f, c_f, c_f, ctypes.c_void_p, ctypes.POINTER(ctypes.c_void_p), c_i,
                                  c_f]),
+    "stg_model_step": (c_i, [ctypes.POINTER(ModelDesc), c_f, c_f, c_f, c_l, c_l, c_l, c_l, c_f, c_l, c_f, c_i, c_i,
+                             c_f, c_f, c_f, c_f, c_f, c_f, c_f, c_f, c_f, ctypes.c_void_p,
+                             ctypes.POINTER(ctypes.c_void_p), c_i, ctypes.POINTER(ctypes.c_void_p), c_i, c_f]),
     "stg_bn_fold": (c_i, [ctypes.POINTER(ModelDesc), c_f, c_f, c_i, c_f, ctypes.POINTER(ctypes.c_void_p), c_i, c_f]),
     "stg_nll_fwd": (c_i, [c_f, c_l, c_l, c_l, c_l, c_f, c_f, c_f, c_i, c_i, c_i, c_f, c_f, c_f]),
     "stg_nll_bwd": (c_i, [c_f, c_f, c_i, c_i, c_i, c_f, c_f]),
diff --git a/social_stgcnn_amd/csrc/model_bwd.hip b/social_stgcnn_amd/csrc/model_bwd.hip
--- a/social_stgcnn_amd/csrc/model_bwd.hip
+++ b/social_stgcnn_amd/csrc/model_bwd.hip
@@ -376,7 +376,7 @@
 }
 
 struct BwdCarve {
-    int64_t rows, slab2, dzg, order, total;
+    int64_t rows, slab2, dzg, order, stamps, total;
 };
 static bool bwd_carve(const ModelLayout &L, const StepPath &path, int N, int V, BwdCarve *c, WgradGeom *wg) {
     const int g1 = bwd_grid(L, path, N, V);
@@ -397,6 +397,11 @@
     }
     c->order = fl;
     c->total = fl + order_floats(N, V);
+    c->stamps = -1;
+    if (diag_env("STG_STAMPS", 0) != 0) {
+        c->stamps = c->total;
+        c->total += (int64_t)N * 32;
+    }
     return true;
 }
 
@@ -414,13 +419,26 @@
     if (!stg::bwd_carve(l, stg::choose_path(l, N, V), N, V, &c, &wg)) return stg::fail(STG_ELDS, "stg_model_bwd: V=%d does not fit the LDS of one CU", V);
     return c.total;
 }
-
-static int model_bwd_impl(const stg_model_desc *d, const float *params, const float *buffers, const float *x, int64_t x_sn,
-                          int64_t x_sc, int64_t x_st, int64_t x_sv, const float *adj, int64_t a_sn,
-                          const int32_t *num_peds, int N, int V, const float *dy, const float *nll_target,
-                          const float *nll_weights, float *nll_losses, const stg_step_tail *tail, const float *ws,
-                          float *scratch, float *grad_params, float *dx, void **events, int n_events, void *stream) {
-    using namespace stg;
+int64_t stg_model_bwd_stamps_offset(const stg_model_desc *d, int N, int V) {
+    stg::ModelLayout l;
+    const int rc = stg::make_layout(d, &l);
+    if (rc != STG_OK) return rc;
+    if (N <= 0 || V <= 0) return stg::fail(STG_EINVAL, "stg_model_bwd_stamps_offset: N=%d V=%d", N, V);
+    stg::BwdCarve c;
+    stg::WgradGeom wg{};
+    if (!stg::bwd_carve(l, stg::choose_path(l, N, V), N, V, &c, &wg)) return stg::fail(STG_ELDS, "stg_model_bwd: V=%d does not fit the LDS of one CU", V);
+    return c.stamps >= 0 ? c.stamps : STG_EUNSUPPORTED;
+}
+
+}
+
+namespace stg {
+
+int model_bwd_impl(const stg_model_desc *d, const float *params, const float *buffers, const float *x, int64_t x_sn,
+                   int64_t x_sc, int64_t x_st, int64_t x_sv, const float *adj, int64_t a_sn, const int32_t *num_peds,
+                   int N, int V, const float *dy, const float *nll_target, const float *nll_weights, float *nll_losses,
+                   const stg_step_tail *tail, const float *ws, float *scratch, float *grad_params, float *dx,
+                   void **events, int n_events, void *stream, const TxpFwdArgs *deferred) {
     BwdArgs a{};
     const int rc = make_layout(d, &a.lay);
     if (rc != STG_OK) return rc;
@@ -487,10 +505,14 @@
         t.split_bf16 = (L.flags & STG_OPT_SPLIT_BF16) ? 1 : 0;
         t.stagger = diag_env("STG_STAGGER_B", 0);
         if (wt.wp >= 0) t.wp = reinterpret_cast<const unsigned *>(ws_end + wt.wp);
-        const int rcw = launch_scene_bwd(path, t, st);
+        if (cv.stamps >= 0) t.stamps = reinterpret_cast<unsigned long long *>(scratch + cv.stamps);
+        STG_REQUIRE(!deferred || step_one_launch(L, path, num_peds, N, V), STG_EINVAL,
+                    "stg_model_bwd: a deferred scene launch outside the one-launch step");
+        const int rcw = deferred ? launch_scene_step(*deferred, t, st) : launch_scene_bwd(path, t, st);
         if (rcw != STG_OK) return rcw;
         slab_rows = N;
     } else {
+        STG_REQUIRE(!deferred, STG_EINVAL, "stg_model_bwd: a deferred scene launch outside the one-launch step");
         const int waves = bwd_waves(path, V);
         const size_t lds = bwd_lds_bytes(L, V, waves);
         STG_REQUIRE(lds <= (size_t)kLdsBytes, STG_ELDS, "stg_model_bwd: V=%d needs %zu bytes of LDS (> %d)", V, lds,
@@ -567,12 +589,18 @@
     return STG_OK;
 }
 
+}
+
+extern "C" {
+
+using stg::model_bwd_impl;
+
 int stg_model_bwd(const stg_model_desc *d, const float *params, const float *buffers, const float *x, int64_t x_sn,
                   int64_t x_sc, int64_t x_st, int64_t x_sv, const float *adj, int64_t a_sn, const int32_t *num_peds,
                   int N, int V, const float *dy, const float *ws, float *scratch, float *grad_params, float *dx,
                   void **events, int n_events, void *stream) {
     return model_bwd_impl(d, params, buffers, x, x_sn, x_sc, x_st, x_sv, adj, a_sn, num_peds, N, V, dy, nullptr, nullptr,
-                          nullptr, nullptr, ws, scratch, grad_params, dx, events, n_events, stream);
+                          nullptr, nullptr, ws, scratch, grad_params, dx, events, n_events, stream, nullptr);
 }
 
 int stg_model_bwd_nll(const stg_model_desc *d, const float *params, const float *buffers, const float *x, int64_t x_sn,
@@ -581,7 +609,7 @@
                       const float *ws, float *scratch, float *grad_params, void **events, int n_events, void *stream) {
     if (!target || !losses || (N > 0 && !y)) return stg::fail(STG_EINVAL, "stg_model_bwd_nll: null pointer");
     return model_bwd_impl(d, params, buffers, x, x_sn, x_sc, x_st, x_sv, adj, a_sn, num_peds, N, V, y, target, weights,
-                          losses, nullptr, ws, scratch, grad_params, nullptr, events, n_events, stream);
+                          losses, nullptr, ws, scratch, grad_params, nullptr, events, n_events, stream, nullptr);
 }
 
 int stg_model_bwd_step(const stg_model_desc *d, const float *params, const float *buffers, const float *x, int64_t x_sn,
@@ -594,7 +622,33 @@
         return stg::fail(STG_EINVAL, "stg_model_bwd_step: bad tail");
     if (N == 0) return STG_EUNSUPPORTED;
     return model_bwd_impl(d, params, buffers, x, x_sn, x_sc, x_st, x_sv, adj, a_sn, num_peds, N, V, y, target, weights,
-                          losses, tail, ws, scratch, grad_params, nullptr, events, n_events, stream);
-}
-
-}
+                          losses, tail, ws, scratch, grad_params, nullptr, events, n_events, stream, nullptr);
+}
+
+int stg_model_step(const stg_model_desc *d, const float *params, const float *buffers, const float *x, int64_t x_sn,
+                   int64_t x_sc, int64_t x_st, int64_t x_sv, const float *adj, int64_t a_sn, const int32_t *num_peds,
+                   int N, int V, float *y, float *ws, float *stats, float *fwd_scratch, const float *target,
+                   const float *weights, float *losses, float *bwd_scratch, float *grad_params,
+                   const stg_step_tail *tail, void **fwd_events, int n_fwd_events, void **bwd_events,
+                   int n_bwd_events, void *stream) {
+    using namespace stg;
+    if (!target || !losses || !y || !ws) return fail(STG_EINVAL, "stg_model_step: null pointer");
+    if (!tail || !tail->params || (tail->stats && !tail->buffers) || tail->n_bn < 0 || tail->n_bn > 3 * STG_MAX_BLOCKS)
+        return fail(STG_EINVAL, "stg_model_step: bad tail");
+    ModelLayout L;
+    const int rc = make_layout(d, &L);
+    if (rc != STG_OK) return rc;
+    STG_REQUIRE(N >= 0 && V > 0, STG_EINVAL, "stg_model_step: bad sizes N=%d V=%d", N, V);
+    if (N == 0 || (L.flags & STG_OPT_SPLIT_BF16) || L.n_txp == 0) return STG_EUNSUPPORTED;
+    STG_REQUIRE(grad_params && bwd_scratch, STG_EINVAL, "stg_model_step: null pointer");
+    TxpFwdArgs f{};
+    const bool one = step_one_launch(L, choose_path(L, N, V), num_peds, N, V);
+    const int rcf = model_fwd_impl(d, params, buffers, x, x_sn, x_sc, x_st, x_sv, adj, a_sn, num_peds, N, V, y, ws, stats,
+                                   fwd_scratch, fwd_events, n_fwd_events, stream, one ? &f : nullptr);
+    if (rcf != STG_OK) return rcf;
+    return model_bwd_impl(d, params, buffers, x, x_sn, x_sc, x_st, x_sv, adj, a_sn, num_peds, N, V, y, target, weights,
+                          losses, tail, ws, bwd_scratch, grad_params, nullptr, bwd_events, n_bwd_events, stream,
+                          one ? &f : nullptr);
+}
+
+}
diff --git a/social_stgcnn_amd/csrc/model_fwd.hip b/social_stgcnn_amd/csrc/model_fwd.hip
--- a/social_stgcnn_amd/csrc/model_fwd.hip
+++ b/social_stgcnn_amd/csrc/model_fwd.hip
@@ -180,13 +180,10 @@
     return (size_t)(plane + reg + waves * 16 + 16) * sizeof(float);
 }
 
-}
-
-extern "C" int stg_model_fwd(const stg_model_desc *d, const float *params, const float *buffers, const float *x,
-                             int64_t x_sn, int64_t x_sc, int64_t x_st, int64_t x_sv, const float *adj,
-                             int64_t a_sn, const int32_t *num_peds, int N, int V, float *y, float *ws,
-                             float *stats, float *scratch, void **events, int n_events, void *stream) {
-    using namespace stg;
+int model_fwd_impl(const stg_model_desc *d, const float *params, const float *buffers, const float *x, int64_t x_sn,
+                   int64_t x_sc, int64_t x_st, int64_t x_sv, const float *adj, int64_t a_sn, const int32_t *num_peds,
+                   int N, int V, float *y, float *ws, float *stats, float *scratch, void **events, int n_events,
+                   void *stream, TxpFwdArgs *defer) {
     FwdArgs a{};
     const int rc = make_layout(d, &a.lay);
     if (rc != STG_OK) return rc;
@@ -205,6 +202,8 @@
     const FwdCarve fc = fwd_carve(L, path, N, V);
     const WsTail wt = ws_tail(L, path, N, V);
     float *ws_end = ws ? ws + wt.base : nullptr;
+    STG_REQUIRE(!defer || step_one_launch(L, path, num_peds, N, V), STG_EINVAL,
+                "stg_model_fwd: a scene launch deferred outside the one-launch step");
     STG_REQUIRE(path.scene() || !(L.flags & STG_OPT_BF16_STORE), STG_EUNSUPPORTED,
                 "stg_model_fwd: bf16 storage (STG_OPT_BF16_STORE) is built for the wave-per-scene kernels only "
                 "(one st_gcn block, input_feat 2, V <= 68, no STG_OPT_WG_PATH)");
@@ -258,7 +257,8 @@
         t.Vl = V;
         t.debug_skip = a.debug_skip;
         t.stagger = diag_env("STG_STAGGER_F", 0);
-        const int rcw = launch_scene_fwd(path, t, st);
+        if (defer) *defer = t;
+        const int rcw = defer ? STG_OK : launch_scene_fwd(path, t, st);
         evl.mark();
         evl.finish();
         return rcw;
@@ -281,3 +281,13 @@
     evl.finish();
     return STG_OK;
 }
+
+}
+
+extern "C" int stg_model_fwd(const stg_model_desc *d, const float *params, const float *buffers, const float *x,
+                             int64_t x_sn, int64_t x_sc, int64_t x_st, int64_t x_sv, const float *adj,
+                             int64_t a_sn, const int32_t *num_peds, int N, int V, float *y, float *ws,
+                             float *stats, float *scratch, void **events, int n_events, void *stream) {
+    return stg::model_fwd_impl(d, params, buffers, x, x_sn, x_sc, x_st, x_sv, adj, a_sn, num_peds, N, V, y, ws, stats,
+                               scratch, events, n_events, stream, nullptr);
+}
diff --git a/social_stgcnn_amd/csrc/model_layout.hip b/social_stgcnn_amd/csrc/model_layout.hip
--- a/social_stgcnn_amd/csrc/model_layout.hip
+++ b/social_stgcnn_amd/csrc/model_layout.hip
@@ -23,7 +23,8 @@
     STG_REQUIRE(d->bn_mode == 0 || d->bn_mode == 1, STG_EINVAL, "bn_mode=%d (0 eval, 1 per-scene train)", d->bn_mode);
     STG_REQUIRE(d->residual0 >= 0 && d->residual0 <= 2, STG_EINVAL, "residual0=%d", d->residual0);
     STG_REQUIRE(d->residual0 != 1 || d->c_in == d->c_out, STG_EINVAL, "identity residual needs c_in == c_out");
-    STG_REQUIRE((d->flags & ~(STG_OPT_WG_PATH | STG_OPT_SPLIT_BF16 | STG_OPT_WAVE_PATH | STG_OPT_BF16_STORE | STG_OPT_F32_MFMA)) == 0, STG_EINVAL,
+    STG_REQUIRE((d->flags & ~(STG_OPT_WG_PATH | STG_OPT_SPLIT_BF16 | STG_OPT_WAVE_PATH | STG_OPT_BF16_STORE | STG_OPT_F32_MFMA |
+                              STG_OPT_SEPARATE_FB)) == 0, STG_EINVAL,
                 "unknown flags 0x%x", d->flags);
     STG_REQUIRE(d->wg_waves == 0 || d->wg_waves == 1 || d->wg_waves == 2 || d->wg_waves == 4 || d->wg_waves == 8,
                 STG_EINVAL, "wg_waves=%d (0 auto, 1, 2, 4, 8)", d->wg_waves);
@@ -92,6 +93,12 @@
     return path.bwd_x6 ? launch_txp_bwd_x6(a, st) : launch_txp_bwd_wave(a, st);
 }
 
+bool step_one_launch(const ModelLayout &L, const StepPath &path, const int32_t *num_peds, int N, int V) {
+    return path.kind == StepPath::SceneX6 && path.fwd_x6 && path.bwd_x6 && !(L.flags & STG_OPT_SEPARATE_FB) &&
+           txp_step_x6_fits(L, num_peds, N, V);
+}
+int launch_scene_step(const TxpFwdArgs &f, const TxpBwdArgs &b, hipStream_t st) { return launch_txp_step_x6(f, b, st); }
+
 __global__ __launch_bounds__(1024) void scene_order_kernel(const int32_t *__restrict__ num_peds, int N, int V,
                                                            int32_t *__restrict__ order,
                                                            int32_t *__restrict__ key_start,
@@ -148,6 +155,14 @@
     if (N < 0 || V <= 0) return stg::fail(STG_EINVAL, "stg_model_fwd_scratch_floats: N=%d V=%d", N, V);
     return stg::fwd_carve(l, stg::choose_path(l, N, V), N, V).total;
 }
+int64_t stg_model_fwd_stamps_offset(const stg_model_desc *d, int N, int V) {
+    stg::ModelLayout l;
+    const int rc = stg::make_layout(d, &l);
+    if (rc != STG_OK) return rc;
+    if (N < 0 || V <= 0) return stg::fail(STG_EINVAL, "stg_model_fwd_stamps_offset: N=%d V=%d", N, V);
+    const int64_t off = stg::fwd_carve(l, stg::choose_path(l, N, V), N, V).stamps;
+    return off >= 0 ? off : STG_EUNSUPPORTED;
+}
 int stg_scene_order(const int32_t *num_peds, int N, int V, int32_t *order, int32_t *key_start, void *stream) {
     STG_REQUIRE(N >= 0 && V > 0, STG_EINVAL, "stg_scene_order: bad sizes N=%d V=%d", N, V);
     if (N == 0) return STG_OK;
diff --git a/social_stgcnn_amd/csrc/step_plan.hpp b/social_stgcnn_amd/csrc/step_plan.hpp
--- a/social_stgcnn_amd/csrc/step_plan.hpp
+++ b/social_stgcnn_amd/csrc/step_plan.hpp
@@ -30,4 +30,17 @@
 int launch_scene_fwd(const StepPath &path, const TxpFwdArgs &a, hipStream_t st);
 int launch_scene_bwd(const StepPath &path, const TxpBwdArgs &a, hipStream_t st);
 
+bool step_one_launch(const ModelLayout &L, const StepPath &path, const int32_t *num_peds, int N, int V);
+int launch_scene_step(const TxpFwdArgs &f, const TxpBwdArgs &b, hipStream_t st);
+
+int model_fwd_impl(const stg_model_desc *d, const float *params, const float *buffers, const float *x, int64_t x_sn,
+                   int64_t x_sc, int64_t x_st, int64_t x_sv, const float *adj, int64_t a_sn, const int32_t *num_peds,
+                   int N, int V, float *y, float *ws, float *stats, float *scratch, void **events, int n_events,
+                   void *stream, TxpFwdArgs *defer);
+int model_bwd_impl(const stg_model_desc *d, const float *params, const float *buffers, const float *x, int64_t x_sn,
+                   int64_t x_sc, int64_t x_st, int64_t x_sv, const float *adj, int64_t a_sn, const int32_t *num_peds,
+                   int N, int V, const float *dy, const float *nll_target, const float *nll_weights, float *nll_losses,
+                   const stg_step_tail *tail, const float *ws, float *scratch, float *grad_params, float *dx,
+                   void **events, int n_events, void *stream, const TxpFwdArgs *deferred);
+
 }
diff --git a/social_stgcnn_amd/csrc/txp_scene_common.hpp b/social_stgcnn_amd/csrc/txp_scene_common.hpp
--- a/social_stgcnn_amd/csrc/txp_scene_common.hpp
+++ b/social_stgcnn_amd/csrc/txp_scene_common.hpp
@@ -64,6 +64,7 @@
     float *dzg;
     const unsigned *wp;
     float *rows;
+    unsigned long long *stamps;
     int debug_skip;
     int split_bf16;
     int stagger;
@@ -74,6 +75,8 @@
 int64_t txp_bwd_x6_wp_floats(const ModelLayout &L);
 int launch_txp_fwd_x6(const TxpFwdArgs &a, hipStream_t st);
 int launch_txp_bwd_x6(const TxpBwdArgs &a, hipStream_t st);
+bool txp_step_x6_fits(const ModelLayout &L, const int32_t *num_peds, int N, int V);
+int launch_txp_step_x6(const TxpFwdArgs &f, const TxpBwdArgs &b, hipStream_t st);
 
 __host__ __device__ inline int ptab_floats(int v) { return ((Cfg::T * v + 1) / 2 + 3) & ~3; }
 __host__ __device__ inline int bwd_ptab_floats(int v) { return ptab_floats(v) + kRedMax; }
diff --git a/social_stgcnn_amd/csrc/txp_x6.hip b/social_stgcnn_amd/csrc/txp_x6.hip
--- a/social_stgcnn_amd/csrc/txp_x6.hip
+++ b/social_stgcnn_amd/csrc/txp_x6.hip
@@ -48,6 +48,15 @@
     if constexpr (S == Shape::Generic) return L.ws_z[l];
     else return kCanonLayout.ws_z[l];
 }
+
+#ifdef STG_DIAG
+#define STG_X6_STAMP(a, n, k)                                                                                          \
+    do {                                                                                                              \
+        if ((a).stamps && (threadIdx.x & 63) == 0) (a).stamps[(int64_t)(n) * 16 + (k)] = __builtin_amdgcn_s_memrealtime(); \
+    } while (0)
+#else
+#define STG_X6_STAMP(a, n, k) do { } while (0)
+#endif
 
 constexpr int kF6Tiles = 10, kF6Slots = 7;
 
@@ -217,8 +226,10 @@
         const int n = __builtin_amdgcn_readfirstlane(a.tier.order ? scene_index(a.tier.order[begin + it], a.N) : it);
         int vi = a.num_peds ? a.num_peds[n] : a.V;
         vi = __builtin_amdgcn_readfirstlane(vi < 0 ? 0 : (vi > a.V ? a.V : vi));
+        STG_X6_STAMP(a, n, 0);
         txp_fwd_scene_x6<BF, SoloScene, S>(a, params, blk_p, blk_b, n, vi, region, ptab, SoloScene{vi});
         __builtin_amdgcn_wave_barrier();
+        STG_X6_STAMP(a, n, 8);
     }
 }
 
@@ -499,9 +510,48 @@
         const int n = __builtin_amdgcn_readfirstlane(a.tier.order ? scene_index(a.tier.order[begin + it], a.N) : it);
         int vi = a.num_peds ? a.num_peds[n] : a.V;
         vi = __builtin_amdgcn_readfirstlane(vi < 0 ? 0 : (vi > a.V ? a.V : vi));
+        STG_X6_STAMP(a, n, 0);
         txp_bwd_scene_x6<BF, SoloScene, S>(a, blk_p, n, vi, region, ptab, SoloScene{vi});
         __builtin_amdgcn_wave_barrier();
-    }
+        STG_X6_STAMP(a, n, 8);
+    }
+}
+
+__host__ __device__ inline int step6_per_wave_floats(int v) {
+    const int f = fwd6_region_floats(v) + ptab_floats(v), b = bwd6_region_floats(v) + bwd_ptab_floats(v);
+    return f > b ? f : b;
+}
+
+template <int WPB, bool BF>
+__global__ __launch_bounds__(WPB * 64, 2) __attribute__((amdgpu_waves_per_eu(2, 2))) void txp_step_x6_kernel(
+    const TxpFwdArgs f0, const TxpBwdArgs b0) {
+    constexpr Shape S = Shape::Canon32;
+    extern __shared__ __attribute__((aligned(16))) float sm[];
+    TxpFwdArgs f = f0;
+    fold_shape<S>(f);
+    f.agg_stride = kCanonAggStride32[1];
+    f.agg_ax = kCanonAggAx32[1];
+    f.agg_cs = kCanonAggCs32[1];
+    TxpBwdArgs b = b0;
+    fold_shape<S>(b);
+    const int wave = threadIdx.x >> 6;
+    const int per_wave = step6_per_wave_floats(kCanonV);
+    float *region = sm + wave * per_wave;
+    ptab_t *ptab = reinterpret_cast<ptab_t *>(region + bwd6_region_floats(kCanonV));
+    float *blk_p = sm + WPB * per_wave, *blk_b = blk_p + ((kCanonLayout.n_blk_params + 3) & ~3);
+    stage_block_params(f.lay, f.params, f.buffers, blk_p, blk_b, WPB * 64);
+    const int n = __builtin_amdgcn_readfirstlane(blockIdx.x * WPB + wave);
+    if (n >= f.N) return;
+    STG_X6_STAMP(f, n, 0);
+    txp_fwd_scene_x6<BF, SoloScene, S>(f, f.params, blk_p, blk_b, n, kCanonV, region, ptab, SoloScene{kCanonV});
+    __builtin_amdgcn_fence(__ATOMIC_RELEASE, "wavefront");
+    __builtin_amdgcn_wave_barrier();
+    __builtin_amdgcn_fence(__ATOMIC_ACQUIRE, "wavefront");
+    STG_X6_STAMP(f, n, 8);
+    STG_X6_STAMP(b, n, 0);
+    txp_bwd_scene_x6<BF, SoloScene, S>(b, blk_p, n, kCanonV, region, ptab, SoloScene{kCanonV});
+    __builtin_amdgcn_wave_barrier();
+    STG_X6_STAMP(b, n, 8);
 }
 
 struct TeamCount {
@@ -737,4 +787,35 @@
                   wpb == 8 ? bwd_x6_kernel<8>(bf, sh) : bwd_x6_kernel<4>(bf, sh), a);
 }
 
-}
+static bool step_x6_plain(int debug_skip_f, int debug_skip_b, int stagger_f, int stagger_b) {
+    const size_t pf = (size_t)(fwd6_region_floats(kCanonV) + ptab_floats(kCanonV)) * sizeof(float);
+    const size_t pb = (size_t)(bwd6_region_floats(kCanonV) + bwd_ptab_floats(kCanonV)) * sizeof(float);
+    return !debug_skip_f && !debug_skip_b && !stagger_f && !stagger_b && wave_wpb(pf) != 8 && wave_wpb(pb) != 8;
+}
+bool txp_step_x6_fits(const ModelLayout &L, const int32_t *num_peds, int N, int V) {
+    TeamGeom g;
+    const int skip = diag_env("STG_DEBUG_SKIP", 0);
+    return is_canonical(L) && V == kCanonV && !num_peds && txp_fwd_x6_fits(L, V) && txp_bwd_x6_fits(L, V) &&
+           !team_wanted(N, V, true, &g) &&
+           step_x6_plain(skip, skip, diag_env("STG_STAGGER_F", 0), diag_env("STG_STAGGER_B", 0));
+}
+static bool txp_step_x6_applies(const TxpFwdArgs &f, const TxpBwdArgs &b) {
+    if (!f.wpf || !b.wp || !f.ws || f.ws != b.ws || f.N != b.N || f.V != b.V || f.params != b.params) return false;
+    if (f.lay.flags != b.lay.flags || !step_x6_plain(f.debug_skip, b.debug_skip, f.stagger, b.stagger)) return false;
+    TeamGeom g;
+    if (team_wanted(f.N, f.V, f.num_peds == nullptr, &g) || team_wanted(b.N, b.V, b.num_peds == nullptr, &g)) return false;
+    bool okf, okb;
+    if (canon_shape(f, &okf) != Shape::Canon32 || canon_shape(b, &okb) != Shape::Canon32) return false;
+    return okf && okb && canon32_agg_matches(f);
+}
+int launch_txp_step_x6(const TxpFwdArgs &f, const TxpBwdArgs &b, hipStream_t st) {
+    STG_REQUIRE(txp_step_x6_applies(f, b), STG_EINVAL, "txp_step_x6: the batch is outside the one-launch scene kernel");
+    constexpr int wpb = 4;
+    const size_t lds = ((size_t)step6_per_wave_floats(kCanonV) * wpb + wave_param_floats(f.lay)) * sizeof(float);
+    const bool bf = (f.lay.flags & STG_OPT_BF16_STORE) != 0;
+    STG_REQUIRE(2 * lds <= (size_t)kLdsBytes, STG_ELDS, "txp_step_x6: %zu bytes of LDS do not fit two workgroups per CU", lds);
+    return launch(Launch{"txp_step_x6", dim3((f.N + wpb - 1) / wpb), dim3(wpb * 64), lds, st},
+                  bf ? txp_step_x6_kernel<wpb, true> : txp_step_x6_kernel<wpb, false>, f, b);
+}
+
+}
diff --git a/social_stgcnn_amd/model.py b/social_stgcnn_amd/model.py
--- a/social_stgcnn_amd/model.py
+++ b/social_stgcnn_amd/model.py
@@ -164,9 +164,14 @@
         return self._forward(v, a, num_peds)
 
     def _forward(self, v, a, num_peds=None, defer_bn_fold=False):
-        assert a.size(-3) == self.st_gcns[0].gcn.kernel_size
         if self.n_txpcnn < 1:
             raise NotImplementedError("social_stgcnn needs n_txpcnn >= 1 (model.py:168 always builds tpcnns[0])")
+        desc, flat_p, flat_b, nbt, dead, params = self._launch_args(a)
+        y = ops.fused_model(v, a, num_peds, desc, flat_p, flat_b, nbt, dead, params, self, defer_bn_fold)
+        return y, a
+
+    def _launch_args(self, a):
+        assert a.size(-3) == self.st_gcns[0].gcn.kernel_size
         for blk in self.st_gcns:
             _check_block(blk, self.training)
         params, bufs, nbt, dead = self._tensors()
@@ -176,5 +181,16 @@
         desc = ops.make_desc(self.n_stgcnn, self.n_txpcnn, self.input_feat, self.output_feat, self.seq_len,
                              self.pred_seq_len, self.kt, self.st_gcns[0].residual_kind, False, self.training,
                              bn.eps, bn.momentum, options=getattr(self, "options", None))
-        y = ops.fused_model(v, a, num_peds, desc, flat_p, flat_b, nbt, dead, params, self, defer_bn_fold)
-        return y, a
+        return desc, flat_p, flat_b, nbt, dead, params
+
+    def _step(self, v, a, target, num_peds, weights, lr, lr_dev):
+        if self.n_txpcnn < 1 or not self.training:
+            return None
+        desc, flat_p, flat_b, nbt, dead, params = self._launch_args(a)
+        res = ops.fused_step(v, a, num_peds, desc, flat_p, flat_b, nbt, dead, params, self, target, weights, lr, lr_dev)
+        if res is None:
+            return None
+        y, losses, total, grads = res
+        for p, g in zip(params, grads):
+            p.grad = g
+        return y, losses, total
diff --git a/social_stgcnn_amd/ops.py b/social_stgcnn_amd/ops.py
--- a/social_stgcnn_amd/ops.py
+++ b/social_stgcnn_amd/ops.py
@@ -153,7 +153,7 @@
 
 class KernelOptions(dict):
     DEFAULTS = {"wg_path": False, "split_bf16": False, "wg_waves": 0, "wave_path": False, "bf16_store": False,
-                "f32_mfma": False}
+                "f32_mfma": False, "separate_fb": False}
 
     def __init__(self, **kw):
         bad = set(kw) - set(self.DEFAULTS)
@@ -172,7 +172,8 @@
     flags = ((_lib.OPT_WG_PATH if o["wg_path"] else 0) | (_lib.OPT_SPLIT_BF16 if o["split_bf16"] else 0)
              | (_lib.OPT_WAVE_PATH if o["wave_path"] else 0)
              | (_lib.OPT_BF16_STORE if o["bf16_store"] else 0)
-             | (_lib.OPT_F32_MFMA if o["f32_mfma"] else 0))
+             | (_lib.OPT_F32_MFMA if o["f32_mfma"] else 0)
+             | (_lib.OPT_SEPARATE_FB if o["separate_fb"] else 0))
     return ModelDesc(n_stgcnn, n_txpcnn, c_in, c_out, t_obs, t_pred, kt, residual0, 1 if use_mdn else 0,
                      1 if training else 0, eps, momentum, flags, int(o["wg_waves"]))
 
@@ -241,19 +242,76 @@
     n: int = 0
 
 
+def _check_model_input(x, adj, desc, flat_params, flat_buffers):
+    require_gpu(x, adj, flat_params, flat_buffers)
+    _lib.as_f32(x, "x")
+    _lib.as_f32(adj, "adj")
+    n, cin, t, v = x.shape
+    if cin != desc.c_in or t != desc.t_obs:
+        raise ValueError("input (N,%d,%d,V) does not match the model (input_feat=%d, seq_len=%d)"
+                         % (cin, t, desc.c_in, desc.t_obs))
+    return n, cin, t, v
+
+
+def _fwd_buffers(desc, n, v, dev, save, training, holder):
+    L, d = lib(), ctypes.byref(desc)
+    out_t = desc.t_pred if desc.n_txpcnn > 0 else desc.t_obs
+    y = torch.empty((n, desc.c_out, out_t, v), device=dev, dtype=torch.float32)
+    ws = None
+    if save:
+        wsf = _size(L.stg_model_ws_floats(d, v), "stg_model_ws_floats")
+        tail = _size(L.stg_model_ws_tail_floats(d, n, v), "stg_model_ws_tail_floats")
+        ws = torch.empty(n * wsf + tail, device=dev, dtype=torch.float32)
+    stats = None
+    if training:
+        sf = L.stg_model_stat_floats(d)
+        stats = torch.empty((n, max(int(sf), 1)), device=dev, dtype=torch.float32)
+    scr = None
+    nscr = _size(L.stg_model_fwd_scratch_floats(d, n, v), "stg_model_fwd_scratch_floats")
+    if nscr > 0:
+        scr = torch.empty(nscr, device=dev, dtype=torch.float32)
+    if holder is not None:
+        holder.last_ws_floats = ws.numel() if save else 0
+        holder._last_fwd_scratch = scr
+    return y, ws, stats, scr
+
+
+def _bwd_buffers(desc, n, v, dev):
+    L, d = lib(), ctypes.byref(desc)
+    np_ = int(L.stg_model_param_count(d))
+    n_scratch = _size(L.stg_model_bwd_scratch_floats(d, n, v), "stg_model_bwd_scratch_floats")
+    slabs = torch.empty(n_scratch, device=dev, dtype=torch.float32)
+    grad = torch.empty(np_, device=dev, dtype=torch.float32)
+    return slabs, grad
+
+
+def _step_tail(flat_params, flat_buffers, step, stats, nbt):
+    lr, lr_dev = step
+    total = torch.empty(1, device=flat_params.device, dtype=torch.float32)
+    tail = _lib.StepTail()
+    tail.params, tail.lr_dev, tail.lr = ptr(flat_params), ptr(lr_dev), float(lr)
+    tail.total = ptr(total)
+    arr = None
+    if stats is not None:
+        arr = _ptr_array(nbt)
+        tail.stats, tail.buffers, tail.nbt, tail.n_bn = ptr(stats), ptr(flat_buffers), arr, len(nbt)
+    return tail, total, arr
+
+
+def _grad_views(grad, shapes, dead, holder):
+    if holder is not None:
+        holder._flat_grad = grad
+        holder._fwd_state = None
+    return [None if i in dead else grad[off:off + cnt].view(shapes[i]) for i, off, cnt in flat_walk(shapes)]
+
+
 class _FusedModel(torch.autograd.Function):
 
     @staticmethod
     def forward(ctx, x, adj, num_peds, desc, flat_params, flat_buffers, nbt, dead, holder, grad_on, defer_bn_fold,
                 *params):
-        require_gpu(x, adj, flat_params, flat_buffers)
-        _lib.as_f32(x, "x")
-        _lib.as_f32(adj, "adj")
+        n, cin, t, v = _check_model_input(x, adj, desc, flat_params, flat_buffers)
         L = lib()
-        n, cin, t, v = x.shape
-        if cin != desc.c_in or t != desc.t_obs:
-            raise ValueError("input (N,%d,%d,V) does not match the model (input_feat=%d, seq_len=%d)"
-                             % (cin, t, desc.c_in, desc.t_obs))
         adj_c, a_sn = _adj_layout(adj, n, t, v)
         peds = peds_arg(num_peds, n, x.device)
         training = desc.bn_mode == 1
@@ -262,24 +320,7 @@
             fields = {f: getattr(desc, f) for f, _ in ModelDesc._fields_}
             fields["flags"] |= _lib.OPT_WG_PATH
             desc = ModelDesc(**fields)
-        out_t = desc.t_pred if desc.n_txpcnn > 0 else desc.t_obs
-        y = torch.empty((n, desc.c_out, out_t, v), device=x.device, dtype=torch.float32)
-        ws = None
-        if need_grad:
-            wsf = _size(L.stg_model_ws_floats(ctypes.byref(desc), v), "stg_model_ws_floats")
-            tail = _size(L.stg_model_ws_tail_floats(ctypes.byref(desc), n, v), "stg_model_ws_tail_floats")
-            ws = torch.empty(n * wsf + tail, device=x.device, dtype=torch.float32)
-        stats = None
-        if training:
-            sf = L.stg_model_stat_floats(ctypes.byref(desc))
-            stats = torch.empty((n, max(int(sf), 1)), device=x.device, dtype=torch.float32)
-        scr = None
-        nscr = _size(L.stg_model_fwd_scratch_floats(ctypes.byref(desc), n, v), "stg_model_fwd_scratch_floats")
-        if nscr > 0:
-            scr = torch.empty(nscr, device=x.device, dtype=torch.float32)
-        if holder is not None:
-            holder.last_ws_floats = ws.numel() if need_grad else 0
-            holder._last_fwd_scratch = scr
+        y, ws, stats, scr = _fwd_buffers(desc, n, v, x.device, need_grad, training, holder)
         sn, sc, st, sv = x.stride()
         timer = _timer_of(holder)
         ev = timer.events("model_fwd") if timer is not None else None
@@ -312,10 +353,7 @@
     L = lib()
     desc, x = rec.desc, rec.x
     n, cin, t, v = x.shape
-    np_ = int(L.stg_model_param_count(ctypes.byref(desc)))
-    n_scratch = _size(L.stg_model_bwd_scratch_floats(ctypes.byref(desc), n, v), "stg_model_bwd_scratch_floats")
-    slabs = torch.empty(n_scratch, device=x.device, dtype=torch.float32)
-    grad = torch.empty(np_, device=x.device, dtype=torch.float32)
+    slabs, grad = _bwd_buffers(desc, n, v, x.device)
     sn, sc, st, sv = x.stride()
     timer = _timer_of(holder)
     ev = timer.events("model_bwd") if timer is not None else None
@@ -331,14 +369,7 @@
         if step is None:
             name, rc = "stg_model_bwd_nll", L.stg_model_bwd_nll(*head, *mid, *end)
         else:
-            lr, lr_dev = step
-            total = torch.empty(1, device=x.device, dtype=torch.float32)
-            tail = _lib.StepTail()
-            tail.params, tail.lr_dev, tail.lr = ptr(rec.flat_params), ptr(lr_dev), float(lr)
-            tail.total = ptr(total)
-            if rec.stats is not None:
-                arr = _ptr_array(rec.nbt)
-                tail.stats, tail.buffers, tail.nbt, tail.n_bn = ptr(rec.stats), ptr(rec.flat_buffers), arr, len(rec.nbt)
+            tail, total, keep = _step_tail(rec.flat_params, rec.flat_buffers, step, rec.stats, rec.nbt)
             name, rc = "stg_model_bwd_step", L.stg_model_bwd_step(*head, *mid, ctypes.addressof(tail), *end)
             out = (losses, total[0])
         if rc == _lib.EUNSUPPORTED:
@@ -346,12 +377,7 @@
                 timer.calls["model_bwd"].pop()
             return None
     check(rc, name)
-    grads = [None if i in rec.dead else grad[off:off + cnt].view(rec.shapes[i])
-             for i, off, cnt in flat_walk(rec.shapes)]
-    if holder is not None:
-        holder._flat_grad = grad
-        holder._fwd_state = None
-    return grads, out
+    return _grad_views(grad, rec.shapes, rec.dead, holder), out
 
 
 def backward_from_target(holder, y, target, weights=None, step=None):
@@ -371,6 +397,41 @@
     for p, g in zip(holder._tensors()[0], res[0]):
         p.grad = g
     return res[1]
+
+
+def fused_step(x, adj, num_peds, desc, flat_params, flat_buffers, nbt, dead, params, holder, target, weights, lr,
+               lr_dev):
+    n, cin, t, v = _check_model_input(x, adj, desc, flat_params, flat_buffers)
+    if desc.bn_mode != 1 or desc.n_txpcnn < 1 or n == 0 or (desc.flags & _lib.OPT_SPLIT_BF16):
+        return None
+    target = target.to(torch.float32).contiguous()
+    if tuple(target.shape) != (n, desc.t_pred, v, 2):
+        raise ValueError("fused_step: target (N,P,V,2) expected, got %s" % (tuple(target.shape),))
+    w = weights.to(torch.float32).contiguous() if weights is not None else None
+    adj_c, a_sn = _adj_layout(adj, n, t, v)
+    peds = peds_arg(num_peds, n, x.device)
+    y, ws, stats, scr = _fwd_buffers(desc, n, v, x.device, True, True, holder)
+    slabs, grad = _bwd_buffers(desc, n, v, x.device)
+    if holder is not None:
+        holder._last_bwd_scratch = slabs
+    losses = torch.empty(n, device=x.device, dtype=torch.float32)
+    tail, total, keep = _step_tail(flat_params, flat_buffers, (lr, lr_dev), stats, nbt)
+    timer = _timer_of(holder)
+    ev_f = timer.events("model_fwd") if timer is not None else None
+    ev_b = timer.events("model_bwd") if timer is not None else None
+    sn, sc, st, sv = x.stride()
+    rc = lib().stg_model_step(ctypes.byref(desc), ptr(flat_params), ptr(flat_buffers), ptr(x), sn, sc, st, sv, ptr(adj_c),
+                              a_sn, ptr(peds), n, v, ptr(y), ptr(ws), ptr(stats), ptr(scr), ptr(target), ptr(w),
+                              ptr(losses), ptr(slabs), ptr(grad), ctypes.addressof(tail),
+                              ev_f.arr if ev_f else None, ev_f.n if ev_f else 0,
+                              ev_b.arr if ev_b else None, ev_b.n if ev_b else 0, stream_ptr())
+    if rc == _lib.EUNSUPPORTED:
+        if timer is not None:
+            timer.calls["model_fwd"].pop()
+            timer.calls["model_bwd"].pop()
+        return None
+    check(rc, "stg_model_step")
+    return y, losses, total[0], _grad_views(grad, [tuple(p.shape) for p in params], dead, holder)
 
 
 def fused_model(x, adj, num_peds, desc, flat_params, flat_buffers, nbt, dead, params, holder=None,
diff --git a/social_stgcnn_amd/trainer.py b/social_stgcnn_amd/trainer.py
--- a/social_stgcnn_amd/trainer.py
+++ b/social_stgcnn_amd/trainer.py
@@ -147,6 +147,14 @@
             return out
         model = self.model
         training = model.training
+        if (training and self.clip_grad is None and torch.is_grad_enabled() and not x.requires_grad
+                and all(p.requires_grad for p in model.parameters())):
+            for p in model.parameters():
+                p.grad = None
+            res = model._step(x, adj, target, num_peds, weights, self.lr, self._lr_tensor(model.flat_parameters().device))
+            if res is not None:
+                y, losses, total = res
+                return total, losses, y
         y, rec = self._forward(x, adj, num_peds, defer_bn_fold=training)
         flat_p = model.flat_parameters()
         lr_dev = self._lr_tensor(flat_p.device)
```

Result: faster. 10.54 million scene-windows/s, median of 6 (+4.9%).
